# HicrestLaboratory/SPARTA

Hardware: AMD Instinct MI355X
Metric: Block-sparse SpMM GFLOP/s (higher is better)
Workload: dtype f32; 1 GPU; cant-like FEM 9x9x257 mesh x 3 dof (62451^2, 4325625 nnz; a synthetic STAND-IN for SuiteSparse cant, which cannot be fetched here), B = 128 cols, fp32; col_block_size=32, n_cols=128, block_rows=1952, nonzero_blocks=21910, vbs_area=22435840, parallelism=single GPU, launch=eager, preroll_steps=6457, kernel_rev=r5i

## Files before the change

### include/sparta_amd.h

```cpp
#ifndef SPARTA_AMD_H
#define SPARTA_AMD_H

#include <stdint.h>

#ifdef __cplusplus
extern "C" {
#endif

#define SPARTA_OK               0
#define SPARTA_ERR_INVALID     -1
#define SPARTA_ERR_ALLOC       -2
#define SPARTA_ERR_HIP         -3
#define SPARTA_ERR_UNSUPPORTED -4
#define SPARTA_ERR_IO          -5
#define SPARTA_ERR_NO_DEVICE   -6

#define SPARTA_F32  0
#define SPARTA_F16  1
#define SPARTA_BF16 2

#define SPARTA_COL_MAJOR 0
#define SPARTA_ROW_MAJOR 1

#define SPARTA_PTR_HOST   0
// ... 124 lines not shown

int sparta_vbs_save(const char* path, const sparta_vbs_host* v);
int sparta_vbs_load(const char* path, sparta_vbs_host* out);

int sparta_vbs_to_blocked_ell(const sparta_vbs_host* v, int64_t* ell_cols_out, int64_t* ell_col_ind, float* ell_values);

int sparta_blocking_info(int64_t rows, int64_t cols, const int64_t* rowptr, const int32_t* colidx,
                         const int64_t* grouping, int64_t col_block_size, int64_t* info_out, float* avg_height_out);

typedef struct sparta_vbs sparta_vbs_t;

int sparta_vbs_create(sparta_vbs_t** out, int64_t rows, int64_t cols, int64_t block_rows, int64_t block_col_size,
                      const int64_t* row_part, const int64_t* nzcount, const int64_t* jab, const float* mab,
                      int32_t dtype, int32_t device);

int sparta_vbs_create_range(sparta_vbs_t** out, int64_t rows, int64_t cols, int64_t block_rows, int64_t block_col_size,
                            const int64_t* row_part, const int64_t* nzcount, const int64_t* jab, const float* mab,
                            int64_t block_row_begin, int64_t block_row_end, int32_t dtype, int32_t device);

#define SPARTA_CREATE_UPDATABLE 1
#define SPARTA_CREATE_TRANSPOSE 2
int sparta_vbs_create_range_ex(sparta_vbs_t** out, int64_t rows, int64_t cols, int64_t block_rows, int64_t block_col_size,
                               const int64_t* row_part, const int64_t* nzcount, const int64_t* jab, const float* mab,
                               int64_t block_row_begin, int64_t block_row_end, int32_t dtype, int32_t device, int32_t flags);
int sparta_vbs_flags(const sparta_vbs_t* A, int32_t* flags_out);

int sparta_vbs_create_from_csr(sparta_vbs_t** out, int64_t rows, int64_t cols, const int64_t* rowptr, const int32_t* colidx, const float* vals,
                               const int64_t* grouping, int64_t col_block_size, int64_t row_block_size, int32_t force_fixed_size,
                               int32_t dtype, int32_t device);

int sparta_vbs_plan_stats(int64_t rows, int64_t cols, const int64_t* rowptr, const int32_t* colidx, const float* vals, const int64_t* grouping,
                          int64_t col_block_size, int64_t row_block_size, int32_t force_fixed_size, int32_t dtype, int64_t* stats);

int sparta_vbs_spmm(sparta_vbs_t* A, const void* B, int64_t ldb, int32_t b_layout, int32_t n_cols,
                    void* C, int64_t ldc, int32_t c_layout, int32_t accumulate,
                    int32_t ptr_space, void* stream, int32_t algo, float* dt_ms);

int sparta_vbs_spmm_gathered(sparta_vbs_t* A, const void* B_gathered, int64_t shard_rows, int64_t shard_stride, int32_t n_cols,
                             void* C, int64_t ldc, int32_t c_layout, int32_t accumulate, void* stream, int32_t algo, float* dt_ms);
int sparta_vbs_spmm_gathered_ld(sparta_vbs_t* A, const void* B_gathered, int64_t shard_rows, int64_t shard_ld, int64_t shard_stride, int32_t n_cols,
                                void* C, int64_t ldc, int32_t c_layout, int32_t accumulate, void* stream, int32_t algo, float* dt_ms);

int sparta_pack_blocks(const void* src, int64_t block_bytes, const int32_t* ids_dev, int64_t n_blocks, void* dst, void* stream);

int sparta_vbs_create_transposed(sparta_vbs_t** out, int64_t rows, int64_t cols, int64_t block_rows, int64_t block_col_size,
                                 const int64_t* row_part, const int64_t* nzcount, const int64_t* jab, const float* mab,
                                 int32_t dtype, int32_t device);
int sparta_vbs_spmm_ba(sparta_vbs_t* At, const void* B, int64_t ldb, int32_t M, void* C, int64_t ldc, int32_t accumulate,
                       int32_t ptr_space, void* stream, float* dt_ms);

int sparta_vbs_sddmm(sparta_vbs_t* A, const void* X, int64_t ldx, const void* Y, int64_t ldy, int32_t k, float* G, int32_t accumulate,
                     int32_t ptr_space, void* stream, float* dt_ms);

int sparta_vbs_set_values(sparta_vbs_t* A, const float* mab, int32_t ptr_space, void* stream, float* dt_ms);

typedef struct sparta_sgd_cfg { float lr, momentum, weight_decay, grad_scale; } sparta_sgd_cfg;
int sparta_vbs_sgd_step(sparta_vbs_t* A, float* W, const float* G, float* M, const sparta_sgd_cfg* cfg, void* stream, float* dt_ms);

typedef struct sparta_adam_cfg { float lr, beta1, beta2, eps, weight_decay, grad_scale; int32_t decoupled; int32_t reserved; } sparta_adam_cfg;
int sparta_vbs_adam_step(sparta_vbs_t* A, float* W, const float* G, float* M, float* V, void* S,
                         const sparta_adam_cfg* cfg, void* stream, float* dt_ms);
int sparta_vbs_step_info(const sparta_vbs_t* A, int64_t* info_out);

#define SPARTA_GRAD_CTL_BYTES 16448
#define SPARTA_GRAD_STATS_CHUNK 4096
#define SPARTA_GRAD_STATS_MAX_GRID 1024
typedef struct sparta_grad_ctl_cfg {
    float max_norm, growth_factor, backoff_factor;
    int32_t growth_interval;
    int32_t reserved[4];
} sparta_grad_ctl_cfg;
int sparta_grad_stats(const float* G, int64_t n, void* R, int32_t accumulate, void* stream, float* dt_ms);
int sparta_grad_ctl_finish(void* R, const sparta_grad_ctl_cfg* cfg, void* stream);
int sparta_vbs_sgd_step_ctl(sparta_vbs_t* A, float* W, const float* G, float* M, const sparta_sgd_cfg* cfg, const void* R, void* stream, float* dt_ms);
int sparta_vbs_adam_step_ctl(sparta_vbs_t* A, float* W, const float* G, float* M, float* V, void* S,
                             const sparta_adam_cfg* cfg, const void* R, void* stream, float* dt_ms);

int sparta_vbs_spmm_t(sparta_vbs_t* A, const void* X, int64_t ldx, int32_t n_cols, float* Ct, int64_t ldo, int32_t accumulate,
                      int32_t ptr_space, void* stream, float* dt_ms);
int sparta_spmm_t_host_check(int64_t rows, int64_t cols, int64_t block_rows, int64_t block_col_size, const int64_t* row_part,
                             const int64_t* nzcount, const int64_t* jab, const float* mab, int64_t block_row_begin, int64_t block_row_end,
                             const float* x, double* y, int64_t* info_out);
int sparta_frag_positions(const uint8_t* nonempty, uint8_t* pos, int32_t* pairs);

typedef struct sparta_b sparta_b_t;
int sparta_vbs_prepare_b(sparta_vbs_t* A, const void* B, int64_t ldb, int64_t shard_rows, int64_t shard_stride, int32_t n_cols, void* stream,
                         sparta_b_t** out);
int sparta_vbs_spmm_prepared(sparta_vbs_t* A, const sparta_b_t* Bp, void* C, int64_t ldc, int32_t c_layout, int32_t accumulate, void* stream,
                             float* dt_ms);
int sparta_b_destroy(sparta_b_t* Bp);

int sparta_vbs_set_class_timing(sparta_vbs_t* A, int32_t enable);
int sparta_vbs_class_times(sparta_vbs_t* A, float* ms_out);

int sparta_vbs_clock_mhz(sparta_vbs_t* A, double* mhz_out);

int sparta_vbs_destroy(sparta_vbs_t* A);

int sparta_vbs_info(const sparta_vbs_t* A, int64_t* info_out);

int sparta_vbs_sparse_info(const sparta_vbs_t* A, int64_t* info_out);

int sparta_vbs_colres_info(const sparta_vbs_t* A, int64_t* info_out);
int sparta_colres_host_check(int64_t rows, int64_t cols, const int64_t* rowptr, const int32_t* colidx, const float* vals, const int64_t* crow, const float* x,
                             float* y, int64_t* info_out);

int sparta_vbs_union_info(const sparta_vbs_t* A, int64_t* info_out);
int sparta_union_host_check(int64_t rows, int64_t cols, const int64_t* rowptr, const int32_t* colidx, const float* vals, const int64_t* grouping, int64_t col_block_size,
                            int64_t row_block_size, int32_t force_fixed_size, int32_t max_workers, const float* x, double* y, int64_t* info_out);

int sparta_vbs_hub_info(const sparta_vbs_t* A, int64_t* info_out);

int sparta_device_count(void);

const char* sparta_last_error(void);
const char* sparta_version(void);

#ifdef __cplusplus
}
#endif
#endif
```

### sparta_amd/__init__.py

```python
from ._lib import (SpartaError, LIB_PATH, F32, F16, BF16, COL_MAJOR, ROW_MAJOR, SPMM_MFMA, SPMM_EXACT,
                   FMT_EL, FMT_MTX, IO_COMPAT, IO_STRICT)
from .host import (CSR, BlockingEngine, VBR, get_permutation, get_partition, get_fixed_size_grouping,
                   row_distance, merge_rows, BLOCKING_ALGOS, save_grouping, read_grouping_file, blocking_csv_row,
                   save_blocking_data, CSV_COLUMNS)
from .device import DeviceVBS, vbs_multiply, device_count
from . import gen, dist, autograd, optim, gradctl
from .optim import VbsSGD, VbsAdamW
from .gradctl import GradCtl

KERNEL_REV = "r5i"

cublas_fixed_blocks_multiply = vbs_multiply
cublas_blockmat_batched = vbs_multiply
cutlas_fixed_blocks_multiply = vbs_multiply
cutlas_blockmat_batched = vbs_multiply
```

### sparta_amd/_lib.py

```python
import ctypes as C
import os

try:
    import torch
except ImportError:
    torch = None

_HERE = os.path.dirname(os.path.abspath(__file__))
LIB_PATH = os.environ.get("SPARTA_AMD_LIB") or os.path.join(_HERE, "libsparta_amd.so")

OK, ERR_INVALID, ERR_ALLOC, ERR_HIP, ERR_UNSUPPORTED, ERR_IO, ERR_NO_DEVICE = 0, -1, -2, -3, -4, -5, -6
F32, F16, BF16 = 0, 1, 2
COL_MAJOR, ROW_MAJOR = 0, 1
PTR_HOST, PTR_DEVICE = 0, 1
SPMM_MFMA, SPMM_EXACT = 0, 1
CREATE_UPDATABLE = 1
CREATE_TRANSPOSE = 2
GRAD_CTL_BYTES, GRAD_STATS_CHUNK, GRAD_STATS_MAX_GRID = 16448, 4096, 1024
FMT_EL, FMT_MTX = 0, 1
IO_COMPAT, IO_STRICT = 0, 1

SYMBOLS = [
    "sparta_reorder_cfg_default", "sparta_reorder", "sparta_get_permutation", "sparta_get_partition",
    "sparta_get_fixed_size_grouping", "sparta_row_distance", "sparta_merge_rows", "sparta_vbs_build",
    "sparta_vbs_host_free", "sparta_blocking_info", "sparta_vbs_create", "sparta_vbs_create_range", "sparta_vbs_create_from_csr",
    "sparta_vbs_spmm", "sparta_vbs_spmm_gathered", "sparta_vbs_spmm_gathered_ld", "sparta_pack_blocks", "sparta_vbs_create_transposed", "sparta_vbs_spmm_ba", "sparta_vbs_set_class_timing",
    "sparta_vbs_class_times", "sparta_vbs_clock_mhz", "sparta_vbs_destroy", "sparta_vbs_info", "sparta_vbs_sparse_info", "sparta_vbs_colres_info", "sparta_colres_host_check", "sparta_vbs_union_info", "sparta_union_host_check", "sparta_vbs_hub_info", "sparta_device_count", "sparta_last_error",
    "sparta_version",
    "sparta_csr_read", "sparta_csr_read_buffer", "sparta_csr_host_free", "sparta_csr_write_edgelist", "sparta_grouping_write", "sparta_grouping_read",
    "sparta_blocking_csv_row", "sparta_degree_permutation", "sparta_vbs_save", "sparta_vbs_load", "sparta_vbs_to_blocked_ell",
    "sparta_vbs_build_partition", "sparta_vbs_partition_check", "sparta_vbs_plan_stats",
    "sparta_vbs_prepare_b", "sparta_vbs_spmm_prepared", "sparta_b_destroy",
    "sparta_vbs_sddmm",
    "sparta_vbs_create_range_ex", "sparta_vbs_set_values", "sparta_vbs_flags", "sparta_frag_positions",
    "sparta_vbs_spmm_t", "sparta_spmm_t_host_check",
    "sparta_vbs_sgd_step", "sparta_vbs_step_info", "sparta_vbs_adam_step",
    "sparta_grad_stats", "sparta_grad_ctl_finish", "sparta_vbs_sgd_step_ctl", "sparta_vbs_adam_step_ctl",
]


class CsrHost(C.Structure):
    _fields_ = [("rows", C.c_int64), ("cols", C.c_int64), ("nnz", C.c_int64), ("pattern_only", C.c_int32),
                ("rowptr", C.POINTER(C.c_int64)), ("colidx", C.POINTER(C.c_int32)), ("vals", C.POINTER(C.c_float))]


class CsvFields(C.Structure):
    _fields_ = [("matrix", C.c_char_p), ("rows", C.c_int64), ("cols", C.c_int64), ("nonzeros", C.c_int64),
                ("symmetrize", C.c_int32), ("blocking_algo", C.c_int32), ("tau", C.c_float),
                ("row_block_size", C.c_int32), ("col_block_size", C.c_int32), ("use_pattern", C.c_int32),
                ("sim_use_groups", C.c_int32), ("sim_measure", C.c_int32), ("reorder", C.c_int32),
                ("exp_name", C.c_char_p), ("b_cols", C.c_int32), ("warmup", C.c_int32), ("exp_repetitions", C.c_int32),
                ("multiplication_algo", C.c_int32), ("n_streams", C.c_int32),
                ("time_to_block", C.c_float), ("time_to_merge", C.c_float), ("time_to_compare", C.c_float),
                ("vbr_nzcount", C.c_int64), ("vbr_nzblocks_count", C.c_int64), ("vbr_average_height", C.c_float),
                ("vbr_longest_row", C.c_int64), ("merge_counter", C.c_int64), ("comparison_counter", C.c_int64),
                ("average_merge_tau", C.c_float), ("average_row_distance", C.c_float),
                ("avg_time_multiply", C.c_float), ("std_time_multiply", C.c_float)]


class ReorderCfg(C.Structure):
    _fields_ = [("blocking_algo", C.c_int32), ("sim_measure", C.c_int32), ("tau", C.c_float), ("use_groups", C.c_int32),
                ("col_block_size", C.c_int64), ("row_block_size", C.c_int64), ("use_pattern", C.c_int32),
                ("force_fixed_size", C.c_int32), ("structured_m", C.c_int32), ("structured_n", C.c_int32),
                ("minhash_bands", C.c_int32), ("minhash_rows", C.c_int32), ("minhash_max_eval", C.c_int32), ("minhash_max_rows", C.c_int32)]


class ReorderStats(C.Structure):
    _fields_ = [("comparison_counter", C.c_int64), ("merge_counter", C.c_int64), ("average_row_distance", C.c_float),
                ("average_merge_tau", C.c_float), ("timer_total", C.c_float), ("timer_comparisons", C.c_float),
                ("timer_merges", C.c_float), ("reserved", C.c_int32)]


class VbsHost(C.Structure):
    _fields_ = [("rows", C.c_int64), ("cols", C.c_int64), ("block_rows", C.c_int64), ("block_cols", C.c_int64),
                ("block_col_size", C.c_int64), ("nztot", C.c_int64), ("nblocks", C.c_int64),
                ("row_part", C.POINTER(C.c_int64)), ("nzcount", C.POINTER(C.c_int64)), ("jab", C.POINTER(C.c_int64)),
                ("mab", C.POINTER(C.c_float))]


class SgdCfg(C.Structure):
    _fields_ = [("lr", C.c_float), ("momentum", C.c_float), ("weight_decay", C.c_float), ("grad_scale", C.c_float)]


class AdamCfg(C.Structure):
    _fields_ = [("lr", C.c_float), ("beta1", C.c_float), ("beta2", C.c_float), ("eps", C.c_float), ("weight_decay", C.c_float),
                ("grad_scale", C.c_float), ("decoupled", C.c_int32), ("reserved", C.c_int32)]


class GradCtlCfg(C.Structure):
    _fields_ = [("max_norm", C.c_float), ("growth_factor", C.c_float), ("backoff_factor", C.c_float), ("growth_interval", C.c_int32),
                ("reserved", C.c_int32 * 4)]


class SpartaError(RuntimeError):
    def __init__(self, code, msg):
        super().__init__("sparta_amd error %d: %s" % (code, msg))
        self.code = code


def _load():
    if not os.path.exists(LIB_PATH):
        raise ImportError("sparta_amd: %s is missing -- build it with `make -C sparta_amd/csrc` "
                          "(python -c 'import __graft_entry__ as g; g.build()'). There is no CPU fallback." % LIB_PATH)
    L = C.CDLL(LIB_PATH)
    i64p, i32p, f32p, vp = C.POINTER(C.c_int64), C.POINTER(C.c_int32), C.POINTER(C.c_float), C.c_void_p
    L.sparta_reorder_cfg_default.argtypes = [C.POINTER(ReorderCfg)]
    L.sparta_reorder_cfg_default.restype = None
    L.sparta_reorder.argtypes = [C.c_int64, C.c_int64, i64p, i32p, C.POINTER(ReorderCfg), i64p, C.POINTER(ReorderStats)]
    L.sparta_get_permutation.argtypes = [i64p, C.c_int64, i64p]
    L.sparta_get_partition.argtypes = [i64p, C.c_int64, i64p, i64p]
    L.sparta_get_fixed_size_grouping.argtypes = [i64p, C.c_int64, C.c_int64, i64p]
    L.sparta_row_distance.argtypes = [C.c_int32, i64p, C.c_int64, C.c_int64, i64p, C.c_int64, C.c_int64, C.c_int64, f32p]
    L.sparta_merge_rows.argtypes = [i64p, C.c_int64, i64p, C.c_int64, i64p, i64p]
    L.sparta_vbs_build.argtypes = [C.c_int64, C.c_int64, i64p, i32p, f32p, i64p, C.c_int64, C.c_int64, C.c_int32,
                                   C.POINTER(VbsHost)]
    L.sparta_vbs_host_free.argtypes = [C.POINTER(VbsHost)]
    L.sparta_vbs_build_partition.argtypes = [C.c_int64, C.c_int64, i64p, i32p, f32p, i64p, C.c_int64, C.c_int64, C.POINTER(VbsHost)]
    L.sparta_vbs_partition_check.argtypes = [i64p, C.c_int64, C.c_int64]
    L.sparta_vbs_save.argtypes = [C.c_char_p, C.POINTER(VbsHost)]
    L.sparta_vbs_load.argtypes = [C.c_char_p, C.POINTER(VbsHost)]
    L.sparta_vbs_to_blocked_ell.argtypes = [C.POINTER(VbsHost), i64p, i64p, f32p]
    L.sparta_vbs_host_free.restype = None
    L.sparta_blocking_info.argtypes = [C.c_int64, C.c_int64, i64p, i32p, i64p, C.c_int64, i64p, f32p]
    L.sparta_vbs_create.argtypes = [C.POINTER(vp), C.c_int64, C.c_int64, C.c_int64, C.c_int64, i64p, i64p, i64p, f32p,
                                    C.c_int32, C.c_int32]
    L.sparta_vbs_create_range.argtypes = [C.POINTER(vp), C.c_int64, C.c_int64, C.c_int64, C.c_int64, i64p, i64p, i64p, f32p,
                                          C.c_int64, C.c_int64, C.c_int32, C.c_int32]
    L.sparta_vbs_create_range_ex.argtypes = [C.POINTER(vp), C.c_int64, C.c_int64, C.c_int64, C.c_int64, i64p, i64p, i64p, f32p,
                                             C.c_int64, C.c_int64, C.c_int32, C.c_int32, C.c_int32]
    L.sparta_vbs_set_values.argtypes = [vp, f32p, C.c_int32, vp, f32p]
    L.sparta_vbs_sgd_step.argtypes = [vp, f32p, f32p, f32p, C.POINTER(SgdCfg), vp, f32p]
    L.sparta_vbs_adam_step.argtypes = [vp, f32p, f32p, f32p, f32p, vp, C.POINTER(AdamCfg), vp, f32p]
    L.sparta_vbs_step_info.argtypes = [vp, i64p]
    L.sparta_grad_stats.argtypes = [f32p, C.c_int64, vp, C.c_int32, vp, f32p]
    L.sparta_grad_ctl_finish.argtypes = [vp, C.POINTER(GradCtlCfg), vp]
    L.sparta_vbs_sgd_step_ctl.argtypes = [vp, f32p, f32p, f32p, C.POINTER(SgdCfg), vp, vp, f32p]
    L.sparta_vbs_adam_step_ctl.argtypes = [vp, f32p, f32p, f32p, f32p, vp, C.POINTER(AdamCfg), vp, vp, f32p]
    L.sparta_vbs_flags.argtypes = [vp, i32p]
    L.sparta_vbs_spmm_t.argtypes = [vp, vp, C.c_int64, C.c_int32, f32p, C.c_int64, C.c_int32, C.c_int32, vp, f32p]
    L.sparta_spmm_t_host_check.argtypes = [C.c_int64, C.c_int64, C.c_int64, C.c_int64, i64p, i64p, i64p, f32p, C.c_int64, C.c_int64, f32p, C.POINTER(C.c_double), i64p]
    L.sparta_frag_positions.argtypes = [C.POINTER(C.c_uint8), C.POINTER(C.c_uint8), i32p]
    L.sparta_vbs_create_from_csr.argtypes = [C.POINTER(vp), C.c_int64, C.c_int64, i64p, i32p, f32p, i64p, C.c_int64, C.c_int64, C.c_int32, C.c_int32, C.c_int32]
    L.sparta_vbs_plan_stats.argtypes = [C.c_int64, C.c_int64, i64p, i32p, f32p, i64p, C.c_int64, C.c_int64, C.c_int32, C.c_int32, i64p]
    L.sparta_vbs_prepare_b.argtypes = [vp, vp, C.c_int64, C.c_int64, C.c_int64, C.c_int32, vp, C.POINTER(vp)]
    L.sparta_vbs_spmm_prepared.argtypes = [vp, vp, vp, C.c_int64, C.c_int32, C.c_int32, vp, f32p]
    L.sparta_b_destroy.argtypes = [vp]
    L.sparta_vbs_create_transposed.argtypes = [C.POINTER(vp), C.c_int64, C.c_int64, C.c_int64, C.c_int64, i64p, i64p, i64p, f32p, C.c_int32, C.c_int32]
    L.sparta_vbs_spmm_ba.argtypes = [vp, vp, C.c_int64, C.c_int32, vp, C.c_int64, C.c_int32, C.c_int32, vp, f32p]
    L.sparta_vbs_spmm.argtypes = [vp, vp, C.c_int64, C.c_int32, C.c_int32, vp, C.c_int64, C.c_int32, C.c_int32, C.c_int32, vp,
                                  C.c_int32, f32p]
    L.sparta_vbs_sddmm.argtypes = [vp, vp, C.c_int64, vp, C.c_int64, C.c_int32, f32p, C.c_int32, C.c_int32, vp, f32p]
    L.sparta_vbs_spmm_gathered.argtypes = [vp, vp, C.c_int64, C.c_int64, C.c_int32, vp, C.c_int64, C.c_int32, C.c_int32, vp, C.c_int32, f32p]
    L.sparta_vbs_spmm_gathered_ld.argtypes = [vp, vp, C.c_int64, C.c_int64, C.c_int64, C.c_int32, vp, C.c_int64, C.c_int32, C.c_int32, vp, C.c_int32, f32p]
    L.sparta_pack_blocks.argtypes = [vp, C.c_int64, vp, C.c_int64, vp, vp]
    L.sparta_vbs_set_class_timing.argtypes = [vp, C.c_int32]
    L.sparta_vbs_class_times.argtypes = [vp, f32p]
    L.sparta_vbs_clock_mhz.argtypes = [vp, C.POINTER(C.c_double)]
    L.sparta_vbs_destroy.argtypes = [vp]
    L.sparta_csr_read.argtypes = [C.c_char_p, C.c_char_p, C.c_int32, C.c_int32, C.c_int32, C.c_int32, C.POINTER(CsrHost)]
    L.sparta_csr_read_buffer.argtypes = [C.c_char_p, C.c_int64, C.c_char_p, C.c_int32, C.c_int32, C.c_int32, C.c_int32, C.POINTER(CsrHost)]
    L.sparta_csr_host_free.argtypes = [C.POINTER(CsrHost)]
    L.sparta_csr_host_free.restype = None
    L.sparta_csr_write_edgelist.argtypes = [C.c_char_p, C.c_int64, i64p, i32p, C.c_char_p, C.c_int32]
    L.sparta_grouping_write.argtypes = [C.c_char_p, i64p, C.c_int64]
    L.sparta_grouping_read.argtypes = [C.c_char_p, C.c_int64, i64p, C.c_int64, C.POINTER(C.c_int64)]
    L.sparta_blocking_csv_row.argtypes = [C.POINTER(CsvFields), C.c_char_p, C.c_int64, C.c_char_p, C.c_int64]
    L.sparta_degree_permutation.argtypes = [C.c_int64, i64p, C.c_int32, i64p]
    L.sparta_vbs_info.argtypes = [vp, i64p]
    L.sparta_vbs_sparse_info.argtypes = [vp, i64p]
    L.sparta_vbs_hub_info.argtypes = [vp, i64p]
    L.sparta_vbs_colres_info.argtypes = [vp, i64p]
    L.sparta_colres_host_check.argtypes = [C.c_int64, C.c_int64, i64p, i32p, f32p, i64p, f32p, f32p, i64p]
    L.sparta_vbs_union_info.argtypes = [vp, i64p]
    L.sparta_union_host_check.argtypes = [C.c_int64, C.c_int64, i64p, i32p, f32p, i64p, C.c_int64, C.c_int64, C.c_int32, C.c_int32, f32p, C.POINTER(C.c_double), i64p]
    L.sparta_device_count.argtypes = []
    L.sparta_last_error.restype = C.c_char_p
    L.sparta_version.restype = C.c_char_p
    return L


lib = _load()


def check(rc):
    if rc != OK:
        raise SpartaError(rc, lib.sparta_last_error().decode(errors="replace"))
```

### sparta_amd/csrc/vbs_capi.cpp

```cpp
#include <memory>

#include <cmath>
#include "vbs_kernel_common.hpp"

using namespace sparta_dev;

#define SPARTA_GUARD_BEGIN try {
#define SPARTA_GUARD_END(name_)                                                                                       \
    }                                                                                                                  \
    catch (const std::bad_alloc&) { return sparta::fail(SPARTA_ERR_ALLOC, std::string(name_) + ": out of host memory"); } \
    catch (const std::exception& e) { return sparta::fail(SPARTA_ERR_INVALID, std::string(name_) + ": " + e.what()); }  \
    catch (...) { return sparta::fail(SPARTA_ERR_INVALID, std::string(name_) + ": unknown C++ exception"); }

namespace {

bool force_generic() { const char* e = std::getenv("SPARTA_FORCE_GENERIC"); return e && e[0] == '1'; }

thread_local bool g_capturing = false;
struct CaptureScope {
    explicit CaptureScope(hipStream_t st, bool device_ptrs) {
        hipStreamCaptureStatus cs = hipStreamCaptureStatusNone;
        g_capturing = device_ptrs && hipStreamIsCapturing(st, &cs) == hipSuccess && cs != hipStreamCaptureStatusNone;
    }
    ~CaptureScope() { g_capturing = false; }
};
int capture_refusal(const char* what, const char* entry = "sparta_vbs_spmm") {
    return sparta::fail(SPARTA_ERR_UNSUPPORTED, std::string(entry) + ": the stream is being captured and this call still has to " + what +
                                                 " -- run it once outside the capture first");
}

int ensure_scratch(void** ptr, size_t* have, size_t need) {
    if (*have >= need) return SPARTA_OK;
    if (g_capturing) return capture_refusal("allocate scratch memory");
    if (*ptr) { (void)hipFree(*ptr); *ptr = nullptr; *have = 0; }
    HIP_TRY(hipMalloc(ptr, need));
    *have = need;
    return SPARTA_OK;
}

void destroy_impl(sparta_vbs* v) {
    if (!v) return;
    DeviceGuard g(v->device);
    if (v->d_A) (void)hipFree(v->d_A);
    if (v->d_jab) (void)hipFree(v->d_jab);
    for (int c = 0; c < 4; c++)
        if (v->d_tiles[c]) (void)hipFree(v->d_tiles[c]);
    if (v->d_brows) (void)hipFree(v->d_brows);
    for (int ty = 0; ty < 2; ty++) {
        if (v->d_steps[ty]) (void)hipFree(v->d_steps[ty]);
        if (v->d_steps_g[ty]) (void)hipFree(v->d_steps_g[ty]);
        if (v->d_wrange[ty]) (void)hipFree(v->d_wrange[ty]);
    }
    if (v->d_a_frag) (void)hipFree(v->d_a_frag);
    if (v->d_hub_steps) (void)hipFree(v->d_hub_steps);
    if (v->d_hub_steps_g) (void)hipFree(v->d_hub_steps_g);
    if (v->d_hub_tiles) (void)hipFree(v->d_hub_tiles);
    if (v->d_hub_wrange) (void)hipFree(v->d_hub_wrange);
    if (v->d_hub_A) (void)hipFree(v->d_hub_A);
    if (v->d_fix) (void)hipFree(v->d_fix);
    if (v->d_fix_slots) (void)hipFree(v->d_fix_slots);
    if (v->d_big_fix) (void)hipFree(v->d_big_fix);
    if (v->d_ws) (void)hipFree(v->d_ws);
    if (v->d_btail) (void)hipFree(v->d_btail);
    if (v->d_tune) (void)hipFree(v->d_tune);
    if (v->d_B16) (void)hipFree(v->d_B16);
    if (v->d_Bt) (void)hipFree(v->d_Bt);
    if (v->d_Ct) (void)hipFree(v->d_Ct);
    if (v->d_clk) (void)hipFree(v->d_clk);
    if (v->tev0) (void)hipEventDestroy(v->tev0);
    if (v->tev1) (void)hipEventDestroy(v->tev1);
    if (v->d_sp_rowptr) (void)hipFree(v->d_sp_rowptr);
    if (v->d_sp_col) (void)hipFree(v->d_sp_col);
    if (v->d_sp_val) (void)hipFree(v->d_sp_val);
    if (v->d_sp_crow) (void)hipFree(v->d_sp_crow);
    if (v->d_sp_list) (void)hipFree(v->d_sp_list);
    if (v->d_sp_segs) (void)hipFree(v->d_sp_segs);
    if (v->d_sp_stream_begin) (void)hipFree(v->d_sp_stream_begin);
    if (v->d_sp_long) (void)hipFree(v->d_sp_long);
    if (v->d_sp_part) (void)hipFree(v->d_sp_part);
    if (v->d_cr_col) (void)hipFree(v->d_cr_col);
    if (v->d_cr_val) (void)hipFree(v->d_cr_val);
    if (v->d_cr_meta) (void)hipFree(v->d_cr_meta);
    if (v->d_cr_parts) (void)hipFree(v->d_cr_parts);
    if (v->d_cr_mode) (void)hipFree(v->d_cr_mode);
    if (v->cr_small.col) (void)hipFree(v->cr_small.col);
    if (v->cr_small.val) (void)hipFree(v->cr_small.val);
    if (v->cr_small.meta) (void)hipFree(v->cr_small.meta);
    if (v->cr_small.dest) (void)hipFree(v->cr_small.dest);
    if (v->cr_small.longs) (void)hipFree(v->cr_small.longs);
    if (v->cr_small.parts) (void)hipFree(v->cr_small.parts);
    if (v->d_cr_dest) (void)hipFree(v->d_cr_dest);
    if (v->d_cr_longs) (void)hipFree(v->d_cr_longs);
    for (int ty = 0; ty < kUnionTypes; ty++) {
        if (v->d_u_rec[ty]) (void)hipFree(v->d_u_rec[ty]);
        if (v->d_u_ids[ty]) (void)hipFree(v->d_u_ids[ty]);
        if (v->d_u_a[ty]) (void)hipFree(v->d_u_a[ty]);
        if (v->d_u_wrange[ty]) (void)hipFree(v->d_u_wrange[ty]);
        if (v->d_u_tail[ty]) (void)hipFree(v->d_u_tail[ty]);
    }
    if (v->d_Brm) (void)hipFree(v->d_Brm);
    if (v->d_B) (void)hipFree(v->d_B);
    if (v->d_C) (void)hipFree(v->d_C);
    if (v->d_sd_items) (void)hipFree(v->d_sd_items);
    if (v->d_sd_ws) (void)hipFree(v->d_sd_ws);
    if (v->d_sd_h16) (void)hipFree(v->d_sd_h16);
    for (int ty = 0; ty < 2; ty++)
        if (v->d_upd_map[ty]) (void)hipFree(v->d_upd_map[ty]);
    if (v->d_upd_hub) (void)hipFree(v->d_upd_hub);
    if (v->d_upd_ws) (void)hipFree(v->d_upd_ws);
    if (v->d_t_items) (void)hipFree(v->d_t_items);
    if (v->d_t_blocks) (void)hipFree(v->d_t_blocks);
    if (v->d_t_A) (void)hipFree(v->d_t_A);
    if (v->d_t_src) (void)hipFree(v->d_t_src);
    if (v->d_t_ws) (void)hipFree(v->d_t_ws);
    if (v->d_t_h16) (void)hipFree(v->d_t_h16);
    if (v->ev0) (void)hipEventDestroy(v->ev0);
    if (v->ev1) (void)hipEventDestroy(v->ev1);
    for (int c = 0; c < 4; c++)
        for (int e = 0; e < 2; e++)
            if (v->cev[c][e]) (void)hipEventDestroy(v->cev[c][e]);
    delete v;
}




constexpr int64_t kColresCells = 160 * 1024 / 4;
struct ColresHost {
    std::vector<uint16_t> col;
    std::vector<float> val;
    std::vector<ColresPartDev> parts;
    std::vector<int32_t> meta, dest;
    std::vector<uint8_t> mode;
    std::vector<ColresLong> longs;
    std::vector<int32_t> krange;
    int32_t max_slices = 0, max_cells = 0, lmax = 0;
// ... 426 lines not shown
                    if (stream_of[(size_t)k] == x) streamed.insert(streamed.end(), sp_segs.begin() + w_begin[(size_t)k], sp_segs.begin() + w_begin[(size_t)k + 1]);
            }
            sp_stream_begin[8] = (int32_t)streamed.size();
            sp_segs.swap(streamed);
        }
    }
    n_sp_short = (int64_t)sp_list.size(); n_sp_long = (int64_t)sp_long.size();
    trace.lap("sparse rows (device form)");
    const uint8_t* skip = sparse_flag.empty() ? nullptr : sparse_flag.data();

    std::vector<TileDesc> tiles[4];
    std::vector<BlockRowDesc> brows;
    std::vector<int32_t> jab32((size_t)std::max<int64_t>(nblocks, 1));
    for (int64_t q = 0; q < nblocks; q++) {
        const int64_t jb = jab[jab_lo + q];
        if (jb < 0 || jb >= block_cols) return fail(SPARTA_ERR_INVALID, "sparta_vbs_create: jab entry out of range");
        jab32[(size_t)q] = (int32_t)jb;
    }
    int64_t exec_area = 0;
    {
        int64_t jo2 = 0, mo2 = 0;
        const int64_t row0 = row_part[br0];
        for (int64_t ib = br0; ib < br1; ib++) {
            const int64_t h = row_part[ib + 1] - row_part[ib];
            const int64_t nb = nzcount[ib];
            if (h > 0) {
                BlockRowDesc br{mo2, jo2, (int32_t)nb, (int32_t)h, (int32_t)(row_part[ib] - row0), 0};
                brows.push_back(br);
                int64_t r0 = skip && skip[ib - br0] ? h : 0;
                while (r0 < h) {
                    const int64_t rem = h - r0;
                    int cls;
                    int64_t mt;
                    if (rem > 32) { cls = 2; mt = std::min<int64_t>(rem, 64); }
                    else if (rem > 16) { cls = 1; mt = rem; }
                    else { cls = 0; mt = rem; }
                    const bool tail = (cols % w != 0) && nb > 0 && jab[jab_lo + jo2 + nb - 1] == block_cols - 1;
                    TileDesc t{mo2 + r0, jo2, (int32_t)nb, (int32_t)h, (int32_t)(row_part[ib] - row0 + r0),
                               (int32_t)mt | (tail ? TILE_TAIL : 0)};
                    tiles[cls].push_back(t);
                    const int64_t padded = cls == 0 ? 16 : ((mt + 31) / 32) * 32;
                    exec_area += padded * w * nb;
                    r0 += mt;
                }
            }
            jo2 += nb;
            mo2 += nb * h * w;
        }
    }

    int64_t n_real[4];
    for (int c = 0; c < 4; c++) n_real[c] = (int64_t)tiles[c].size();
    {
        const char* ord = std::getenv("SPARTA_TILE_ORDER");
        const bool natural = ord && std::strcmp(ord, "natural") == 0;
        for (int c = 0; c < 4; c++) {
            std::vector<TileDesc>& L = tiles[c];
            if (L.empty()) continue;
            const int64_t rows_pad = c == 0 ? 16 : (c == 1 ? 32 : 64);
            auto cost = [&](const TileDesc& t) { return (int64_t)t.nb * rows_pad + rows_pad / 4; };
            int64_t total = 0;
            for (const TileDesc& t : L) total += cost(t);
            std::vector<std::vector<TileDesc>> chunk(8);
            int64_t acc_cost = 0;
            for (const TileDesc& t : L) {
                int x = (int)std::min<int64_t>(7, (acc_cost * 8) / std::max<int64_t>(total, 1));
                chunk[(size_t)x].push_back(t);
                acc_cost += cost(t);
            }
            size_t maxlen = 0;
            for (auto& ch : chunk) {
                if (!natural) std::stable_sort(ch.begin(), ch.end(), [&](const TileDesc& a, const TileDesc& b) { return cost(a) > cost(b); });
                maxlen = std::max(maxlen, ch.size());
            }
            std::vector<TileDesc> arranged(maxlen * 8, TileDesc{0, 0, 0, 1, 0, 0});
            for (size_t x = 0; x < 8; x++)
                for (size_t j = 0; j < chunk[x].size(); j++) arranged[j * 8 + x] = chunk[x][j];
            L.swap(arranged);
        }
    }

    StreamPlanHost plan;
    {
        StreamPlanIn pin{cols, w, br0, br1, jab_lo, mab_lo, row_part, nzcount, jab, mab, dtype, device, skip, updatable && h16};
        trace.lap("tile lists");
        if (int rc = build_stream_plans(pin, plan)) return rc;
        trace.lap("stream plans");
    }
    UnionDevPlan uplan;
    if (ext && !ext->uni.empty()) {
        int n_cus = 256;
        if (!plan_debug) { hipDeviceProp_t pr; if (hipGetDeviceProperties(&pr, device) == hipSuccess && pr.multiProcessorCount > 0) n_cus = pr.multiProcessorCount; }
        const int wpc = [] { const char* e = std::getenv("SPARTA_UNION_WPC"); return e ? std::max(1, atoi(e)) : 3; }();
        if (int rc = build_union_plan(ext->uni, wpc * n_cus, uplan, dtype, n_cus)) return rc;
        trace.lap("column-compacted tiles (plan)");
    }
    std::vector<StepRec>(&steps)[2] = plan.steps;
    std::vector<int32_t>(&wrange)[2] = plan.wrange;
    std::vector<FixRec>& fix = plan.fix;
    std::vector<int32_t>& fix_slots = plan.fix_slots;
    const int n_workers = plan.n_workers, n_split = plan.n_split;
    const int64_t kp = plan.kp;

    struct VbsDeleter { void operator()(sparta_vbs* q) const { destroy_impl(q); } };
    std::unique_ptr<sparta_vbs, VbsDeleter> hold(new (std::nothrow) sparta_vbs);
    if (plan_debug) return fail(SPARTA_ERR_NO_DEVICE, "sparta_vbs_create: no HIP device visible (this path has no CPU fallback)");
    sparta_vbs* v = hold.get();
    if (!v) return fail(SPARTA_ERR_ALLOC, "sparta_vbs_create: out of host memory");
    v->device = device; v->dtype = dtype; v->create_flags = flags;
    v->zero_ranges = plan.zero_ranges;
    v->rows = row_part[br1] - row_part[br0]; v->cols = cols; v->block_rows = br1 - br0; v->w = w;
    v->nblocks = nblocks; v->nztot = nztot; v->exec_area = exec_area;

    DeviceGuard guard(device);
    if (!guard.ok) return fail(SPARTA_ERR_HIP, "sparta_vbs_create: hipSetDevice failed");
#define CREATE_TRY(expr)                                                                                     \
    do {                                                                                                     \
        hipError_t e_ = (expr);                                                                              \
        if (e_ != hipSuccess) {                                                                              \
            std::string m_ = std::string(#expr) + ": " + hipGetErrorString(e_);                              \
            return fail(e_ == hipErrorOutOfMemory ? SPARTA_ERR_ALLOC : SPARTA_ERR_HIP, m_);                  \
        }                                                                                                    \
    } while (0)
    if (!h16) {
        v->a_bytes = (nztot + 128) * (int64_t)sizeof(float);
        CREATE_TRY(hipMalloc((void**)&v->d_A, (size_t)v->a_bytes));
        CREATE_TRY(hipMemset(v->d_A, 0, (size_t)v->a_bytes));
        if (nztot > 0) CREATE_TRY(hipMemcpy(v->d_A, mab + mab_lo, (size_t)nztot * sizeof(float), hipMemcpyHostToDevice));
    } else {
        const std::vector<uint16_t>& a0 = plan.a16_steps[0];
        const std::vector<uint16_t>& a1 = plan.a16_steps[1];
        v->a_bytes = ((int64_t)a0.size() + (int64_t)a1.size() + 8 * 64 * 64) * (int64_t)sizeof(uint16_t);
        CREATE_TRY(hipMalloc((void**)&v->d_A, (size_t)v->a_bytes));
        CREATE_TRY(hipMemset(v->d_A, 0, (size_t)v->a_bytes));
        if (!a0.empty()) CREATE_TRY(hipMemcpy(v->d_A, a0.data(), a0.size() * sizeof(uint16_t), hipMemcpyHostToDevice));
        if (!a1.empty()) CREATE_TRY(hipMemcpy((uint16_t*)v->d_A + a0.size(), a1.data(), a1.size() * sizeof(uint16_t), hipMemcpyHostToDevice));
        v->kp16 = (int)kp;
        v->upd_base[1] = (int64_t)a0.size();
        for (int ty = 0; ty < 2 && updatable; ty++) {
            if (plan.upd_map[ty].empty()) continue;
            for (const UpdSlice& u : plan.upd_map[ty]) v->upd_cover[ty] += (int64_t)(u.rows_lo + u.rows_hi) * kp;
            CREATE_TRY(hipMalloc((void**)&v->d_upd_map[ty], plan.upd_map[ty].size() * sizeof(UpdSlice)));
            CREATE_TRY(hipMemcpy(v->d_upd_map[ty], plan.upd_map[ty].data(), plan.upd_map[ty].size() * sizeof(UpdSlice), hipMemcpyHostToDevice));
        }
        if (updatable && !plan.upd_hub.empty()) {
            v->n_upd_hub = (int64_t)plan.upd_hub.size();
            CREATE_TRY(hipMalloc((void**)&v->d_upd_hub, plan.upd_hub.size() * sizeof(UpdSlice)));
            CREATE_TRY(hipMemcpy(v->d_upd_hub, plan.upd_hub.data(), plan.upd_hub.size() * sizeof(UpdSlice), hipMemcpyHostToDevice));
        }
    }
    CREATE_TRY(hipMalloc((void**)&v->d_jab, jab32.size() * sizeof(int32_t)));
    CREATE_TRY(hipMemcpy(v->d_jab, jab32.data(), jab32.size() * sizeof(int32_t), hipMemcpyHostToDevice));
    for (int c = 0; c < 4; c++) {
        v->n_tiles[c] = (int64_t)tiles[c].size();
        v->n_real_tiles[c] = n_real[c];
        if (tiles[c].empty()) continue;
        CREATE_TRY(hipMalloc((void**)&v->d_tiles[c], tiles[c].size() * sizeof(TileDesc)));
        CREATE_TRY(hipMemcpy(v->d_tiles[c], tiles[c].data(), tiles[c].size() * sizeof(TileDesc), hipMemcpyHostToDevice));
    }
    v->n_brows = (int64_t)brows.size();
    if (!brows.empty()) {
        CREATE_TRY(hipMalloc((void**)&v->d_brows, brows.size() * sizeof(BlockRowDesc)));
        CREATE_TRY(hipMemcpy(v->d_brows, brows.data(), brows.size() * sizeof(BlockRowDesc), hipMemcpyHostToDevice));
    }
    if (!steps[0].empty() || !steps[1].empty() || !fix.empty() || !plan.zero_ranges.empty() || plan.n_hub_steps > 0) {
        v->has_tail = (cols % w) != 0;
        v->n_workers = n_workers; v->n_fix = (int32_t)fix.size(); v->n_split = n_split; v->n_slots = (int32_t)fix_slots.size();
        std::vector<int32_t> big_fix;
        for (size_t q = 0; q < fix.size(); q++) {
            v->max_tile_slots = std::max(v->max_tile_slots, fix[q].n_slots);
            if (fix[q].n_slots > 2 * kFixGroup) big_fix.push_back((int32_t)q);
        }
        v->n_big_fix = (int32_t)big_fix.size();
        if (!big_fix.empty()) {
            CREATE_TRY(hipMalloc((void**)&v->d_big_fix, big_fix.size() * sizeof(int32_t)));
            CREATE_TRY(hipMemcpy(v->d_big_fix, big_fix.data(), big_fix.size() * sizeof(int32_t), hipMemcpyHostToDevice));
        }
        for (int ty = 0; ty < 2; ty++) {
            std::vector<StepRec>& st = steps[ty];
            v->n_steps[ty] = (int64_t)st.size();
            if (st.empty()) continue;
            if (updatable && !h16) for (const StepRec& r : st) v->upd_cover[ty] += (int64_t)(r.mt_flags & 0xffff) * SK_KP;
            for (int k = 0; k < 32; k++) { StepRec d = st[(size_t)v->n_steps[ty] - 1]; d.mt_flags = (d.mt_flags & ~(STEP_LAST | STEP_SPLIT)) | STEP_FIRST; st.push_back(d); }
            CREATE_TRY(hipMalloc((void**)&v->d_steps[ty], st.size() * sizeof(StepRec)));
            CREATE_TRY(hipMemcpy(v->d_steps[ty], st.data(), st.size() * sizeof(StepRec), hipMemcpyHostToDevice));
            v->h_steps[ty] = st;
            v->n_plan_tiles[ty] = plan.n_plan_tiles[ty];
            v->tiles_row_aligned[ty] = plan.tiles_row_aligned[ty];
            if (ty == 0) v->wide16 = plan.wide16;
            CREATE_TRY(hipMalloc((void**)&v->d_wrange[ty], wrange[ty].size() * sizeof(int32_t)));
            CREATE_TRY(hipMemcpy(v->d_wrange[ty], wrange[ty].data(), wrange[ty].size() * sizeof(int32_t), hipMemcpyHostToDevice));
        }
        if (!plan.a_frag.empty()) {
            if (hipMalloc((void**)&v->d_a_frag, plan.a_frag.size() * sizeof(float)) == hipSuccess) {
                CREATE_TRY(hipMemcpy(v->d_a_frag, plan.a_frag.data(), plan.a_frag.size() * sizeof(float), hipMemcpyHostToDevice));
                v->a_bytes += (int64_t)(plan.a_frag.size() * sizeof(float));
            } else {
                (void)hipGetLastError();
                v->d_a_frag = nullptr;
            }
        }
        if (plan.n_hub_steps > 0) {
            v->hub_g = plan.hub_g; v->hub_workers = plan.hub_workers; v->n_hub_steps = plan.n_hub_steps; v->hub_area = plan.hub_area;
            v->hub_union_area = plan.hub_union_area; v->n_hub_tiles = plan.n_hub_tiles; v->n_hub_groups = plan.n_hub_groups;
            v->hub_chunks = plan.hub_chunks; v->hub_segments = plan.hub_segments;
            CREATE_TRY(hipMalloc((void**)&v->d_hub_steps, plan.hub_steps.size() * sizeof(HubStep)));
            CREATE_TRY(hipMemcpy(v->d_hub_steps, plan.hub_steps.data(), plan.hub_steps.size() * sizeof(HubStep), hipMemcpyHostToDevice));
            CREATE_TRY(hipMalloc((void**)&v->d_hub_tiles, plan.hub_tiles.size() * sizeof(HubTile)));
            CREATE_TRY(hipMemcpy(v->d_hub_tiles, plan.hub_tiles.data(), plan.hub_tiles.size() * sizeof(HubTile), hipMemcpyHostToDevice));
            CREATE_TRY(hipMalloc((void**)&v->d_hub_wrange, plan.hub_wrange.size() * sizeof(int32_t)));
            CREATE_TRY(hipMemcpy(v->d_hub_wrange, plan.hub_wrange.data(), plan.hub_wrange.size() * sizeof(int32_t), hipMemcpyHostToDevice));
            const size_t a_elems = plan.hub_a16_elems;
            CREATE_TRY(hipMalloc((void**)&v->d_hub_A, (a_elems + 64) * sizeof(uint16_t)));
            if (a_elems > 0) CREATE_TRY(hipMemcpy(v->d_hub_A, plan.hub_a16.get(), a_elems * sizeof(uint16_t), hipMemcpyHostToDevice));
            v->a_bytes += (int64_t)(a_elems * sizeof(uint16_t));
            v->exec_area += plan.hub_union_area;
            v->h_hub_steps.swap(plan.hub_steps);
        }
        if (!fix.empty()) {
            CREATE_TRY(hipMalloc((void**)&v->d_fix, fix.size() * sizeof(FixRec)));
            CREATE_TRY(hipMemcpy(v->d_fix, fix.data(), fix.size() * sizeof(FixRec), hipMemcpyHostToDevice));
        }
        CREATE_TRY(hipMalloc((void**)&v->d_fix_slots, std::max<size_t>(fix_slots.size(), 1) * sizeof(int32_t)));
        if (!fix_slots.empty()) CREATE_TRY(hipMemcpy(v->d_fix_slots, fix_slots.data(), fix_slots.size() * sizeof(int32_t), hipMemcpyHostToDevice));
    }
    for (int ty = 0; ty < kUnionTypes; ty++) {
        if (uplan.n_steps[ty] == 0) continue;
        v->u_workers[ty] = uplan.n_workers[ty]; v->u_steps[ty] = uplan.n_steps[ty]; v->u_tiles[ty] = uplan.n_tiles[ty]; v->u_steps_total += uplan.n_steps[ty];
        CREATE_TRY(hipMalloc((void**)&v->d_u_rec[ty], uplan.rec[ty].size() * sizeof(UnionRec)));
        CREATE_TRY(hipMemcpy(v->d_u_rec[ty], uplan.rec[ty].data(), uplan.rec[ty].size() * sizeof(UnionRec), hipMemcpyHostToDevice));
        CREATE_TRY(hipMalloc((void**)&v->d_u_ids[ty], uplan.ids[ty].size() * sizeof(int32_t)));
        CREATE_TRY(hipMemcpy(v->d_u_ids[ty], uplan.ids[ty].data(), uplan.ids[ty].size() * sizeof(int32_t), hipMemcpyHostToDevice));
        const size_t a_bytes_ty = h16 ? uplan.a16[ty].size() * sizeof(uint16_t) : uplan.a[ty].size() * sizeof(float);
        CREATE_TRY(hipMalloc((void**)&v->d_u_a[ty], a_bytes_ty));
        CREATE_TRY(hipMemcpy(v->d_u_a[ty], h16 ? (const void*)uplan.a16[ty].data() : (const void*)uplan.a[ty].data(), a_bytes_ty, hipMemcpyHostToDevice));
        CREATE_TRY(hipMalloc((void**)&v->d_u_wrange[ty], uplan.wrange[ty].size() * sizeof(int32_t)));
        CREATE_TRY(hipMemcpy(v->d_u_wrange[ty], uplan.wrange[ty].data(), uplan.wrange[ty].size() * sizeof(int32_t), hipMemcpyHostToDevice));
        CREATE_TRY(hipMalloc(&v->d_u_tail[ty], uplan.tail[ty].size() * sizeof(uint32_t)));
        CREATE_TRY(hipMemcpy(v->d_u_tail[ty], uplan.tail[ty].data(), uplan.tail[ty].size() * sizeof(uint32_t), hipMemcpyHostToDevice));
        v->a_bytes += (int64_t)(a_bytes_ty + uplan.ids[ty].size() * sizeof(int32_t) + uplan.tail[ty].size() * sizeof(uint32_t));
        v->exec_area += uplan.n_steps[ty] * 32 * uplan.type_rows[ty];
        v->u_exec_area += uplan.n_steps[ty] * 32 * uplan.type_rows[ty];
    }
    if (ext) {
        v->u_area = uplan.area; v->u_cols = uplan.cols; v->u_nnz = ext->uni.nnz; v->u_tail_nnz = ext->uni.tail_nnz; v->u_rows = uplan.rows;
        for (int hh = 0; hh < 2; hh++) { v->u_tiles_h[hh] = uplan.tiles_by_height[hh]; v->u_steps_h[hh] = uplan.steps_by_height[hh]; }
    }
    if (!sp_crow.empty()) {
        v->n_sp_rows = (int64_t)sp_crow.size(); v->n_sp_short = n_sp_short; v->n_sp_long = n_sp_long; v->sp_nnz = sp_rowptr.back();
        CREATE_TRY(hipMalloc((void**)&v->d_sp_rowptr, sp_rowptr.size() * sizeof(int64_t)));
        CREATE_TRY(hipMemcpy(v->d_sp_rowptr, sp_rowptr.data(), sp_rowptr.size() * sizeof(int64_t), hipMemcpyHostToDevice));
        CREATE_TRY(hipMalloc((void**)&v->d_sp_col, (sp_col.size() + 64) * sizeof(int32_t)));
        CREATE_TRY(hipMemset(v->d_sp_col, 0, (sp_col.size() + 64) * sizeof(int32_t)));
        CREATE_TRY(hipMalloc((void**)&v->d_sp_val, (sp_val.size() + 64) * sizeof(float)));
        CREATE_TRY(hipMemset(v->d_sp_val, 0, (sp_val.size() + 64) * sizeof(float)));
        if (!sp_col.empty()) {
            CREATE_TRY(hipMemcpy(v->d_sp_col, sp_col.data(), sp_col.size() * sizeof(int32_t), hipMemcpyHostToDevice));
            CREATE_TRY(hipMemcpy(v->d_sp_val, sp_val.data(), sp_val.size() * sizeof(float), hipMemcpyHostToDevice));
        }
        CREATE_TRY(hipMalloc((void**)&v->d_sp_crow, sp_crow.size() * sizeof(int32_t)));
        CREATE_TRY(hipMemcpy(v->d_sp_crow, sp_crow.data(), sp_crow.size() * sizeof(int32_t), hipMemcpyHostToDevice));
        if (!sp_list.empty()) {
            CREATE_TRY(hipMalloc((void**)&v->d_sp_list, sp_list.size() * sizeof(int32_t)));
            CREATE_TRY(hipMemcpy(v->d_sp_list, sp_list.data(), sp_list.size() * sizeof(int32_t), hipMemcpyHostToDevice));
        }
        if (!sp_long.empty()) {
            v->n_sp_segs = (int64_t)sp_segs.size();
            CREATE_TRY(hipMalloc(&v->d_sp_segs, sp_segs.size() * sizeof(SpSegRec)));
            CREATE_TRY(hipMemcpy(v->d_sp_segs, sp_segs.data(), sp_segs.size() * sizeof(SpSegRec), hipMemcpyHostToDevice));
            if (!sp_stream_begin.empty()) {
                CREATE_TRY(hipMalloc((void**)&v->d_sp_stream_begin, 9 * sizeof(int32_t)));
                CREATE_TRY(hipMemcpy(v->d_sp_stream_begin, sp_stream_begin.data(), 9 * sizeof(int32_t), hipMemcpyHostToDevice));
                for (int x = 0; x < 8; x++) v->sp_max_stream = std::max<int64_t>(v->sp_max_stream, sp_stream_begin[(size_t)x + 1] - sp_stream_begin[(size_t)x]);
            }
            CREATE_TRY(hipMalloc(&v->d_sp_long, sp_long.size() * sizeof(SpLongRec)));
            CREATE_TRY(hipMemcpy(v->d_sp_long, sp_long.data(), sp_long.size() * sizeof(SpLongRec), hipMemcpyHostToDevice));
        }
    }
    if (!h16 && !sp_crow.empty()) {
        ColresHost H;
        if (build_colres(v->rows, cols, sp_rowptr, sp_col, sp_val, sp_crow, H)) {
            CREATE_TRY(hipMalloc(&v->d_cr_col, H.col.size() * sizeof(uint16_t)));
            CREATE_TRY(hipMemcpy(v->d_cr_col, H.col.data(), H.col.size() * sizeof(uint16_t), hipMemcpyHostToDevice));
            if (!H.val.empty()) {
// ... 157 lines not shown
}

int sparta_vbs_create_from_csr(sparta_vbs_t** out, int64_t rows, int64_t cols, const int64_t* rowptr, const int32_t* colidx, const float* vals,
                               const int64_t* grouping, int64_t col_block_size, int64_t row_block_size, int32_t force_fixed_size,
                               int32_t dtype, int32_t device) {
    return create_from_csr_impl(out, rows, cols, rowptr, colidx, vals, grouping, col_block_size, row_block_size, force_fixed_size, dtype, device, false);
}

int sparta_vbs_create_transposed(sparta_vbs_t** out, int64_t rows, int64_t cols, int64_t block_rows, int64_t w, const int64_t* row_part,
                                 const int64_t* nzcount, const int64_t* jab, const float* mab, int32_t dtype, int32_t device) {
    using sparta::fail;
    if (!out) return fail(SPARTA_ERR_INVALID, "sparta_vbs_create_transposed: out is NULL");
    *out = nullptr;
    if (rows <= 0 || cols <= 0 || block_rows <= 0 || w <= 0 || !row_part || !nzcount)
        return fail(SPARTA_ERR_INVALID, "sparta_vbs_create_transposed: bad dimensions or NULL index array");
    if (rows > INT32_MAX || cols > INT32_MAX) return fail(SPARTA_ERR_UNSUPPORTED, "sparta_vbs_create_transposed: more than 2^31 - 1 rows or columns");
    try {
        std::vector<int64_t> rp((size_t)cols + 1, 0);
        int64_t jo = 0, mo = 0;
        for (int64_t ib = 0; ib < block_rows; ib++) {
            const int64_t h = row_part[ib + 1] - row_part[ib], nb = nzcount[ib];
            if (h < 0 || nb < 0) return fail(SPARTA_ERR_INVALID, "sparta_vbs_create_transposed: invalid row_part / nzcount");
            for (int64_t b = 0; b < nb; b++) {
                const int64_t c0 = jab[jo + b] * w;
                if (c0 < 0 || c0 >= cols) return fail(SPARTA_ERR_INVALID, "sparta_vbs_create_transposed: jab entry out of range");
                for (int64_t k = 0; k < w && c0 + k < cols; k++)
                    for (int64_t i = 0; i < h; i++) rp[(size_t)(c0 + k) + 1] += mab[mo + (b * w + k) * h + i] != 0.0f;
            }
            jo += nb; mo += nb * h * w;
        }
        for (int64_t j = 0; j < cols; j++) rp[(size_t)j + 1] += rp[(size_t)j];
        std::vector<int32_t> ci((size_t)rp[(size_t)cols]);
        std::vector<float> va((size_t)rp[(size_t)cols]);
        std::vector<int64_t> fill(rp.begin(), rp.end() - 1);
        jo = 0; mo = 0;
        for (int64_t ib = 0; ib < block_rows; ib++) {
            const int64_t h = row_part[ib + 1] - row_part[ib], nb = nzcount[ib];
            for (int64_t b = 0; b < nb; b++) {
                const int64_t c0 = jab[jo + b] * w;
                for (int64_t k = 0; k < w && c0 + k < cols; k++)
                    for (int64_t i = 0; i < h; i++) {
                        const float a = mab[mo + (b * w + k) * h + i];
                        if (a != 0.0f) { const int64_t q = fill[(size_t)(c0 + k)]++; ci[(size_t)q] = (int32_t)(row_part[ib] + i); va[(size_t)q] = a; }
                    }
            }
            jo += nb; mo += nb * h * w;
        }
        std::vector<int64_t> grouping((size_t)cols);
        for (int64_t j = 0; j < cols; j++) grouping[(size_t)j] = j / w;
        return create_from_csr_impl(out, cols, rows, rp.data(), ci.data(), va.data(), grouping.data(), 32, 0, 0, dtype, device, true);
    } catch (const std::bad_alloc&) {
        return fail(SPARTA_ERR_ALLOC, "sparta_vbs_create_transposed: out of host memory");
    } catch (const std::exception& e) {
        return fail(SPARTA_ERR_INVALID, std::string("sparta_vbs_create_transposed: ") + e.what());
    }
}

int sparta_vbs_spmm_ba(sparta_vbs_t* At, const void* B, int64_t ldb, int32_t M, void* C, int64_t ldc, int32_t accumulate, int32_t ptr_space,
                       void* stream, float* dt_ms) {
    using sparta::fail;
    if (!At) return fail(SPARTA_ERR_INVALID, "sparta_vbs_spmm_ba: NULL handle");
    if (M <= 0 || ldb < M || ldc < M) return fail(SPARTA_ERR_INVALID, "sparta_vbs_spmm_ba: need M > 0, ldb >= M, ldc >= M");
    return sparta_vbs_spmm(At, B, ldb, SPARTA_ROW_MAJOR, M, C, ldc, SPARTA_ROW_MAJOR, accumulate, ptr_space, stream, SPARTA_SPMM_MFMA, dt_ms);
}

int sparta_vbs_create(sparta_vbs_t** out, int64_t rows, int64_t cols, int64_t block_rows, int64_t w, const int64_t* row_part,
                      const int64_t* nzcount, const int64_t* jab, const float* mab, int32_t dtype, int32_t device) {
    return sparta_vbs_create_range(out, rows, cols, block_rows, w, row_part, nzcount, jab, mab, 0, block_rows, dtype, device);
}

int sparta_vbs_destroy(sparta_vbs_t* A) {
    destroy_impl(A);
    return SPARTA_OK;
}

int sparta_vbs_info(const sparta_vbs_t* A, int64_t* info) {
    if (!A || !info) return sparta::fail(SPARTA_ERR_INVALID, "sparta_vbs_info: NULL argument");
    std::memset(info, 0, 16 * sizeof(int64_t));
    info[0] = A->rows; info[1] = A->cols; info[2] = A->block_rows; info[3] = A->w; info[4] = A->nblocks; info[5] = A->nztot;
    for (int c = 0; c < 3; c++) info[6 + c] = A->n_real_tiles[c];
    info[9] = A->n_sp_rows;
    info[10] = A->a_bytes; info[11] = A->exec_area;
    info[12] = A->n_steps[0] + A->n_steps[1]; info[13] = A->n_workers; info[14] = A->n_split; info[15] = A->last_path;
    return SPARTA_OK;
}

int sparta_vbs_flags(const sparta_vbs_t* A, int32_t* flags_out) {
    if (!A || !flags_out) return sparta::fail(SPARTA_ERR_INVALID, "sparta_vbs_flags: NULL argument");
    *flags_out = A->create_flags;
    return SPARTA_OK;
}

int sparta_frag_positions(const uint8_t* nonempty, uint8_t* pos, int32_t* pairs) {
    if (!nonempty || !pos || !pairs) return sparta::fail(SPARTA_ERR_INVALID, "sparta_frag_positions: NULL argument");
    uint32_t mask = 0;
    for (int k = 0; k < 32; k++) mask |= (uint32_t)(nonempty[k] != 0) << k;
    for (int k = 0; k < 32; k++) pos[k] = (uint8_t)frag_position(mask, k);
    *pairs = frag_pairs(mask);
    return SPARTA_OK;
}

int sparta_vbs_hub_info(const sparta_vbs_t* A, int64_t* info) {
    if (!A || !info) return sparta::fail(SPARTA_ERR_INVALID, "sparta_vbs_hub_info: NULL argument");
    info[0] = A->n_hub_steps; info[1] = A->n_hub_tiles; info[2] = A->n_hub_groups; info[3] = A->n_hub_steps > 0 ? A->hub_g : 0;
    info[4] = A->hub_area; info[5] = A->hub_union_area; info[6] = A->n_hub_steps > 0 ? A->hub_workers : 0; info[7] = A->hub_chunks; info[8] = A->hub_segments; info[9] = 0;
    return SPARTA_OK;
}

int sparta_vbs_union_info(const sparta_vbs_t* A, int64_t* info) {
    if (!A || !info) return sparta::fail(SPARTA_ERR_INVALID, "sparta_vbs_union_info: NULL argument");
    info[0] = A->u_tiles_h[0]; info[1] = A->u_tiles_h[1]; info[2] = A->u_steps_h[0]; info[3] = A->u_steps_h[1];
    info[4] = A->u_area; info[5] = A->u_cols; info[6] = A->u_nnz; info[7] = 0;
    for (int ty = 0; ty < kUnionTypes; ty++) info[7] = std::max<int64_t>(info[7], A->u_workers[ty]);
    info[8] = A->u_rows; info[9] = A->u_tail_nnz;
    info[10] = A->u_exec_area; info[11] = A->u_steps_total > 0 ? (A->dtype == SPARTA_F32 ? 16 : 32) : 0;
    return SPARTA_OK;
}

int sparta_vbs_sparse_info(const sparta_vbs_t* A, int64_t* info) {
    if (!A || !info) return sparta::fail(SPARTA_ERR_INVALID, "sparta_vbs_sparse_info: NULL argument");
    info[0] = A->n_sp_rows; info[1] = A->sp_nnz; info[2] = A->n_sp_short; info[3] = A->n_sp_long;
    return SPARTA_OK;
}

int sparta_colres_host_check(int64_t rows, int64_t cols, const int64_t* rowptr, const int32_t* colidx, const float* vals, const int64_t* crow, const float* x, float* y,
                             int64_t* info) {
    using sparta::fail;
    SPARTA_GUARD_BEGIN
    if (rows <= 0 || cols <= 0 || !rowptr || !colidx || !vals || !x || !y || !info) return fail(SPARTA_ERR_INVALID, "sparta_colres_host_check: bad argument");
    std::vector<int64_t> rp{0};
    std::vector<int32_t> ci, cr;
    std::vector<float> va;
    for (int64_t i = 0; i < rows; i++) {
        if (crow && crow[i] == -1) continue;
        ci.insert(ci.end(), colidx + rowptr[i], colidx + rowptr[i + 1]);
        va.insert(va.end(), vals + rowptr[i], vals + rowptr[i + 1]);
        rp.push_back((int64_t)ci.size());
        cr.push_back(crow ? (int32_t)(uint32_t)(crow[i] & 0xffffffffll) : (int32_t)i);
    }
    ColresHost H;
    for (int k = 0; k < 12; k++) info[k] = 0;
    const int force_parts = [] { const char* e = std::getenv("SPARTA_COLRES_FORCE_PARTS"); return e ? atoi(e) : 0; }();
    if (!build_colres(rows, cols, rp, ci, va, cr, H, force_parts)) return SPARTA_OK;
    const int n_ranges = (int)H.krange.size() - 1;
    for (const ColresPartDev& pd : H.parts) {
        const int32_t* wslice = H.meta.data() + pd.meta;
        const int32_t* woff = wslice + 17;
        const int32_t* bnd = woff + (size_t)n_ranges * 17;
        std::vector<float> acc((size_t)pd.n_slices * 64, 0.0f), cell((size_t)pd.plane, 0.0f);
        for (int r = 0; r < n_ranges; r++) {
            const int64_t k0 = H.krange[(size_t)r], klen = H.krange[(size_t)r + 1] - k0;
            for (int w = 0; w < kColresWaves; w++) {
                for (int32_t i = wslice[w]; i < wslice[w + 1]; i++) {
                    const int32_t t0 = i == wslice[w] ? 0 : bnd[(size_t)r * pd.n_slices + i - 1], t1 = bnd[(size_t)r * pd.n_slices + i];
                    if (t1 <= t0) return fail(SPARTA_ERR_INVALID, "sparta_colres_host_check: an empty slice in the image");
                    for (int l = 0; l < 64; l++) {
                        float a = acc[(size_t)i * 64 + (size_t)l];
                        for (int32_t t = t0; t < t1; t++) {
                            for (int u = 0; u < 4; u++) {
                                const size_t at = ((size_t)(woff[(size_t)r * 17 + w] + t) * 64 + (size_t)l) * 4 + (size_t)u;
                                const int64_t c = H.col[at];
                                if (c > klen) return fail(SPARTA_ERR_INVALID, "sparta_colres_host_check: column out of range in the image");
                                const float b = c == klen ? 0.0f : x[k0 + c];
                                a = H.val.empty() ? a + b : std::fma(H.val[at], b, a);
                            }
                        }
// ... 68 lines not shown
    if (!A || !info) return sparta::fail(SPARTA_ERR_INVALID, "sparta_vbs_colres_info: NULL argument");
    info[0] = A->cr_slices; info[1] = A->cr_entries; info[2] = A->cr_long; info[3] = A->cr_plane; info[4] = A->cr_lmax; info[5] = A->last_colres_nc;
    info[6] = A->cr_slices > 0 ? A->sp_nnz : 0; info[7] = A->cr_slices > 0 && A->cr_unit ? 1 : 0; info[8] = A->cr_parts; info[9] = A->cr_ranges; info[10] = A->cr_small.n_parts; info[11] = A->last_colres_small ? 1 : 0;
    return SPARTA_OK;
}

#ifdef SPARTA_TIMELINE
int sparta_debug_timeline(sparta_vbs_t* A, long long* out) {
    if (!A || !out || !A->d_clk) return -1;
    DeviceGuard guard(A->device);
    if (hipDeviceSynchronize() != hipSuccess) return -1;
    return hipMemcpy(out, A->d_clk + 16, (4 * 64 * 8 + 2048) * sizeof(long long), hipMemcpyDeviceToHost) == hipSuccess ? 0 : -1;
}
#endif

int sparta_vbs_clock_mhz(sparta_vbs_t* A, double* mhz_out) {
    using sparta::fail;
    if (!A || !mhz_out) return fail(SPARTA_ERR_INVALID, "sparta_vbs_clock_mhz: NULL argument");
    DeviceGuard guard(A->device);
    for (int c = 0; c < 4; c++) mhz_out[c] = 0.0;
    if (!A->class_timing || !A->d_clk) return SPARTA_OK;
    long long h[16];
    HIP_TRY(hipDeviceSynchronize());
    HIP_TRY(hipMemcpy(h, A->d_clk, sizeof(h), hipMemcpyDeviceToHost));
    for (int c = 0; c < 4; c++) {
        if (!A->class_ran[c]) continue;
        const long long dc = h[4 * c + 2] - h[4 * c], dr = h[4 * c + 3] - h[4 * c + 1];
        if (dr > 0 && dc > 0) mhz_out[c] = (double)dc / (double)dr * 100.0;
    }
    return SPARTA_OK;
}

}

namespace {

bool ring_tiles(const sparta_vbs_t* A) { return !A->tiles_row_aligned[0] && A->n_steps[0] < 6 * A->n_plan_tiles[0]; }

int32_t c_store_nt(const sparta_vbs_t* A, int ty, const float* C, int64_t ldc, bool c_row_major, bool ring = false) {
    if (const char* e = std::getenv("SPARTA_C_NT")) return atoi(e) != 0;
    if (A->n_plan_tiles[ty] <= 0) return 0;
    if (A->n_steps[ty] >= 6 * A->n_plan_tiles[ty]) return 1;
    return !c_row_major && (A->tiles_row_aligned[ty] || ring) && ldc % 32 == 0 && ((uintptr_t)C % 128) == 0;
}

void launch_zero_ranges(sparta_vbs_t* A, float* C, int64_t ldc, bool c_row_major, int n_cols, hipStream_t st) {
    for (const auto& zr : A->zero_ranges) {
        const int64_t n_lines = c_row_major ? zr.second : (int64_t)n_cols, line_len = c_row_major ? (int64_t)n_cols : zr.second;
        const unsigned gx = (unsigned)std::max<int64_t>(1, std::min<int64_t>(64, (line_len / 4 + kThreads - 1) / kThreads));
        const unsigned gy = (unsigned)std::max<int64_t>(1, std::min<int64_t>(n_lines, 16384));
        launch_zero_rows(dim3(gx, gy), st, C, ldc, (int)c_row_major, zr.first, zr.second, n_cols);
    }
}

int ensure_gathered_steps(sparta_vbs_t* A, int64_t shard_rows, hipStream_t st) {
    if (A->g_shard_rows == shard_rows) return SPARTA_OK;
    if (g_capturing) return capture_refusal("build the step lists of this slab height");
    for (int ty = 0; ty < 2; ty++) {
        if (A->h_steps[ty].empty()) continue;
        std::vector<StepRec> g = A->h_steps[ty];
        for (StepRec& r : g) { r.pad = (int32_t)(r.b_row / shard_rows); r.b_row = (int32_t)(r.b_row % shard_rows); }
        if (!A->d_steps_g[ty]) HIP_TRY(hipMalloc((void**)&A->d_steps_g[ty], g.size() * sizeof(StepRec)));
        HIP_TRY(hipMemcpyAsync(A->d_steps_g[ty], g.data(), g.size() * sizeof(StepRec), hipMemcpyHostToDevice, st));
        HIP_TRY(hipStreamSynchronize(st));
    }
    if (!A->h_hub_steps.empty()) {
        std::vector<HubStep> g = A->h_hub_steps;
        for (HubStep& r : g) if (!(r.flags & STEP_TAIL)) { r.shard = (int32_t)(r.b_row / shard_rows); r.b_row = (int32_t)(r.b_row % shard_rows); }
        if (!A->d_hub_steps_g) HIP_TRY(hipMalloc((void**)&A->d_hub_steps_g, g.size() * sizeof(HubStep)));
        HIP_TRY(hipMemcpyAsync(A->d_hub_steps_g, g.data(), g.size() * sizeof(HubStep), hipMemcpyHostToDevice, st));
        HIP_TRY(hipStreamSynchronize(st));
    }
    A->g_shard_rows = shard_rows;
    return SPARTA_OK;
}


int ensure_legacy_image(sparta_vbs_t* A, hipStream_t st) {
    if (A->d_A || A->dtype != SPARTA_F32) return SPARTA_OK;
    if (g_capturing) return capture_refusal("rebuild the reference-layout image of A");
    const size_t bytes = (size_t)(A->nztot + 128) * sizeof(float);
    HIP_TRY(hipMalloc((void**)&A->d_A, bytes));
    HIP_TRY(hipMemsetAsync(A->d_A, 0, bytes, st));
    if (A->n_steps[0] > 0) launch_f32_legacy_from_frag(st, A->d_steps[0], A->n_steps[0], A->d_a_frag, A->d_A);
    HIP_TRY(hipGetLastError());
    A->a_bytes += (int64_t)bytes;
    return SPARTA_OK;
}
void drop_legacy_image(sparta_vbs_t* A) {
    static const bool keep = [] { const char* e = std::getenv("SPARTA_F32_KEEP_LEGACY"); return e && atoi(e) != 0; }();
    if (A->create_flags & SPARTA_CREATE_TRANSPOSE) return;
    if (keep || g_capturing || A->legacy_dropped || !A->d_A || !A->d_a_frag || A->dtype != SPARTA_F32 || A->n_steps[1] != 0 || A->n_sp_rows != 0 || A->class_timing) return;
    (void)hipFree(A->d_A);
    A->d_A = nullptr;
    A->a_bytes -= (int64_t)((A->nztot + 128) * sizeof(float));
    A->legacy_dropped = true;
}

int ensure_brm(sparta_vbs_t* A, const void* dB, int64_t ldb, bool b_row_major, int64_t shard_rows, int64_t shard_stride, int bk, int32_t n_cols, hipStream_t st,
               bool aligned16) {
    if (A->brm_ready) return SPARTA_OK;
    const size_t esz = bk == 0 ? 4 : 2;
    const int64_t per16 = 16 / (int64_t)esz;
    if (b_row_major && shard_rows == 0 && (!aligned16 || (ldb % per16 == 0 && ((uintptr_t)dB % 16) == 0))) { A->brm_ready = dB; A->brm_ld = ldb; return SPARTA_OK; }
    if (A->prepared_brm && !b_row_major) { A->brm_ready = A->prepared_brm; A->brm_ld = A->prepared_ld; return SPARTA_OK; }
    if (g_capturing && A->d_Brm_bytes < (size_t)A->cols * (size_t)((n_cols + per16 - 1) / per16 * per16) * esz) return capture_refusal("allocate the row-major copy of B");
    const int64_t ld = (n_cols + per16 - 1) / per16 * per16;
    if (int rc = ensure_scratch(&A->d_Brm, &A->d_Brm_bytes, (size_t)A->cols * (size_t)ld * esz)) return rc;
    if (b_row_major) {
        HIP_TRY(hipMemcpy2DAsync(A->d_Brm, (size_t)ld * esz, dB, (size_t)ldb * esz, (size_t)n_cols * esz, (size_t)A->cols, hipMemcpyDeviceToDevice, st));
    } else {
        const int64_t n_wg = ((A->cols + 63) / 64) * (int64_t)((n_cols + 63) / 64);
        if (n_wg > INT32_MAX) return sparta::fail(SPARTA_ERR_UNSUPPORTED, "sparta_vbs_spmm: B too large for the transpose grid");
        launch_b_to_row_major(bk != 0, (unsigned)n_wg, st, dB, ldb, shard_rows, shard_stride, A->cols, (int)n_cols, A->d_Brm, ld);
    }
    A->brm_ready = A->d_Brm; A->brm_ld = ld;
    return SPARTA_OK;
}

int launch_union_tiles(sparta_vbs_t* A, const void* dB, int64_t ldb, bool b_row_major, int64_t shard_rows, int64_t shard_stride, int32_t n_cols, float* dC,
                       int64_t ldc, bool c_row_major, bool accumulate, hipStream_t st) {
    if (A->u_steps_total == 0) return SPARTA_OK;
    if ((c_row_major ? 64 * ldc + 128 : 32 * ldc + 128) * 4 >= ((int64_t)1 << 31) - 65536)
        return sparta::fail(SPARTA_ERR_UNSUPPORTED, "sparta_vbs_spmm: leading dimension of C too large for the column-compacted tile kernel (32-bit offsets inside a tile)");
    const int bk = A->dtype == SPARTA_F32 ? 0 : (A->dtype == SPARTA_BF16 ? 2 : 1);
    if (int rc = ensure_brm(A, dB, ldb, b_row_major, shard_rows, shard_stride, bk, n_cols, st, true)) return rc;
    UnionParams up;
    up.B = (const float*)A->brm_ready; up.ldb = A->brm_ld; up.C = dC; up.ldc = ldc;
    up.n_cols = n_cols; up.accumulate = accumulate ? 1 : 0; up.c_row_major = c_row_major ? 1 : 0;
    up.pad = [] { const char* e = std::getenv("SPARTA_UNION_PROBE"); return e ? atoi(e) : 0; }();
    for (int ty = 0; ty < kUnionTypes; ty++) {
        UnionSide& sd = up.side[ty];
        sd.rec = A->d_u_rec[ty]; sd.ids = A->d_u_ids[ty]; sd.A = A->d_u_a[ty]; sd.worker_range = A->d_u_wrange[ty]; sd.tail = (const uint2*)A->d_u_tail[ty];
        sd.n_workers = A->u_steps[ty] > 0 ? A->u_workers[ty] : 0;
        const char* e = std::getenv("SPARTA_C_NT");
        sd.c_nt = e ? (atoi(e) != 0) : (A->u_steps[ty] >= 6 * A->u_tiles[ty] ? 1 : 0);
    }
    if (bk == 0) launch_union_f32((unsigned)((n_cols + kTN - 1) / kTN), st, up);
    else launch_union_h16(bk == 2, (unsigned)((n_cols + kTN - 1) / kTN), st, up);
    HIP_TRY(hipGetLastError());
    return SPARTA_OK;
}

int launch_sparse_rows(sparta_vbs_t* A, const void* dB, int64_t ldb, bool b_row_major, int64_t shard_rows, int64_t shard_stride, int bk,
                       int32_t n_cols, float* dC, int64_t ldc, bool c_row_major, bool accumulate, hipStream_t st) {
    const size_t esz = bk == 0 ? 4 : 2;
    A->last_colres_nc = 0;
    if (bk == 0 && A->cr_slices > 0 && !b_row_major && !c_row_major && shard_rows == 0) {
        const int nc = colres_columns(A, n_cols);
        if (nc > 0) {
            int nc_used = nc;
            bool used_small = false;
            ColresParams cp;
            cp.col4 = (const uint2*)A->d_cr_col; cp.val4 = (const float4*)A->d_cr_val; cp.parts = (const ColresPartDev*)A->d_cr_parts; cp.meta = A->d_cr_meta;
            cp.dest = A->d_cr_dest; cp.longs = (const ColresLong*)A->d_cr_longs; cp.mode = (const uint8_t*)A->d_cr_mode;
            cp.B = (const float*)dB; cp.ldb = ldb; cp.C = dC; cp.ldc = ldc;
            for (int r = 0; r <= kColresMaxRanges; r++) cp.krange[r] = A->cr_krange[r];
            cp.n_parts = A->cr_parts; cp.n_ranges = A->cr_ranges; cp.N = n_cols; cp.accumulate = accumulate ? 1 : 0;
            cp.vec_out = ldc % 4 == 0 && ((uintptr_t)dC % 16) == 0 ? 1 : 0;
            cp.vec_in = ldb % 4 == 0 && ((uintptr_t)dB % 16) == 0 ? 1 : 0;
            cp.probe = [] { const char* e = std::getenv("SPARTA_COLRES_PROBE"); return e ? atoi(e) : 0; }();
            size_t lds_bytes = (size_t)A->cr_plane * (size_t)nc * sizeof(float);
            if (A->cr_small.slices > 0) {
                const char* es = std::getenv("SPARTA_COLRES_SMALL");
                const char* en = std::getenv("SPARTA_COLRES_NC");
                const int fit = (int)std::min<int64_t>(std::min<int64_t>(4, kColresCells / A->cr_plane), n_cols);
                int ncs = 0;
                for (int c = 1; c <= fit && ncs == 0; c++) if ((int64_t)((n_cols + c - 1) / c) * A->cr_small.n_parts <= 256 && A->cr_small.slices <= colres_max_slices(c)) ncs = c;
                if (ncs > 0 && !en && !(es && atoi(es) == 0)) {
                    nc_used = ncs; used_small = true;
                    cp.col4 = (const uint2*)A->cr_small.col; cp.val4 = (const float4*)A->cr_small.val; cp.parts = (const ColresPartDev*)A->cr_small.parts; cp.meta = A->cr_small.meta;
                    cp.dest = A->cr_small.dest; cp.longs = (const ColresLong*)A->cr_small.longs;
                    cp.n_parts = A->cr_small.n_parts;
                    lds_bytes = (size_t)A->cr_plane * (size_t)ncs * sizeof(float);
                }
// ... 240 lines not shown
        A->prepared_brm = nullptr;
        if (int rc = spmm16_core(A, A->d_Bt, ld_t, b_layout, shard_rows, shard_rows > 0 ? shard_rows * kTN : 0, kTN, A->d_Ct, A->rows, SPARTA_COL_MAJOR, 0,
                                 SPARTA_PTR_DEVICE, st, algo, nullptr)) return rc;
    }
    launch_col_tail_merge(st, (const float*)A->d_Ct, A->rows, dC, ldc, (int)(c_layout == SPARTA_ROW_MAJOR), n_main, n_t, (int)(accumulate != 0));
    HIP_TRY(hipGetLastError());
    if (dt_ms) {
        HIP_TRY(hipEventRecord(A->tev1, st));
        HIP_TRY(hipEventSynchronize(A->tev1));
        HIP_TRY(hipEventElapsedTime(dt_ms, A->tev0, A->tev1));
    }
    if (ptr_space == SPARTA_PTR_HOST) {
        HIP_TRY(hipMemcpyAsync(C, A->d_C, c_elems * sizeof(float), hipMemcpyDeviceToHost, st));
        HIP_TRY(hipStreamSynchronize(st));
    }
    return SPARTA_OK;
}

int spmm_impl(sparta_vbs_t* A, const void* B, int64_t ldb, int32_t b_layout, int64_t shard_rows, int64_t shard_stride, int32_t n_cols,
              void* C, int64_t ldc, int32_t c_layout, int32_t accumulate, int32_t ptr_space, void* stream, int32_t algo,
              float* dt_ms) {
    using sparta::fail;
    if (!A || !B || !C) return fail(SPARTA_ERR_INVALID, "sparta_vbs_spmm: NULL argument");
    if (n_cols <= 0) return fail(SPARTA_ERR_INVALID, "sparta_vbs_spmm: n_cols must be > 0");
    if (b_layout != SPARTA_COL_MAJOR && b_layout != SPARTA_ROW_MAJOR) return fail(SPARTA_ERR_INVALID, "sparta_vbs_spmm: bad b_layout");
    if (c_layout != SPARTA_COL_MAJOR && c_layout != SPARTA_ROW_MAJOR) return fail(SPARTA_ERR_INVALID, "sparta_vbs_spmm: bad c_layout");
    if (shard_rows == 0 && ldb < (b_layout == SPARTA_COL_MAJOR ? A->cols : (int64_t)n_cols))
        return fail(SPARTA_ERR_INVALID, "sparta_vbs_spmm: ldb too small");
    if (ldc < (c_layout == SPARTA_COL_MAJOR ? A->rows : (int64_t)n_cols)) return fail(SPARTA_ERR_INVALID, "sparta_vbs_spmm: ldc too small");
    if (algo != SPARTA_SPMM_MFMA && algo != SPARTA_SPMM_EXACT) return fail(SPARTA_ERR_INVALID, "sparta_vbs_spmm: bad algo");
    if (ptr_space != SPARTA_PTR_HOST && ptr_space != SPARTA_PTR_DEVICE) return fail(SPARTA_ERR_INVALID, "sparta_vbs_spmm: bad ptr_space");

    DeviceGuard guard(A->device);
    if (!guard.ok) return fail(SPARTA_ERR_HIP, "sparta_vbs_spmm: hipSetDevice failed");
    hipStream_t st = (hipStream_t)stream;
    const CaptureScope capture(st, ptr_space == SPARTA_PTR_DEVICE);
    if (g_capturing && dt_ms) return capture_refusal("time the product (dt_ms != NULL synchronises)");
    if (A->dtype != SPARTA_F32)
        return spmm16_impl(A, B, ldb, b_layout, shard_rows, shard_stride, n_cols, C, ldc, c_layout, accumulate, ptr_space, st, algo, dt_ms);

    const float* dB = (const float*)B;
    float* dC = (float*)C;
    const size_t b_elems = (size_t)ldb * (size_t)(b_layout == SPARTA_COL_MAJOR ? n_cols : A->cols);
    const size_t c_elems = (size_t)ldc * (size_t)(c_layout == SPARTA_COL_MAJOR ? n_cols : A->rows);
    if (ptr_space == SPARTA_PTR_HOST) {
        if (int rc = ensure_scratch(&A->d_B, &A->d_B_bytes, b_elems * sizeof(float))) return rc;
        if (int rc = ensure_scratch(&A->d_C, &A->d_C_bytes, c_elems * sizeof(float))) return rc;
        HIP_TRY(hipMemcpyAsync(A->d_B, B, b_elems * sizeof(float), hipMemcpyHostToDevice, st));
        if (accumulate) HIP_TRY(hipMemcpyAsync(A->d_C, C, c_elems * sizeof(float), hipMemcpyHostToDevice, st));
        else if (c_elems > 0) HIP_TRY(hipMemsetAsync(A->d_C, 0, c_elems * sizeof(float), st));
        dB = (const float*)A->d_B;
        dC = (float*)A->d_C;
    }

    struct BrmScope { sparta_vbs_t* a; ~BrmScope() { a->brm_ready = nullptr; a->brm_ld = 0; } } brm_scope{A};
    A->brm_ready = nullptr; A->brm_ld = 0;
    if (algo == SPARTA_SPMM_EXACT && A->ext_sparse && (A->n_sp_rows > 0 || A->u_steps_total > 0))
        return fail(SPARTA_ERR_UNSUPPORTED, "sparta_vbs_spmm: SPARTA_SPMM_EXACT needs the dense image of every block-row (handle made by sparta_vbs_create_from_csr)");
    if (dt_ms) HIP_TRY(hipEventRecord(A->ev0, st));
    if (algo == SPARTA_SPMM_EXACT) {
        if (int rc = ensure_legacy_image(A, st)) return rc;
        if (A->n_brows > 0) {
            launch_f32_exact((unsigned)A->n_brows, st, A->d_brows, A->d_jab, A->d_A, dB, dC, ldb, ldc, A->cols, (int)n_cols, (int)A->w,
                             (int)(b_layout == SPARTA_ROW_MAJOR), (int)(c_layout == SPARTA_ROW_MAJOR), (int)accumulate, shard_rows, shard_stride);
        }
    } else {
        const char* nv = std::getenv("SPARTA_NO_VEC");
        const bool novec = nv && nv[0] == '1';
        const int n_nt = (n_cols + kTN - 1) / kTN;
        const bool full_slabs = (n_cols % kTN) == 0;
        const int64_t ld_lim = ((int64_t)1 << 31) / (128 * 4) - 64;
        const bool ld_ok = (b_layout == SPARTA_ROW_MAJOR ? ldb * 32 : ldb * 128) < ((int64_t)1 << 29) - 4096 &&
                           (c_layout == SPARTA_ROW_MAJOR ? ldc * 64 : ldc * 128) < ((int64_t)1 << 29) - 4096;
        (void)ld_lim;
        const bool can_stream = A->n_workers > 0 && full_slabs && !novec && !force_generic() && ld_ok;
        const bool can_class = (A->w % kKP) == 0 && full_slabs && !novec && !force_generic();

        auto run_stream = [&](float* Cout, bool prof) -> int {
            const size_t slab = (size_t)A->n_slots * SK_SLOT_FLOATS;
            if (A->n_split > 0)
                if (int rc = ensure_scratch(&A->d_ws, &A->d_ws_bytes, slab * n_nt * sizeof(float))) return rc;
            if (shard_rows > 0)
                if (int rc = ensure_gathered_steps(A, shard_rows, st)) return rc;
            if (A->n_steps[1] > 0 || !(A->d_a_frag && b_layout == SPARTA_COL_MAJOR && shard_rows == 0))
                if (int rc = ensure_legacy_image(A, st)) return rc;
            StreamParams sp;
            sp.A = A->d_A; sp.B = dB; sp.C = Cout; sp.ws = (float*)A->d_ws;
            sp.ldb = ldb; sp.ldc = ldc; sp.cols = A->cols; sp.shard_rows = shard_rows; sp.shard_stride = shard_stride;
            sp.ws_slab_stride = (int64_t)slab; sp.accumulate = accumulate != 0; sp.c_row_major = c_layout == SPARTA_ROW_MAJOR;
            sp.N = n_cols; sp.w = (int32_t)A->w; sp.B_tail = nullptr;
            sp.clk = nullptr;
            sp.stagger = [] { const char* e = std::getenv("SPARTA_STAGGER"); return e ? atoi(e) : 0; }();
            if (A->n_steps[0] + A->n_steps[1] > 0) {
                if (prof) HIP_TRY(hipEventRecord(A->cev[0][0], st));
                if (A->has_tail && shard_rows == 0) {
                    if (int rc = ensure_scratch(&A->d_btail, &A->d_btail_bytes, (size_t)A->w * n_cols * sizeof(float))) return rc;
                    const int64_t row0 = ((A->cols - 1) / A->w) * A->w;
                    launch_tail_copy(st, dB, ldb, (int)(b_layout == SPARTA_ROW_MAJOR), row0, A->cols, (int)A->w, (int)n_cols, (float*)A->d_btail);
                    sp.B_tail = (const float*)A->d_btail;
                }
                const dim3 grid((unsigned)A->n_workers, (unsigned)n_nt);
                const int probe_ty = A->n_steps[1] >= A->n_steps[0] ? 1 : 0;
                for (int ty = 1; ty >= 0; ty--) {
                    if (A->n_steps[ty] == 0) continue;
                    sp.steps = shard_rows > 0 ? A->d_steps_g[ty] : A->d_steps[ty]; sp.worker_range = A->d_wrange[ty]; sp.c_nt = c_store_nt(A, ty, sp.C, sp.ldc, sp.c_row_major != 0);
                    sp.clk = (prof && ty == probe_ty) ? A->d_clk : nullptr;
                    if (ty == 0 && A->d_a_frag && b_layout == SPARTA_COL_MAJOR && shard_rows == 0) {
                        StreamParams sd = sp;
                        sd.A = A->d_a_frag;
                        const int cst = [] { const char* e = std::getenv("SPARTA_CSTAGE"); return e ? atoi(e) : -1; }();
                        const bool c_stage = c_layout == SPARTA_COL_MAJOR && (cst >= 0 ? cst != 0 : ring_tiles(A));
                        sd.c_nt = c_store_nt(A, ty, sd.C, sd.ldc, sd.c_row_major != 0, c_stage);
                        launch_f32_direct(c_stage, grid, st, sd);
                    } else launch_f32_stream(ty != 0, b_layout == SPARTA_ROW_MAJOR, shard_rows > 0, grid, st, sp);
                }
                if (prof) { HIP_TRY(hipEventRecord(A->cev[0][1], st)); A->class_ran[0] = true; }
            }
            const bool fix_launch = A->n_fix > 0 && !(accumulate && A->n_split == 0);
            const bool zero_launch = !A->zero_ranges.empty() && !accumulate;
            if (fix_launch || zero_launch) {
                if (prof) HIP_TRY(hipEventRecord(A->cev[1][0], st));
                if (fix_launch && A->n_big_fix > 0)
                    launch_fixup_group(dim3((unsigned)A->n_big_fix, (unsigned)n_nt, (unsigned)((A->max_tile_slots + kFixGroup - 1) / kFixGroup)), st, A->d_fix,
                                       A->d_big_fix, A->d_fix_slots, (float*)A->d_ws, (int64_t)slab);
                if (fix_launch)
                    launch_fixup(dim3((unsigned)A->n_fix, (unsigned)n_nt), st, A->d_fix, A->d_fix_slots, (const float*)A->d_ws, (int64_t)slab, Cout, ldc,
                                 (int)(c_layout == SPARTA_ROW_MAJOR), (int)(accumulate != 0));
                if (zero_launch) launch_zero_ranges(A, Cout, ldc, c_layout == SPARTA_ROW_MAJOR, n_cols, st);
                if (prof) { HIP_TRY(hipEventRecord(A->cev[1][1], st)); A->class_ran[1] = true; }
            }
            return SPARTA_OK;
        };
        auto run_class = [&](float* Cout, bool generic, bool prof) -> int {
            if (int rc = ensure_legacy_image(A, st)) return rc;
            SpmmParams p;
            p.jab = A->d_jab; p.A = A->d_A; p.B = dB; p.C = Cout; p.ldb = ldb; p.ldc = ldc; p.cols = A->cols;
            p.n_ntiles = n_nt; p.N = n_cols; p.w = (int32_t)A->w;
            p.b_row_major = b_layout == SPARTA_ROW_MAJOR; p.c_row_major = c_layout == SPARTA_ROW_MAJOR;
            p.accumulate = accumulate != 0;
            p.shard_rows = shard_rows; p.shard_stride = shard_stride;
            p.vec_ok = novec ? 0 : 1;
            for (int c = 3; c >= 0; c--) {
                if (A->n_tiles[c] == 0) continue;
                if (A->n_tiles[c] * (int64_t)p.n_ntiles > INT32_MAX) return fail(SPARTA_ERR_UNSUPPORTED, "sparta_vbs_spmm: grid too large");
                p.tiles = A->d_tiles[c]; p.n_tiles = (int32_t)A->n_tiles[c];
                p.clk = prof ? A->d_clk + 4 * c : nullptr;
                if (prof) HIP_TRY(hipEventRecord(A->cev[c][0], st));
                launch_f32_class(c, p.b_row_major != 0, generic, p, st);
                if (prof) { HIP_TRY(hipEventRecord(A->cev[c][1], st)); A->class_ran[c] = true; }
            }
            return SPARTA_OK;
        };

        int path = 3;
        const char* pe = std::getenv("SPARTA_PATH");
        const std::string forced = pe ? pe : "auto";
        if (forced == "stream") path = can_stream ? 1 : 3;
        else if (forced == "class") path = can_class ? 2 : 3;
        else if (forced == "generic") path = 3;
        else if (can_stream && can_class) {
            const int64_t key = ((int64_t)n_cols << 8) | (b_layout << 2) | (c_layout << 1) | (shard_rows > 0 ? 1 : 0);
            path = 0;
            for (const auto& kv : A->tuned) if (kv.first == key) path = kv.second;
            if (path == 0 && g_capturing) return capture_refusal("time its two product paths");
            if (path == 0) {
                if (int rc = ensure_scratch(&A->d_tune, &A->d_tune_bytes, c_elems * sizeof(float))) return rc;
                float best[3] = {0.0f, 1e30f, 1e30f};
                for (int cand = 1; cand <= 2; cand++) {
                    for (int rep = 0; rep < 4; rep++) {
                        HIP_TRY(hipEventRecord(A->tev0, st));
                        if (int rc = cand == 1 ? run_stream((float*)A->d_tune, false) : run_class((float*)A->d_tune, false, false)) return rc;
                        HIP_TRY(hipEventRecord(A->tev1, st));
                        HIP_TRY(hipEventSynchronize(A->tev1));
                        float ms = 0.0f;
                        HIP_TRY(hipEventElapsedTime(&ms, A->tev0, A->tev1));
                        if (rep > 0) best[cand] = std::min(best[cand], ms);
                    }
                }
                path = best[1] <= best[2] ? 1 : 2;
                A->tuned.emplace_back(key, path);
                A->tune_ms[0] = best[1]; A->tune_ms[1] = best[2];
            }
        } else if (can_stream) path = 1;
        else if (can_class) path = 2;

        const bool prof = A->class_timing;
        for (int c = 0; c < 4; c++) A->class_ran[c] = false;
        if (path == 1) { if (int rc = run_stream(dC, prof)) return rc; }
        else if (int rc = run_class(dC, path == 3, prof)) return rc;
        A->last_path = path;
        if (path == 1 && b_layout == SPARTA_COL_MAJOR && shard_rows == 0) drop_legacy_image(A);

        if (A->u_steps_total > 0) {
            const bool rec = prof && !A->class_ran[2];
            if (rec) HIP_TRY(hipEventRecord(A->cev[2][0], st));
            if (int rc = launch_union_tiles(A, dB, ldb, b_layout == SPARTA_ROW_MAJOR, shard_rows, shard_stride, n_cols, dC, ldc, c_layout == SPARTA_ROW_MAJOR,
// ... 644 lines not shown
```

### sparta_amd/csrc/vbs_device.hpp

```cpp
#pragma once
#include <hip/hip_runtime.h>

#include <algorithm>
#include <cstdint>
#include <cstdlib>
#include <cstring>
#include <new>
#include <string>
#include <type_traits>
#include <utility>
#include <memory>
#include <vector>

#include "host_core.hpp"

namespace sparta_dev {

typedef float f32x4 __attribute__((ext_vector_type(4)));
typedef float f32x4u __attribute__((ext_vector_type(4), aligned(4)));
typedef float f32x16 __attribute__((ext_vector_type(16)));
typedef unsigned int u32x4 __attribute__((ext_vector_type(4)));

constexpr int kThreads = 256;
constexpr int kTN = 128;
constexpr int kKP = 64;

struct TileDesc {
    int64_t a_off;
    int64_t jab_off;
    int32_t nb;
    int32_t h;
    int32_t c_row;
    int32_t mt_flags;
};
constexpr int32_t TILE_TAIL = 1 << 16;
static_assert(sizeof(TileDesc) == 32, "TileDesc must stay 32 bytes");

struct SpmmParams {
    const TileDesc* tiles;
    const int32_t* jab;
    const float* A;
    const float* B;
    float* C;
    int64_t ldb, ldc;
    int64_t cols;
    int32_t n_tiles, n_ntiles;
    int32_t N, w;
    int32_t b_row_major, c_row_major;
    int32_t accumulate, vec_ok;
    int64_t shard_stride;
    int64_t shard_rows;
    long long* clk;
};

constexpr int SK_KP = 32;
constexpr int SK_TM = 64;
constexpr int32_t STEP_FIRST = 1 << 16;
constexpr int32_t STEP_LAST = 1 << 17;
constexpr int32_t STEP_SPLIT = 1 << 18;
constexpr int32_t STEP_LO_ABSENT = 1 << 27;
constexpr int32_t STEP_HI_ABSENT = 1 << 28;
constexpr int32_t STEP_KPAIRS_SHIFT = 24;
constexpr int64_t kAFragSlice = 1040;
constexpr int32_t STEP_TAIL = 1 << 19;
constexpr int SK_SLOT_FLOATS = 32 * kThreads;

struct StepRec {
    int64_t a_off;
    int32_t b_row;
    int32_t h;
    int32_t c_row;
    int32_t mt_flags;
    int32_t slot;
    int32_t pad;
};
static_assert(sizeof(StepRec) == 32, "StepRec must stay 32 bytes");

struct FixRec {
    int32_t c_row, mt;
    int32_t slot_begin, n_slots;
};

struct StreamParams {
    const StepRec* steps;
    const int32_t* worker_range;
    const float* A;
    const float* B;
    const float* B_tail;
    float* C;
    float* ws;
    int64_t ldb, ldc, cols;
    int64_t shard_rows, shard_stride;
    int64_t ws_slab_stride;
    int32_t accumulate, c_row_major;
    int32_t N, w;
    long long* clk;
    int32_t c_nt;
    int32_t stagger;
    int32_t sub_ranges = 0;
};

constexpr int kHubGMax = 4;
struct HubStep {
    uint32_t a_lo, a_hi;
    int32_t b_row;
    int32_t shard;
    int32_t flags;
    int32_t slot;
    int32_t tile;
    int32_t pad;
};
static_assert(sizeof(HubStep) == 32, "HubStep must stay 32 bytes");
struct HubTile { int32_t c_row[4]; int32_t mt[4]; };
struct HubParams {
    const HubStep* steps;
    const int32_t* worker_range;
    const HubTile* tiles;
    const uint16_t* A;
    const uint16_t* B;
    const uint16_t* B_tail;
    float* C;
    float* ws;
    int64_t ldb, ldc;
    int64_t shard_stride;
    int64_t ws_slab_stride;
    int32_t accumulate, c_row_major, c_nt, w;
    int32_t n_slabs;
    int32_t n_workers;
    int32_t n_cols;
    int32_t pad0;
};

constexpr int kFixGroup = 16;

struct SparseParams {
    const int64_t* rowptr;
    const int32_t* col;
    const float* val;
    const int32_t* crow;
    const int32_t* list;
    int32_t n_list;
    const void* B;
    int64_t b_col_stride;
    int64_t shard_rows, shard_stride;
    int64_t ldb;
    float* out;
    int64_t ldo;
    int32_t out_is_c, accumulate, N;
    int32_t scalar_gather;
};

constexpr int kColresWaves = 16;
struct ColresLong { int32_t row, first, n, pad; };
constexpr int kColresMaxParts = 4, kColresMaxRanges = 4;
constexpr int kColresCellsPerPlane = 160 * 1024 / 4;
struct ColresPartDev {
    int32_t r0, rows;
    int32_t n_slices, n_long;
    int32_t plane;
    int32_t meta;
    int32_t dest;
    int32_t longs;
    int32_t all_store;
    int32_t pad;
// ... 70 lines not shown
struct SgdCfg { float lr, momentum, weight_decay, grad_scale; };
constexpr int kGradCtlUnroll = 4;
constexpr int64_t kGradCtlChunk = (int64_t)kThreads * 4 * kGradCtlUnroll;
constexpr int kGradCtlMaxGrid = 1024;
constexpr size_t kGradCtlBytes = 64 + 16 * (size_t)kGradCtlMaxGrid;
constexpr int kGradCtlCoef = 7, kGradCtlSkip = 8;
struct AdamCfg { float lr, beta1, beta2, eps, weight_decay, grad_scale, omb1, omb2, dk; int32_t decoupled; };
struct AdamArgs { float* W; const float* G; float* M; float* V; float* S; AdamCfg c; const uint32_t* R = nullptr; };

struct SpmmTBlock { int64_t off; int32_t h, r0; };
static_assert(sizeof(SpmmTBlock) == 16, "SpmmTBlock must stay 16 bytes");
struct SpmmTItem { int32_t jb, q0, l0, l1; };
struct SpmmTSrc { int64_t src, dst; int32_t h, pad0; int64_t pad1; };
static_assert(sizeof(SpmmTSrc) == 32, "SpmmTSrc must stay 32 bytes");
struct SpmmTParams {
    const SpmmTItem* items;
    const SpmmTBlock* blocks;
    const void* A;
    const void* X;
    float* Ct;
    int64_t ldx, ldo, cols;
    int32_t n_cols, w, accumulate, pad;
};
constexpr int kSpmmTSlab = 128;

#define HIP_TRY(expr)                                                                                   \
    do {                                                                                                \
        hipError_t e_ = (expr);                                                                         \
        if (e_ != hipSuccess)                                                                           \
            return sparta::fail(SPARTA_ERR_HIP, std::string(#expr) + ": " + hipGetErrorString(e_));     \
    } while (0)

struct DeviceGuard {
    int prev = -1;
    bool ok = true;
    explicit DeviceGuard(int dev) {
        if (hipGetDevice(&prev) != hipSuccess) { ok = false; return; }
        if (prev != dev && hipSetDevice(dev) != hipSuccess) ok = false;
    }
    ~DeviceGuard() {
        int cur = -1;
        if (prev >= 0 && hipGetDevice(&cur) == hipSuccess && cur != prev) (void)hipSetDevice(prev);
    }
};

}

struct sparta_vbs {
    int device = 0, dtype = SPARTA_F32;
    int64_t rows = 0, cols = 0, block_rows = 0, w = 0, nblocks = 0, nztot = 0;
    float* d_A = nullptr;
    int kp16 = 0;
    int32_t* d_jab = nullptr;
    sparta_dev::TileDesc* d_tiles[4] = {nullptr, nullptr, nullptr, nullptr};
    int64_t n_tiles[4] = {0, 0, 0, 0};
    int64_t n_real_tiles[4] = {0, 0, 0, 0};
    sparta_dev::BlockRowDesc* d_brows = nullptr;
    int64_t n_brows = 0;
    int64_t exec_area = 0;
    int64_t a_bytes = 0;
    hipEvent_t ev0 = nullptr, ev1 = nullptr;
    hipEvent_t cev[4][2] = {{nullptr, nullptr}, {nullptr, nullptr}, {nullptr, nullptr}, {nullptr, nullptr}};
    bool class_timing = false;
    bool class_ran[4] = {false, false, false, false};
    sparta_dev::StepRec* d_steps[2] = {nullptr, nullptr};
    std::vector<sparta_dev::StepRec> h_steps[2];
    sparta_dev::StepRec* d_steps_g[2] = {nullptr, nullptr};
    int64_t g_shard_rows = 0;
    int32_t* d_wrange[2] = {nullptr, nullptr};
    sparta_dev::FixRec* d_fix = nullptr;
    std::vector<std::pair<int64_t, int64_t>> zero_ranges;
    int32_t* d_fix_slots = nullptr;
    int64_t n_steps[2] = {0, 0};
    int32_t n_workers = 0, n_fix = 0, n_split = 0, n_slots = 0;
    int32_t max_tile_slots = 0;
    int32_t* d_big_fix = nullptr;
    int32_t n_big_fix = 0;
    void* d_ws = nullptr;
    size_t d_ws_bytes = 0;
    int64_t n_plan_tiles[2] = {0, 0};
    bool tiles_row_aligned[2] = {true, true};
    bool wide16 = false;
    float* d_a_frag = nullptr;
    bool legacy_dropped = false;
    sparta_dev::HubStep* d_hub_steps = nullptr;
    sparta_dev::HubStep* d_hub_steps_g = nullptr;
    std::vector<sparta_dev::HubStep> h_hub_steps;
    sparta_dev::HubTile* d_hub_tiles = nullptr;
    int32_t* d_hub_wrange = nullptr;
    uint16_t* d_hub_A = nullptr;
    int hub_g = 0, hub_workers = 0;
    int64_t n_hub_steps = 0, hub_area = 0, hub_union_area = 0, n_hub_tiles = 0, n_hub_groups = 0, hub_chunks = 0, hub_segments = 0;
    bool has_tail = false;
    void* d_btail = nullptr;
    size_t d_btail_bytes = 0;
    int last_path = 0;
    std::vector<std::pair<int64_t, int>> tuned;
    float tune_ms[2] = {0.0f, 0.0f};
    void* d_tune = nullptr;
    size_t d_tune_bytes = 0;
    void* d_B16 = nullptr;
    size_t d_B16_bytes = 0;
    void* d_Bt = nullptr;
    size_t d_Bt_bytes = 0;
    void* d_Ct = nullptr;
    size_t d_Ct_bytes = 0;
    long long* d_clk = nullptr;
    hipEvent_t tev0 = nullptr, tev1 = nullptr;
    int64_t n_sp_rows = 0, n_sp_short = 0, n_sp_long = 0, sp_nnz = 0;
    bool ext_sparse = false;
    int64_t* d_sp_rowptr = nullptr;
    int32_t* d_sp_col = nullptr;
    float* d_sp_val = nullptr;
    int32_t* d_sp_crow = nullptr;
    int32_t* d_sp_list = nullptr;
    void* d_sp_segs = nullptr;
    void* d_sp_long = nullptr;
    int64_t n_sp_segs = 0;
    int32_t* d_sp_stream_begin = nullptr;
    int64_t sp_max_stream = 0;
    void* d_sp_part = nullptr;
    size_t d_sp_part_bytes = 0;
    void* d_cr_col = nullptr;
    void* d_cr_val = nullptr;
    int32_t* d_cr_meta = nullptr;
    int32_t* d_cr_dest = nullptr;
    void* d_cr_longs = nullptr;
    int32_t cr_slices = 0, cr_long = 0, cr_plane = 0, cr_lmax = 0;
    int32_t cr_parts = 0, cr_ranges = 0, cr_span = 0;
    int32_t cr_krange[sparta_dev::kColresMaxRanges + 1] = {0, 0, 0, 0, 0};
    void* d_cr_parts = nullptr;
    void* d_cr_mode = nullptr;
    bool cr_unit = false;
    struct ColresSmall {
        void* col = nullptr; void* val = nullptr; int32_t* meta = nullptr; int32_t* dest = nullptr; void* longs = nullptr; void* parts = nullptr;
        int32_t slices = 0, plane = 0, n_parts = 0;
    } cr_small;
    bool last_colres_small = false;
    int64_t cr_entries = 0;
    int last_colres_nc = 0;
    sparta_dev::UnionRec* d_u_rec[sparta_dev::kUnionTypes] = {nullptr, nullptr, nullptr, nullptr};
    int32_t* d_u_ids[sparta_dev::kUnionTypes] = {nullptr, nullptr, nullptr, nullptr};
    void* d_u_a[sparta_dev::kUnionTypes] = {nullptr, nullptr, nullptr, nullptr};
    int32_t* d_u_wrange[sparta_dev::kUnionTypes] = {nullptr, nullptr, nullptr, nullptr};
    void* d_u_tail[sparta_dev::kUnionTypes] = {nullptr, nullptr, nullptr, nullptr};
    int32_t u_workers[sparta_dev::kUnionTypes] = {0, 0, 0, 0};
    int64_t u_steps[sparta_dev::kUnionTypes] = {0, 0, 0, 0}, u_tiles[sparta_dev::kUnionTypes] = {0, 0, 0, 0};
    int64_t u_tiles_h[2] = {0, 0}, u_steps_h[2] = {0, 0}, u_steps_total = 0;
    int64_t u_area = 0, u_cols = 0, u_nnz = 0;
    int64_t u_tail_nnz = 0, u_rows = 0;
    int64_t u_exec_area = 0;
    const void* brm_ready = nullptr;
    int64_t brm_ld = 0;
    void* d_Brm = nullptr;
    size_t d_Brm_bytes = 0;
    const void* prepared_brm = nullptr;
    int64_t prepared_ld = 0;
    void* d_B = nullptr;
    size_t d_B_bytes = 0;
    void* d_C = nullptr;
    size_t d_C_bytes = 0;
    sparta_dev::SddmmItem* d_sd_items = nullptr;
    int64_t n_sd_items = -1;
    void* d_sd_ws = nullptr;
    size_t d_sd_ws_bytes = 0;
    void* d_sd_h16 = nullptr;
    size_t d_sd_h16_bytes = 0;
    int32_t create_flags = 0;
    sparta_dev::UpdSlice* d_upd_map[2] = {nullptr, nullptr};
    int64_t upd_base[2] = {0, 0};
    sparta_dev::UpdSlice* d_upd_hub = nullptr;
    int64_t n_upd_hub = 0;
    void* d_upd_ws = nullptr;
    size_t d_upd_ws_bytes = 0;
    int64_t upd_cover[2] = {0, 0};
    int32_t step_last_fused = -1, step_last_launches = 0;
    sparta_dev::SpmmTItem* d_t_items = nullptr;
    sparta_dev::SpmmTBlock* d_t_blocks = nullptr;
    int64_t n_t_items = 0;
    uint16_t* d_t_A = nullptr;
    sparta_dev::SpmmTSrc* d_t_src = nullptr;
    int64_t n_t_src = 0;
    void* d_t_ws = nullptr;
    size_t d_t_ws_bytes = 0;
    void* d_t_h16 = nullptr;
    size_t d_t_h16_bytes = 0;
};

namespace sparta_dev {

void launch_f32_class(int cls, bool b_row_major, bool generic, const SpmmParams& p, hipStream_t st);
void launch_f32_exact(unsigned n_brows, hipStream_t st, const BlockRowDesc* rows, const int32_t* jab, const float* A, const float* B, float* C,
                      int64_t ldb, int64_t ldc, int64_t cols, int N, int w, int b_row_major, int c_row_major, int accumulate, int64_t shard_rows,
                      int64_t shard_stride);
void launch_f32_stream(bool mi2, bool b_row_major, bool gathered, dim3 grid, hipStream_t st, const StreamParams& sp);
void launch_f32_direct(bool c_stage, dim3 grid, hipStream_t st, const StreamParams& sp);
void launch_f32_legacy_from_frag(hipStream_t st, const StepRec* steps, int64_t n_steps, const float* a_frag, float* A);
void launch_fixup_group(dim3 grid, hipStream_t st, const FixRec* fix, const int32_t* big, const int32_t* fix_slots, float* ws_all, int64_t ws_slab_stride);
void launch_fixup(dim3 grid, hipStream_t st, const FixRec* fix, const int32_t* fix_slots, const float* ws_all, int64_t ws_slab_stride, float* C, int64_t ldc,
                  int c_row_major, int accumulate);
void launch_tail_copy(hipStream_t st, const float* B, int64_t ldb, int b_row_major, int64_t row0, int64_t cols, int w, int N, float* B_tail);
void launch_zero_rows(dim3 grid, hipStream_t st, float* C, int64_t ldc, int c_row_major, int64_t row0, int64_t nrows, int N);
void launch_h16_stream(int kp, bool mi2, bool bf16, bool gathered, bool c_stage, bool wide, dim3 grid, hipStream_t st, const StreamParams& sp);
void launch_h16_slab256(bool bf16, dim3 grid, hipStream_t st, const StreamParams& sp);
bool h16_uses_direct_kernel(int kp, bool mi2);
void launch_h16_quad(int kp, bool bf16, bool gathered, dim3 grid, hipStream_t st, const StreamParams& sp);
void launch_h16_hub(int variant, bool bf16, bool gathered, hipStream_t st, const HubParams& p);
int hub_variant_kp(int variant);
int hub_variant_g(int variant);
void launch_tail_copy_h16(hipStream_t st, const uint16_t* B, int64_t ldb, int64_t row0, int64_t cols, int w, int N, uint16_t* B_tail);
void launch_convert_h16(bool bf16, hipStream_t st, const float* src, int64_t ld_in, int64_t rows, int64_t n_cols, uint16_t* dst, int64_t ld_out);
void launch_col_tail_merge(hipStream_t st, const float* Ct, int64_t rows, float* C, int64_t ldc, int c_row_major, int col0, int n_t, int accumulate);
void launch_sparse_kernels(int vec, int bk, const SparseParams& q, unsigned gy, hipStream_t st, const int32_t* list, int64_t n_short, const SpSegRec* segs,
                           int64_t n_segs, const SpLongRec* longs, int64_t n_long, float* part, const int32_t* stream_begin = nullptr, int64_t max_stream = 0);
void launch_b_to_row_major(bool is16, unsigned grid, hipStream_t st, const void* B, int64_t ldb, int64_t shard_rows, int64_t shard_stride, int64_t rows, int N,
                           void* out, int64_t ld_out);
void launch_union_f32(unsigned n_slabs, hipStream_t st, const UnionParams& p);
void launch_union_h16(bool bf16, unsigned n_slabs, hipStream_t st, const UnionParams& p);
void launch_sddmm(int dtype, unsigned n_items, hipStream_t st, const SddmmParams& p);
void launch_update_copy(hipStream_t st, const float* mab, int64_t n, float* A);
void launch_update_f32_frag(hipStream_t st, StepRec* steps, int64_t n_steps, const float* mab, float* a_frag, float* A_out);
void launch_update_h16(bool bf16, bool hub, int tms, int kp, hipStream_t st, const UpdSlice* map, int64_t n_slices, const float* mab, uint16_t* dst);
void launch_update_h16_t(bool bf16, hipStream_t st, const SpmmTSrc* src, int64_t n_blocks, int w, const float* mab, uint16_t* dst);
void launch_sgd_step(hipStream_t st, int64_t n, float* W, const float* G, float* M, const SgdCfg& cfg, const uint32_t* R);
void launch_sgd_f32_frag(hipStream_t st, StepRec* steps, int64_t n_steps, float* W, const float* G, float* M, const SgdCfg& cfg, const uint32_t* R, float* a_frag, float* A_out);
void launch_sgd_h16(bool bf16, int tms, int kp, hipStream_t st, const UpdSlice* map, int64_t n_slices, float* W, const float* G, float* M, const SgdCfg& cfg, const uint32_t* R, uint16_t* dst);
void launch_adam_tick(hipStream_t st, const AdamArgs& a);
void launch_adam_step(hipStream_t st, int64_t n, const AdamArgs& a);
void launch_adam_f32_frag(hipStream_t st, StepRec* steps, int64_t n_steps, const AdamArgs& a, float* a_frag, float* A_out);
void launch_adam_h16(bool bf16, int tms, int kp, hipStream_t st, const UpdSlice* map, int64_t n_slices, const AdamArgs& a, uint16_t* dst);
void launch_spmm_t(int dtype, unsigned n_items, hipStream_t st, const SpmmTParams& p);
int launch_colres(int nc, const ColresParams& p, size_t lds_bytes, hipStream_t st);
int colres_max_slices(int nc);
void launch_pack_blocks(dim3 grid, hipStream_t st, const void* src, const int32_t* ids, void* dst, int64_t block_vec);
void launch_grad_stats(hipStream_t st, const float* G, int64_t n, void* R, bool accumulate);
void launch_grad_ctl_finish(hipStream_t st, void* R, float max_norm, float growth_factor, float backoff_factor, int32_t growth_interval);

struct StreamPlanIn {
    int64_t cols, w, br0, br1, jab_lo, mab_lo;
    const int64_t* row_part; const int64_t* nzcount; const int64_t* jab; const float* mab;
    int32_t dtype, device;
    const uint8_t* skip;
    bool updatable = false;
};
struct StreamPlanHost {
    std::vector<StepRec> steps[2];
    std::vector<int32_t> wrange[2];
    std::vector<FixRec> fix;
    std::vector<std::pair<int64_t, int64_t>> zero_ranges;
    std::vector<int32_t> fix_slots;
    std::vector<uint16_t> a16_steps[2];
    int n_workers = 0, n_split = 0;
    int plan_aligned[2] = {0, 0};
    bool wide16 = false;
    bool window_plan = false;
    int64_t kp = SK_KP;
    int64_t n_plan_tiles[2] = {0, 0};
    bool tiles_row_aligned[2] = {true, true};
    std::vector<float> a_frag;
    std::vector<HubStep> hub_steps;
    std::vector<HubTile> hub_tiles;
    std::vector<int32_t> hub_wrange;
    std::unique_ptr<uint16_t[]> hub_a16;
    size_t hub_a16_elems = 0;
    int hub_g = 0;
    int hub_workers = 0;
    int64_t n_hub_steps = 0, hub_area = 0, hub_union_area = 0;
    int64_t n_hub_tiles = 0, n_hub_groups = 0, hub_chunks = 0, hub_segments = 0;
    std::vector<UpdSlice> upd_map[2];
    std::vector<UpdSlice> upd_hub;
};
struct UnionDevPlan {
    std::vector<UnionRec> rec[kUnionTypes];
    std::vector<int32_t> ids[kUnionTypes];
    std::vector<float> a[kUnionTypes];
    std::vector<uint16_t> a16[kUnionTypes];
    std::vector<int32_t> wrange[kUnionTypes];
    std::vector<uint32_t> tail[kUnionTypes];
    int32_t n_workers[kUnionTypes] = {0, 0, 0, 0};
    int64_t n_steps[kUnionTypes] = {0, 0, 0, 0}, n_tiles[kUnionTypes] = {0, 0, 0, 0};
    int32_t type_rows[kUnionTypes] = {0, 0, 0, 0};
    int64_t tiles_by_height[2] = {0, 0}, steps_by_height[2] = {0, 0};
    int64_t area = 0, cols = 0, rows = 0;
};
int build_union_plan(const sparta::UnionPlanHost& U, int max_workers, UnionDevPlan& P, int dtype = SPARTA_F32, int n_cus = 0);
void union_plan_host_apply(const UnionDevPlan& P, const float* x, double* y);

constexpr int64_t kZeroRangeRows = 2048;
int build_stream_plans(const StreamPlanIn& in, StreamPlanHost& P);
struct SpmmTIndexHost {
    std::vector<SpmmTBlock> blocks;
    std::vector<SpmmTItem> items;
    std::vector<SpmmTSrc> src;
    int64_t image_elems = 0;
    int64_t cols_with_blocks = 0, max_list = 0;
};
int build_spmm_t_index(int64_t cols, int64_t w, int64_t br0, int64_t br1, const int64_t* row_part, const int64_t* nzcount, const int64_t* jab, int64_t jab_lo, bool h16,
                       SpmmTIndexHost& T);
void pack_spmm_t_block(const float* blk, int64_t h, int64_t w, bool bf16, uint16_t* dst);
uint16_t to_h16(float v, bool bf16);

}
```

### sparta_amd/csrc/vbs_kernel_common.hpp

```cpp
#pragma once
#include "vbs_device.hpp"

namespace sparta_dev {

__host__ __device__ inline uint32_t frag_seq_mask(uint32_t nonempty) {
    uint32_t seq = 0;
    for (int m = 0; m < 8; m++) {
        const uint32_t nib = (nonempty >> (4 * m)) & 15u, r = (uint32_t)(m & 3);
        seq |= (((nib >> r) | (nib << (4 - r))) & 15u) << (4 * m);
    }
    return seq;
}
__host__ __device__ inline int frag_position(uint32_t nonempty, int k) {
    const uint32_t seq = frag_seq_mask(nonempty);
    const int m = k >> 2, s = 4 * m + (((k & 3) - m) & 3);
    const uint32_t before = (1u << s) - 1u;
    const int c = ((nonempty >> k) & 1u) ? __builtin_popcount(seq & before) : __builtin_popcount(seq) + __builtin_popcount(~seq & before);
    return (c >> 1) + 16 * (c & 1);
}
__host__ __device__ inline int frag_pairs(uint32_t nonempty) {
    const int nk = __builtin_popcount(nonempty), n_mfma = nk + 1 >= 2 ? (nk + 1) / 2 : 1;
    return (n_mfma + 1) / 2;
}

}

#ifdef __HIP__
namespace sparta_dev {

#ifdef SPARTA_TIMELINE
#define TL_STEPS 64
#define TL_FIRST 16
#define TL_STAMP(k) do { if (tl_on) asm volatile("s_memtime %0" : "=s"(tl[k])); } while (0)
#else
#define TL_STAMP(k) do { } while (0)
#endif


template <int I, int N, class F>
__device__ __forceinline__ void static_for(F&& f) {
    if constexpr (I < N) { f(std::integral_constant<int, I>{}); static_for<I + 1, N>(f); }
}

__device__ __forceinline__ void clock_probe(long long* clk, int slot) {
    if (clk != nullptr && blockIdx.x == 0 && blockIdx.y == 0 && threadIdx.x == 0) {
        clk[slot] = (long long)__builtin_readcyclecounter();
        clk[slot + 1] = (long long)wall_clock64();
    }
}

template <int MF>
struct Acc;
template <>
struct Acc<32> { typedef f32x16 type; };
template <>
struct Acc<16> { typedef f32x4 type; };

__device__ __forceinline__ int32_t sk_field(int vrec0, int vrec1, int s, int f) {
    const int ln = ((s & 7) << 3) + f;
    const int32_t x0 = __builtin_amdgcn_readlane(vrec0, ln), x1 = __builtin_amdgcn_readlane(vrec1, ln);
    return ((s >> 3) & 1) ? x1 : x0;
}

__device__ __forceinline__ void sk_store_tile(const f32x16& acc0, const f32x16& acc1, int mt, int c_row, int col0, float* C,
                                              int64_t ldc, int c_row_major, int accumulate, int lm, int g) {
#pragma unroll
    for (int mi = 0; mi < 2; mi++) {
        const int row = mi * 32 + lm;
        if (row >= mt) continue;
#pragma unroll
        for (int r = 0; r < 16; r++) {
            const int col = col0 + (r & 3) + 8 * (r >> 2) + 4 * g;
            float* dst = c_row_major ? C + (int64_t)(c_row + row) * ldc + col : C + (int64_t)(c_row + row) + (int64_t)col * ldc;
            float v = mi == 0 ? acc0[r] : acc1[r];
            if (accumulate) v += *dst;
            *dst = v;
        }
    }
}

constexpr int kCRingStride = 65;
constexpr int kCRingFloats = 32 * kCRingStride;
struct CRing {
    float* ring;
    int32_t win_base = 0, pend_lo = 0, pend_hi = 0;

    __device__ __forceinline__ void flush_block(const StreamParams& p, int n0, int lm, int g, uint32_t voffC, int32_t b, int32_t lo, int32_t hi) {
        float* cbase = p.C + (int64_t)b + (int64_t)n0 * p.ldc;
        const __amdgpu_buffer_rsrc_t rC = __builtin_amdgcn_make_buffer_rsrc(cbase, 0, 0x7ffffff0, 0x00020000);
        const uint32_t jstep = (uint32_t)p.ldc * 4u;
        const int32_t row = b + lm;
        if (row >= lo && row < hi) {
            float v[16];
#pragma unroll
            for (int q = 0; q < 16; q++) v[q] = ring[((q & 3) + 8 * (q >> 2) + 4 * g) * kCRingStride + (row & 63)];
            if (p.accumulate) {
                uint32_t old[16];
#pragma unroll
                for (int q = 0; q < 16; q++) old[q] = __builtin_amdgcn_raw_buffer_load_b32(rC, voffC, (uint32_t)((q & 3) + 8 * (q >> 2)) * jstep, 0);
#pragma unroll
                for (int q = 0; q < 16; q++) v[q] += __uint_as_float(old[q]);
            }
            if (p.c_nt) {
#pragma unroll
                for (int q = 0; q < 16; q++) __builtin_amdgcn_raw_buffer_store_b32(__float_as_uint(v[q]), rC, voffC, (uint32_t)((q & 3) + 8 * (q >> 2)) * jstep, 2);
// ... 27 lines not shown
```

### sparta_amd/csrc/vbs_plan.cpp

```cpp
#include <cstdio>
#include <queue>

#include "vbs_kernel_common.hpp"

namespace sparta_dev {

uint16_t to_h16(float v, bool bf16) {
    if (bf16) {
        uint32_t u;
        std::memcpy(&u, &v, 4);
        if ((u & 0x7fffffffu) > 0x7f800000u) return (uint16_t)((u >> 16) | 0x40);
        return (uint16_t)((u + 0x7fffu + ((u >> 16) & 1u)) >> 16);
    }
    const _Float16 h = (_Float16)v;
    uint16_t o;
    std::memcpy(&o, &h, 2);
    return o;
}


int build_stream_plans(const StreamPlanIn& in, StreamPlanHost& P) {
    using sparta::fail;
    const int64_t cols = in.cols, w = in.w, br0 = in.br0, br1 = in.br1, jab_lo = in.jab_lo, mab_lo = in.mab_lo;
    const int64_t* row_part = in.row_part; const int64_t* nzcount = in.nzcount; const int64_t* jab = in.jab; const float* mab = in.mab;
// ... 25 lines not shown
        if (const char* e = std::getenv("SPARTA_STREAM_INTERLEAVE")) interleave_mode = atoi(e);
        interleave = interleave_mode != 0;
        double slot_bias = 0.0;
        if (const char* e = std::getenv("SPARTA_SLOT_BIAS")) slot_bias = std::max(-0.9, std::min(0.9, atof(e)));
        int align_mode = -1;
        if (const char* e = std::getenv("SPARTA_STREAM_ALIGN")) align_mode = atoi(e) ? 1 : 0;
        if ((int64_t)cols > INT32_MAX)
            return fail(SPARTA_ERR_UNSUPPORTED, "sparta_vbs_create: matrix too large for 32-bit step indexing");
        struct PairSrc { int64_t a_off_hi; int32_t h_hi, rows_hi, lo_present, hi_present; };
        std::vector<PairSrc> pair_tab(1);
        std::vector<uint8_t> pair_role((size_t)(br1 - br0), 0);
        std::vector<int64_t> jo_of((size_t)(br1 - br0) + 1, 0), mo_of((size_t)(br1 - br0) + 1, 0);
        for (int64_t ib = br0; ib < br1; ib++) {
            jo_of[(size_t)(ib - br0) + 1] = jo_of[(size_t)(ib - br0)] + nzcount[ib];
            mo_of[(size_t)(ib - br0) + 1] = mo_of[(size_t)(ib - br0)] + nzcount[ib] * (row_part[ib + 1] - row_part[ib]) * w;
        }
        const bool pair_on = h16 && [] { const char* e = std::getenv("SPARTA_H16_PAIR"); return !e || atoi(e) != 0; }();
        if (pair_on) {
            for (int64_t ib = br0; ib + 1 < br1; ib++) {
                const int64_t h1 = row_part[ib + 1] - row_part[ib], h2 = row_part[ib + 2] - row_part[ib + 1];
                const bool s1 = in.skip && in.skip[ib - br0], s2 = in.skip && in.skip[ib + 1 - br0];
                if (!s1 && !s2 && h1 == 32 && h2 >= 1 && h2 <= 32 && nzcount[ib] > 0 && nzcount[ib + 1] > 0) {
                    pair_role[(size_t)(ib - br0)] = 1; pair_role[(size_t)(ib + 1 - br0)] = 2;
                    ib++;
                }
            }
        }
        std::vector<uint8_t> hub_role((size_t)(br1 - br0), 0);
        struct HubGroup { int64_t ib[kHubGMax]; int n; };
        std::vector<HubGroup> hub_groups;
        int hub_G = 4;
        {
            const char* e0 = std::getenv("SPARTA_HUB");
            const bool hub_on = h16 && kp == 64 && !(e0 && atoi(e0) == 0) && [] { const char* e = std::getenv("SPARTA_H16_PATH"); return !(e && e[0] == 'l'); }();
            if (const char* e = std::getenv("SPARTA_HUB_G")) hub_G = atoi(e) == 2 ? 2 : 4;
            int64_t hub_min = 64;
            if (const char* e = std::getenv("SPARTA_HUB_MIN_STEPS")) hub_min = std::max<int64_t>(1, atoll(e));
            double tau = 0.5;
            if (const char* e = std::getenv("SPARTA_HUB_TAU")) tau = atof(e);
            const int window = 48;
            if (hub_on) {
                std::vector<int64_t> cand;
                for (int64_t ib = br0; ib < br1; ib++) {
                    const int64_t h = row_part[ib + 1] - row_part[ib], nb = nzcount[ib];
                    if ((in.skip && in.skip[ib - br0]) || pair_role[(size_t)(ib - br0)] != 0) continue;
                    if (h > 32 && h <= 64 && nb * (w / 64) >= hub_min) cand.push_back(ib);
                }
                std::stable_sort(cand.begin(), cand.end(), [&](int64_t a, int64_t b) { return nzcount[a] > nzcount[b]; });
                auto jaccard = [&](int64_t a, int64_t b) {
                    const int64_t* pa = jab + jab_lo + jo_of[(size_t)(a - br0)]; const int64_t na = nzcount[a];
                    const int64_t* pb = jab + jab_lo + jo_of[(size_t)(b - br0)]; const int64_t nb2 = nzcount[b];
                    int64_t i = 0, j = 0, both = 0;
                    while (i < na && j < nb2) { if (pa[i] == pb[j]) { both++; i++; j++; } else if (pa[i] < pb[j]) i++; else j++; }
                    return (double)both / (double)(na + nb2 - both);
                };
                std::vector<uint8_t> used(cand.size(), 0);
                int64_t hub_steps_total = 0;
                for (size_t q = 0; q < cand.size(); q++) {
                    if (used[q]) continue;
                    used[q] = 1;
                    HubGroup g{{cand[q], 0, 0, 0}, 1};
                    std::vector<std::pair<double, size_t>> sim;
                    int seen = 0;
                    for (size_t r = q + 1; r < cand.size() && seen < window; r++) {
                        if (used[r]) continue;
                        seen++;
                        if ((double)nzcount[cand[r]] < tau * (double)nzcount[cand[q]]) break;
                        const double js = jaccard(cand[q], cand[r]);
                        if (js >= tau) sim.emplace_back(-js, r);
                    }
                    std::sort(sim.begin(), sim.end());
                    for (size_t k = 0; k < sim.size() && g.n < hub_G; k++) { g.ib[g.n++] = cand[sim[k].second]; used[sim[k].second] = 1; }
                    if (g.n < 2) continue;
                    std::sort(g.ib, g.ib + g.n);
                    hub_groups.push_back(g);
                    hub_steps_total += nzcount[cand[q]] * (w / 64);
                }
                int64_t hub_min_total = 8 * (int64_t)n_workers;
                if (const char* e = std::getenv("SPARTA_HUB_MIN_TOTAL")) hub_min_total = atoll(e);
                if (hub_steps_total < hub_min_total) hub_groups.clear();
                for (const HubGroup& g : hub_groups) for (int u = 0; u < g.n; u++) hub_role[(size_t)(g.ib[u] - br0)] = 1;
            }
        }
        for (int ty = 0; ty < 2; ty++) {
            std::vector<StepRec>& st = steps[ty];
            struct TileSpan { int64_t first, last; int32_t c_row, mt; };
            std::vector<TileSpan> spans;
            std::vector<int64_t> cum;
            int64_t total_cost = 0;
            {
                int64_t jo2 = 0, mo2 = 0;
                const int64_t row0 = row_part[br0];
                for (int64_t ib = br0; ib < br1; ib++) {
                    const int64_t h = row_part[ib + 1] - row_part[ib];
                    const int64_t nb = nzcount[ib];
                    const bool skipped = in.skip && in.skip[ib - br0];
#ifdef SPARTA_TIMELINE
                    const int dbg_probe = [] { const char* e = std::getenv("SPARTA_DBG_PROBE"); return e ? atoi(e) : 0; }();
#else
                    constexpr int dbg_probe = 0;
#endif
                    const bool zero_range = nb == 0 && !skipped && h >= kZeroRangeRows;
                    if (zero_range && ty == 0) P.zero_ranges.emplace_back(row_part[ib] - row0, h);
                    const uint8_t role = pair_role[(size_t)(ib - br0)];
                    if (role == 1 && ty == 1) {
                        const int64_t h2 = row_part[ib + 2] - row_part[ib + 1], nb2 = nzcount[ib + 1];
                        const int64_t jo_b = jo_of[(size_t)(ib + 1 - br0)], mo_b = mo_of[(size_t)(ib + 1 - br0)];
                        const int32_t c_row = (int32_t)(row_part[ib] - row0), mt = (int32_t)(32 + h2);
                        TileSpan sp{(int64_t)st.size(), 0, c_row, mt};
                        int64_t a = 0, b2 = 0;
                        while (a < nb || b2 < nb2) {
                            const int64_t ja = a < nb ? jab[jab_lo + jo2 + a] : INT64_MAX, jb2 = b2 < nb2 ? jab[jab_lo + jo_b + b2] : INT64_MAX;
                            const int64_t jb = std::min(ja, jb2);
                            const bool lo = ja == jb, hi = jb2 == jb;
                            for (int64_t ks = 0; ks < w; ks += kp) {
                                StepRec r;
                                r.a_off = lo ? mo2 + (a * w + ks) * h : 0;
                                r.b_row = (int32_t)(jb * w + ks);
                                r.h = (int32_t)h;
                                r.c_row = c_row;
                                r.mt_flags = mt | (lo ? 0 : STEP_LO_ABSENT) | (hi ? 0 : STEP_HI_ABSENT);
                                if ((jb + 1) * w > cols) { r.mt_flags |= STEP_TAIL; r.b_row = (int32_t)ks; }
                                r.slot = -1;
                                r.pad = (int32_t)pair_tab.size();
                                pair_tab.push_back(PairSrc{hi ? mo_b + (b2 * w + ks) * h2 : 0, (int32_t)h2, (int32_t)h2, lo ? 1 : 0, hi ? 1 : 0});
                                cum.push_back(total_cost);
                                total_cost += c2;
                                st.push_back(r);
                            }
                            a += lo; b2 += hi;
                        }
                        total_cost += ct;
                        sp.last = (int64_t)st.size() - 1;
                        st[(size_t)sp.first].mt_flags |= STEP_FIRST;
                        st[(size_t)sp.last].mt_flags |= STEP_LAST;
                        spans.push_back(sp);
                    }
                    if (role != 0 || hub_role[(size_t)(ib - br0)]) { jo2 += nb; mo2 += nb * h * w; continue; }
                    for (int64_t r0 = 0; r0 < h && !skipped && !zero_range; r0 += SK_TM) {
                        const int32_t mt = (int32_t)std::min<int64_t>(SK_TM, h - r0);
                        if ((mt > 32 ? 1 : 0) != ty) continue;
                        const int32_t c_row = (int32_t)(row_part[ib] - row0 + r0);
                        if (nb == 0) {
                            fix.push_back(FixRec{c_row, mt, 0, 0});
                            continue;
                        }
                        TileSpan sp{(int64_t)st.size(), 0, c_row, mt};
                        for (int64_t b = 0; b < nb; b++) {
                            const int64_t jb = jab[jab_lo + jo2 + b];
                            for (int64_t ks = 0; ks < w; ks += kp) {
                                StepRec r;
                                r.a_off = mo2 + r0 + (b * w + ks) * h;
                                r.b_row = (int32_t)(jb * w + ks);
                                r.h = (int32_t)h;
                                r.c_row = c_row;
                                r.mt_flags = mt;
                                if ((jb + 1) * w > cols) { r.mt_flags |= STEP_TAIL; r.b_row = (int32_t)ks; }
                                r.slot = -1;
                                r.pad = 0;
                                if (dbg_probe) {
                                    if (dbg_probe & 1) r.b_row = (int32_t)ks;
                                    if ((dbg_probe & 2) && h16) r.a_off = (ks) * h;
                                    if ((dbg_probe & 2) && !h16) r.a_off = r0 + (b * w + ks) * h;
                                    if (dbg_probe & 4) r.c_row = 0;
                                }
                                cum.push_back(total_cost);
                                total_cost += ty ? c2 : c1;
                                st.push_back(r);
                            }
                        }
                        total_cost += ct;
                        sp.last = (int64_t)st.size() - 1;
                        st[(size_t)sp.first].mt_flags |= STEP_FIRST;
                        st[(size_t)sp.last].mt_flags |= STEP_LAST;
                        spans.push_back(sp);
                    }
                    jo2 += nb;
                    mo2 += nb * h * w;
                }
            }
            if ((int64_t)st.size() > INT32_MAX - 64)
                return fail(SPARTA_ERR_UNSUPPORTED, "sparta_vbs_create: matrix too large for 32-bit step indexing");
            const int64_t S = (int64_t)st.size();
            P.n_plan_tiles[ty] = (int64_t)spans.size();
            for (const TileSpan& sp : spans) if (sp.c_row % 32 != 0) P.tiles_row_aligned[ty] = false;
            if (S == 0) continue;
            const bool ring_like = ty == 0 && !P.tiles_row_aligned[ty] && S < 6 * (int64_t)spans.size() &&
                                   [] { const char* e = std::getenv("SPARTA_CSTAGE"); return !e || atoi(e) != 0; }();
            const bool wide = h16 && kp == 32 && ty == 0 && !ring_like && [] { const char* e = std::getenv("SPARTA_H16_WIDE"); return e && atoi(e) != 0; }() &&
                              [] { const char* e = std::getenv("SPARTA_H16_PATH"); return !(e && e[0] == 'l'); }();
            if (ty == 0) P.wide16 = wide;
            const int n_workers = wide ? 2 * P.n_workers : P.n_workers;
            cum.push_back(total_cost);
            const int per_x = n_workers / 8;
            std::vector<int64_t> bnd((size_t)n_workers + 1, S);
            bnd[0] = 0;
            int64_t win_cols = 0;
            if (const char* e = std::getenv("SPARTA_TILE_WINDOW_COLS")) win_cols = std::max(0, atoi(e));
            const bool win_plan = h16 && ty == 1 && !wide && win_cols >= w && S >= 4 * (int64_t)n_workers;
            std::vector<int32_t> sp_tile, sp_seq, tile_pieces;
            std::vector<TileSpan> tile_spans;
            if (win_plan) {
                int64_t min_steps = 64;
                if (const char* e = std::getenv("SPARTA_TILE_WINDOW_MIN")) min_steps = std::max(1, atoi(e));
                struct Piece { int64_t first, last, win; int32_t tile, seq; };
                std::vector<Piece> pieces;
                auto win_of = [&](int64_t q) { const StepRec& r = st[(size_t)q]; return ((r.mt_flags & STEP_TAIL) ? cols - 1 : (int64_t)r.b_row) / win_cols; };
                tile_spans = spans;
                tile_pieces.assign(spans.size(), 0);
                for (size_t t = 0; t < spans.size(); t++) {
                    int64_t a = spans[t].first;
                    int32_t seq = 0;
                    while (a <= spans[t].last) {
                        int64_t b = a, wcur = win_of(a);
                        while (b < spans[t].last) {
                            const int64_t wn = win_of(b + 1);
                            if (wn != wcur) { if (b - a + 1 >= min_steps) break; wcur = wn; }
                            b++;
                        }
                        if (spans[t].last - b < min_steps) b = spans[t].last;
                        pieces.push_back(Piece{a, b, win_of(a), (int32_t)t, seq++});
                        a = b + 1;
                    }
                    tile_pieces[t] = seq;
                }
                std::stable_sort(pieces.begin(), pieces.end(), [](const Piece& x, const Piece& y) { return x.win < y.win; });
                std::vector<std::vector<size_t>> mine((size_t)n_workers);
                {
                    typedef std::pair<int64_t, int> LW;
                    std::priority_queue<LW, std::vector<LW>, std::greater<LW>> heap;
                    for (int pos = 0; pos < n_workers; pos++) heap.push(LW(0, pos));
                    for (size_t i = 0; i < pieces.size(); i++) {
                        LW lw = heap.top();
                        heap.pop();
                        mine[(size_t)lw.second].push_back(i);
                        lw.first += (pieces[i].last - pieces[i].first + 1) * (int64_t)c2 + ct;
                        heap.push(lw);
                    }
                }
                std::vector<StepRec> ns;
                std::vector<TileSpan> nspans;
                ns.reserve(st.size());
                for (int pos = 0; pos < n_workers; pos++) {
                    bnd[(size_t)pos] = (int64_t)ns.size();
                    for (size_t i : mine[(size_t)pos]) {
                        const Piece& pc = pieces[i];
                        TileSpan sp = tile_spans[(size_t)pc.tile];
                        sp.first = (int64_t)ns.size();
                        ns.insert(ns.end(), st.begin() + pc.first, st.begin() + pc.last + 1);
                        sp.last = (int64_t)ns.size() - 1;
// ... 119 lines not shown
            for (int pos = 0; pos < n_workers; pos++) {
                const int64_t s0 = bnd[(size_t)pos], s1 = bnd[(size_t)pos + 1];
                if (s0 >= s1) continue;
                while (ti < spans.size() && spans[ti].last < s0) ti++;
                for (size_t t = ti; t < spans.size() && spans[t].first < s1; t++) {
                    const int64_t a = std::max(spans[t].first, s0), b = std::min(spans[t].last, s1 - 1);
                    const bool whole = a == spans[t].first && b == spans[t].last && (!win_plan || tile_pieces[(size_t)sp_tile[t]] == 1);
                    st[(size_t)a].mt_flags |= STEP_FIRST;
                    st[(size_t)b].mt_flags |= STEP_LAST;
                    if (!whole && win_plan) {
                        const int32_t slot = slot_base + n_win_slots++;
                        st[(size_t)b].mt_flags |= STEP_SPLIT;
                        st[(size_t)b].slot = slot;
                        tile_slots[(size_t)sp_tile[t]].push_back(std::make_pair(sp_seq[t], slot));
                    } else if (!whole) {
                        const int32_t slot = (int32_t)fix_slots.size();
                        st[(size_t)b].mt_flags |= STEP_SPLIT;
                        st[(size_t)b].slot = slot;
                        if (a == spans[t].first) {
                            fix.push_back(FixRec{spans[t].c_row, spans[t].mt, (int32_t)fix_slots.size(), 0});
                            n_split++;
                        }
                        fix_slots.push_back(slot);
                        fix.back().n_slots++;
                    }
                }
            }
            if (win_plan)
                for (size_t t = 0; t < tile_slots.size(); t++) {
                    if (tile_slots[t].empty()) continue;
                    std::sort(tile_slots[t].begin(), tile_slots[t].end());
                    fix.push_back(FixRec{tile_spans[t].c_row, tile_spans[t].mt, (int32_t)fix_slots.size(), (int32_t)tile_slots[t].size()});
                    for (const auto& ps : tile_slots[t]) fix_slots.push_back(ps.second);
                    n_split++;
                }
            if (h16) {
                const size_t slice = (size_t)(ty ? 64 : 32) * (size_t)kp;
                const int64_t tms = ty ? 64 : 32;
                const size_t base = ty ? a16_steps[0].size() : 0;
                a16_steps[ty].assign((size_t)S * slice, 0);
                const bool bf = dtype == SPARTA_BF16;
                uint16_t* all = a16_steps[ty].data();
                if (in.updatable) P.upd_map[ty].assign((size_t)S, UpdSlice{0, 0, 0, 0, 0, 0});
                sparta::parallel_for_dynamic(S, 256, [&](int64_t lo, int64_t hi, int) {
                    for (int64_t q = lo; q < hi; q++) {
                        StepRec& r = st[(size_t)q];
                        uint16_t* dst = all + (size_t)q * slice;
                        if (r.pad != 0) {
                            const PairSrc& ps = pair_tab[(size_t)r.pad];
                            for (int64_t kk = 0; kk < kp; kk++) {
                                uint16_t* d2 = dst + (kk >> 3) * tms * 8 + (kk & 7);
                                if (ps.lo_present) {
                                    const float* colp = mab + mab_lo + r.a_off + kk * (int64_t)r.h;
                                    for (int64_t rr = 0; rr < 32; rr++) d2[rr * 8] = to_h16(colp[rr], bf);
                                }
                                if (ps.hi_present) {
                                    const float* colp = mab + mab_lo + ps.a_off_hi + kk * (int64_t)ps.h_hi;
                                    for (int64_t rr = 0; rr < ps.rows_hi; rr++) d2[(32 + rr) * 8] = to_h16(colp[rr], bf);
                                }
                            }
                            if (in.updatable)
                                P.upd_map[ty][(size_t)q] = UpdSlice{ps.lo_present ? r.a_off : 0, ps.hi_present ? ps.a_off_hi : 0, r.h, ps.h_hi, ps.lo_present ? 32 : 0, ps.hi_present ? ps.rows_hi : 0};
                            r.pad = 0;
                            r.a_off = (int64_t)(base + (size_t)q * slice);
                            continue;
                        }
                        const float* blk = mab + mab_lo + r.a_off;
                        const int64_t hh = r.h, mt = r.mt_flags & 0xffff;
                        for (int64_t kk = 0; kk < kp; kk++) {
                            const float* colp = blk + kk * hh;
                            uint16_t* d2 = dst + (kk >> 3) * tms * 8 + (kk & 7);
                            for (int64_t rr = 0; rr < mt; rr++) d2[rr * 8] = to_h16(colp[rr], bf);
                        }
                        if (in.updatable) P.upd_map[ty][(size_t)q] = UpdSlice{r.a_off, 0, r.h, 0, (int32_t)mt, 0};
                        r.a_off = (int64_t)(base + (size_t)q * slice);
                    }
                });
            }
            {
                const char* de = std::getenv("SPARTA_F32_PLAN");
                const bool off = de && std::strcmp(de, "legacy") == 0;
                int64_t one_tile_area = 0;
                for (int64_t q = 0; q < S; q++) one_tile_area += (int64_t)(st[(size_t)q].mt_flags & 0xffff) * SK_KP;
                if (!off && ty == 0 && !h16 && S <= ((int64_t)2 << 20) && S * kAFragSlice <= 4 * std::max<int64_t>(one_tile_area, 1) + (1 << 20)) {
                    std::vector<float>& af = P.a_frag;
                    af.assign(((size_t)S + 4) * (size_t)kAFragSlice, 0.0f);
                    sparta::parallel_for_dynamic(S, 256, [&](int64_t lo, int64_t hi, int) {
                        for (int64_t q = lo; q < hi; q++) {
                            StepRec& r = st[(size_t)q];
                            const float* blk = mab + mab_lo + r.a_off;
                            const int64_t hh = r.h, mt = r.mt_flags & 0xffff;
                            uint32_t nonempty = 0;
                            for (int k = 0; k < 32; k++) {
                                bool any = false;
                                for (int64_t m = 0; m < mt && !any; m++) any = blk[(int64_t)k * hh + m] != 0.0f;
                                nonempty |= (uint32_t)any << k;
                            }
                            uint8_t pos[32];
                            for (int k = 0; k < 32; k++) pos[k] = (uint8_t)frag_position(nonempty, k);
                            float* dst = af.data() + (size_t)q * (size_t)kAFragSlice;
                            std::memcpy(dst, pos, 32);
                            float* frag = dst + 16;
                            for (int k = 0; k < 32; k++) {
                                if (!((nonempty >> k) & 1u)) continue;
                                const int kp = pos[k], g = kp >> 4, j = (kp & 15) >> 2, e = kp & 3;
                                for (int64_t m = 0; m < mt; m++) frag[((j * 2 + g) * 32 + m) * 4 + e] = blk[(int64_t)k * hh + m];
                            }
                            const int pairs = frag_pairs(nonempty);
                            r.mt_flags = (r.mt_flags & ~(7 << STEP_KPAIRS_SHIFT)) | ((pairs - 1) << STEP_KPAIRS_SHIFT);
                        }
                    });
                    for (size_t q = (size_t)S; q < (size_t)S + 4; q++) {
                        uint8_t pos[32];
                        for (int k = 0; k < 32; k++) pos[k] = (uint8_t)k;
                        std::memcpy(af.data() + q * (size_t)kAFragSlice, pos, 32);
                    }
                }
            }
        }
        if (!hub_groups.empty()) {
            const int G = hub_G;
            const int64_t block_cols = (cols - 1) / w + 1, spb = w / 64;
            const int hub_workers = P.n_workers;
            int64_t n_ranges = 16;
            struct UStep { int32_t jb; int8_t mask; int32_t bidx[kHubGMax]; };
            std::vector<std::vector<UStep>> un(hub_groups.size());
            sparta::parallel_for_dynamic((int64_t)hub_groups.size(), 1, [&](int64_t lo, int64_t hi, int) {
                for (int64_t gi = lo; gi < hi; gi++) {
                    const HubGroup& g = hub_groups[(size_t)gi];
                    int64_t pos[kHubGMax] = {0, 0, 0, 0};
                    std::vector<UStep>& u = un[(size_t)gi];
                    for (;;) {
                        int64_t jb = INT64_MAX;
                        for (int k = 0; k < g.n; k++) if (pos[k] < nzcount[g.ib[k]]) jb = std::min(jb, jab[jab_lo + jo_of[(size_t)(g.ib[k] - br0)] + pos[k]]);
                        if (jb == INT64_MAX) break;
                        UStep x{(int32_t)jb, 0, {-1, -1, -1, -1}};
                        for (int k = 0; k < g.n; k++)
                            if (pos[k] < nzcount[g.ib[k]] && jab[jab_lo + jo_of[(size_t)(g.ib[k] - br0)] + pos[k]] == jb) { x.mask |= (int8_t)(1 << k); x.bidx[k] = (int32_t)pos[k]; pos[k]++; }
                        u.push_back(x);
                    }
                }
            });
            int64_t total_union = 0;
            for (const auto& u : un) total_union += (int64_t)u.size();
            const int64_t S_all = total_union * spb;
            auto unit_sizes = [&](int64_t C, std::vector<int64_t>& cost) {
                cost.assign((size_t)(C * (int64_t)hub_groups.size()), 0);
                for (size_t gi = 0; gi < hub_groups.size(); gi++) {
                    size_t c0 = 0;
                    for (int64_t c = 0; c < C; c++) {
                        const int64_t jb_end = (c + 1) * block_cols / C;
                        size_t c1 = c0;
                        while (c1 < un[gi].size() && un[gi][c1].jb < jb_end) c1++;
                        cost[(size_t)(c * (int64_t)hub_groups.size()) + gi] = (int64_t)(c1 - c0) * spb;
                        c0 = c1;
                    }
                }
            };
            auto aligned_cut = [&](const std::vector<int64_t>& cost, std::vector<int64_t>* bnd_out) -> int64_t {
                const double T = (double)S_all / (double)hub_workers;
                int64_t worst = 0, load = 0, at = 0;
                int wk = 0;
                if (bnd_out) { bnd_out->assign((size_t)hub_workers + 1, S_all); (*bnd_out)[0] = 0; }
                for (size_t q = 0; q < cost.size(); q++) {
                    if (cost[q] == 0) continue;
                    if (load > 0 && (double)load + 0.5 * (double)cost[q] > T && wk + 1 < hub_workers) {
                        worst = std::max(worst, load); load = 0; wk++;
// ... 249 lines not shown
```

### sparta_amd/device.py

```python
import ctypes as C
import numpy as np

from . import _lib
from ._lib import lib, check

_i64p = C.POINTER(C.c_int64)
_f32p = C.POINTER(C.c_float)


def _ctl_ptr(ctl, device):
    if ctl is None:
        return None
    R = getattr(ctl, "R", ctl)
    if not (R.is_cuda and R.device.index == device and R.is_contiguous() and R.numel() * R.element_size() >= _lib.GRAD_CTL_BYTES):
        raise ValueError("ctl must be a GradCtl, or a contiguous tensor of GRAD_CTL_BYTES = %d bytes, on device %d" % (_lib.GRAD_CTL_BYTES, device))
    return C.c_void_p(R.data_ptr())


def device_count():
    return int(lib.sparta_device_count())


class ValuesRecord:
    _autograd_values = None
# ... 17 lines not shown
        mab = np.ascontiguousarray(vbmat.mab, np.float32)
        b0, b1 = (0, vbmat.block_rows) if block_row_range is None else block_row_range
        check(lib.sparta_vbs_create_range_ex(C.byref(self.h), vbmat.rows, vbmat.cols, vbmat.block_rows, vbmat.block_col_size,
                                             rp.ctypes.data_as(_i64p), nz.ctypes.data_as(_i64p), jab.ctypes.data_as(_i64p),
                                             mab.ctypes.data_as(_f32p), int(b0), int(b1), int(dtype), self.device,
                                             (_lib.CREATE_UPDATABLE if updatable else 0) | (_lib.CREATE_TRANSPOSE if transposable else 0)))
        info = self.info()
        self.rows, self.cols = info["rows"], info["cols"]

    @classmethod
    def from_csr(cls, cmat, grouping, col_block_size, row_block_size=0, force_fixed_size=False, device=0, dtype=_lib.F32):
        self = cls(None, device=device, dtype=dtype)
        g = np.ascontiguousarray(grouping, np.int64)
        if g.shape != (cmat.rows,):
            raise ValueError("grouping must have one entry per row")
        rp = np.ascontiguousarray(cmat.rowptr, np.int64)
        ci = np.ascontiguousarray(cmat.colidx, np.int32)
        vals = None if cmat.vals is None else np.ascontiguousarray(cmat.vals, np.float32)
        check(lib.sparta_vbs_create_from_csr(C.byref(self.h), cmat.rows, cmat.cols, rp.ctypes.data_as(_i64p), ci.ctypes.data_as(C.POINTER(C.c_int32)),
                                             None if vals is None else vals.ctypes.data_as(_f32p), g.ctypes.data_as(_i64p), int(col_block_size),
                                             int(row_block_size), int(bool(force_fixed_size)), int(dtype), self.device))
        info = self.info()
        self.rows, self.cols = info["rows"], info["cols"]
        return self

    @staticmethod
    def plan_stats(cmat, grouping, col_block_size, row_block_size=0, force_fixed_size=False, dtype=_lib.F32):
        g = np.ascontiguousarray(grouping, np.int64)
        if g.shape != (cmat.rows,):
            raise ValueError("grouping must have one entry per row")
        rp = np.ascontiguousarray(cmat.rowptr, np.int64)
        ci = np.ascontiguousarray(cmat.colidx, np.int32)
        vals = None if cmat.vals is None else np.ascontiguousarray(cmat.vals, np.float32)
        st = np.zeros(8, np.int64)
        check(lib.sparta_vbs_plan_stats(cmat.rows, cmat.cols, rp.ctypes.data_as(_i64p), ci.ctypes.data_as(C.POINTER(C.c_int32)),
                                        None if vals is None else vals.ctypes.data_as(_f32p), g.ctypes.data_as(_i64p), int(col_block_size),
                                        int(row_block_size), int(bool(force_fixed_size)), int(dtype), st.ctypes.data_as(_i64p)))
        keys = ["tile_blocks", "tile_area", "mfma_steps", "sparse_nnz", "sparse_rows", "block_rows", "rows", "union_steps"]
        return {k: int(st[i]) for i, k in enumerate(keys)}

    @staticmethod
    def predict_cost(cmat, grouping, col_block_size, row_block_size=0, force_fixed_size=False, dtype=_lib.F32, n_cols=128):
        st = DeviceVBS.plan_stats(cmat, grouping, col_block_size, row_block_size, force_fixed_size, dtype)
        esz = 4.0 if dtype == _lib.F32 else 2.0
        t_tiles = 2.0 * st["tile_area"] * n_cols / ((100e12 if dtype == _lib.F32 else 220e12))
        rate = 9.5e12 if (cmat.cols >= 4 * 65536 and st["sparse_nnz"] >= (4 << 20)) else 5.9e12
        t_sparse = st["sparse_nnz"] * (n_cols * esz + 8.0) / rate + st["sparse_rows"] * n_cols * 4.0 / 5.9e12
        st["ms_tiles"], st["ms_sparse"] = t_tiles * 1e3, t_sparse * 1e3
        st["ms"] = (t_tiles + t_sparse) * 1e3
        return st

    @classmethod
    def transposed_of(cls, vbmat, device=0, dtype=_lib.F32):
        self = cls(None, device=device, dtype=dtype)
        rp = np.ascontiguousarray(vbmat.row_part, np.int64)
        nz = np.ascontiguousarray(vbmat.nzcount, np.int64)
        jab = np.ascontiguousarray(vbmat.jab, np.int64)
        mab = np.ascontiguousarray(vbmat.mab, np.float32)
        check(lib.sparta_vbs_create_transposed(C.byref(self.h), vbmat.rows, vbmat.cols, vbmat.block_rows, vbmat.block_col_size,
                                               rp.ctypes.data_as(_i64p), nz.ctypes.data_as(_i64p), jab.ctypes.data_as(_i64p),
                                               mab.ctypes.data_as(_f32p), int(dtype), self.device))
        info = self.info()
        self.rows, self.cols = info["rows"], info["cols"]
        return self

    def spmm_BA_host(self, B, M, C_out, accumulate=True):
        B = np.ascontiguousarray(B, np.float32).reshape(-1)
        if not (isinstance(C_out, np.ndarray) and C_out.dtype == np.float32 and C_out.flags.c_contiguous):
            raise ValueError("C must be a contiguous float32 numpy array (it is written in place)")
        if B.size < M * self.cols or C_out.size < M * self.rows:
            raise ValueError("B or C too small")
        dt = C.c_float(0)
        check(lib.sparta_vbs_spmm_ba(self.h, B.ctypes.data_as(C.c_void_p), int(M), int(M), C_out.ctypes.data_as(C.c_void_p), int(M),
                                     int(bool(accumulate)), _lib.PTR_HOST, None, C.byref(dt)))
        return dt.value

    def info(self):
        a = np.zeros(16, np.int64)
        check(lib.sparta_vbs_info(self.h, a.ctypes.data_as(_i64p)))
        keys = ["rows", "cols", "block_rows", "block_col_size", "nblocks", "nztot", "tiles16", "tiles32", "tiles64",
                "sparse_rows", "a_bytes", "exec_area", "stream_steps", "stream_workers", "split_tiles", "last_path"]
        return {k: int(a[i]) for i, k in enumerate(keys)}

    def sparse_info(self):
        a = np.zeros(4, np.int64)
        check(lib.sparta_vbs_sparse_info(self.h, a.ctypes.data_as(_i64p)))
        return {"rows": int(a[0]), "nnz": int(a[1]), "short_rows": int(a[2]), "hub_rows": int(a[3])}

    def colres_info(self):
        a = np.zeros(12, np.int64)
        check(lib.sparta_vbs_colres_info(self.h, a.ctypes.data_as(_i64p)))
        return {"slices": int(a[0]), "entries": int(a[1]), "long_rows": int(a[2]), "plane": int(a[3]), "lmax": int(a[4]), "nc": int(a[5]), "nnz": int(a[6]), "unit": int(a[7]),
                "parts": int(a[8]), "ranges": int(a[9]), "small_parts": int(a[10]), "used_small": int(a[11])}

    def union_info(self):
        a = np.zeros(12, np.int64)
        check(lib.sparta_vbs_union_info(self.h, a.ctypes.data_as(_i64p)))
        keys = ["tiles32", "tiles64", "steps32", "steps64", "area", "list_entries", "nnz", "workers", "rows", "tail_nnz", "exec_area", "row_tile"]
        return {k: int(a[i]) for i, k in enumerate(keys)}

    def hub_info(self):
        a = np.zeros(10, np.int64)
        check(lib.sparta_vbs_hub_info(self.h, a.ctypes.data_as(_i64p)))
        keys = ["steps", "tiles", "groups", "tiles_per_group", "stored_area", "union_area", "workers", "chunks", "segments"]
        return {k: int(a[i]) for i, k in enumerate(keys)}

    def spmm_host(self, B, n_cols, C_out, accumulate=True, algo=_lib.SPMM_MFMA, b_layout=_lib.COL_MAJOR,
                  c_layout=_lib.COL_MAJOR):
        B = np.ascontiguousarray(B, np.float32).reshape(-1)
        if not (isinstance(C_out, np.ndarray) and C_out.dtype == np.float32 and C_out.flags.c_contiguous):
            raise ValueError("C must be a contiguous float32 numpy array (it is written in place)")
        ldb = self.cols if b_layout == _lib.COL_MAJOR else n_cols
        ldc = self.rows if c_layout == _lib.COL_MAJOR else n_cols
        if B.size < self.cols * n_cols or C_out.size < self.rows * n_cols:
            raise ValueError("B or C too small")
        dt = C.c_float(0)
        check(lib.sparta_vbs_spmm(self.h, B.ctypes.data_as(C.c_void_p), ldb, b_layout, int(n_cols),
                                  C_out.ctypes.data_as(C.c_void_p), ldc, c_layout, int(bool(accumulate)), _lib.PTR_HOST, None,
                                  int(algo), C.byref(dt)))
        return dt.value

    def spmm(self, B, C_out, n_cols, accumulate=False, algo=_lib.SPMM_MFMA, b_layout=_lib.COL_MAJOR, c_layout=_lib.COL_MAJOR,
             ldb=None, ldc=None, timed=False, stream=None):
        import torch
        want_b = {_lib.F32: torch.float32, _lib.F16: torch.float16, _lib.BF16: torch.bfloat16}[self.dtype]
        if not (B.is_cuda and C_out.is_cuda and B.dtype == want_b and C_out.dtype == torch.float32):
            raise ValueError("B must be a %s tensor and C a float32 tensor, both on the GPU" % want_b)
        if B.device.index != self.device or C_out.device.index != self.device:
            raise ValueError("B and C must live on device %d" % self.device)
        ldb = (self.cols if b_layout == _lib.COL_MAJOR else n_cols) if ldb is None else ldb
        ldc = (self.rows if c_layout == _lib.COL_MAJOR else n_cols) if ldc is None else ldc
        need_b = ldb * (n_cols if b_layout == _lib.COL_MAJOR else self.cols)
        need_c = ldc * (n_cols if c_layout == _lib.COL_MAJOR else self.rows)
        if B.numel() < need_b or C_out.numel() < need_c or not B.is_contiguous() or not C_out.is_contiguous():
            raise ValueError("B or C too small / not contiguous for the stated leading dimensions")
        st = torch.cuda.current_stream(self.device).cuda_stream if stream is None else stream
        dt = C.c_float(0)
        check(lib.sparta_vbs_spmm(self.h, C.c_void_p(B.data_ptr()), int(ldb), b_layout, int(n_cols), C.c_void_p(C_out.data_ptr()),
                                  int(ldc), c_layout, int(bool(accumulate)), _lib.PTR_DEVICE, C.c_void_p(st), int(algo),
                                  C.byref(dt) if timed else None))
        return dt.value if timed else None

    def _nztot(self):
        if getattr(self, "_nztot_cached", None) is None:
            self._nztot_cached = self.info()["nztot"]
        return self._nztot_cached

    def sddmm(self, X, Y, G_out, k, accumulate=False, ldx=None, ldy=None, timed=False, stream=None):
        import torch
        want = {_lib.F32: torch.float32, _lib.F16: torch.float16, _lib.BF16: torch.bfloat16}[self.dtype]
        if not (X.is_cuda and Y.is_cuda and G_out.is_cuda and X.dtype == want and Y.dtype == want and G_out.dtype == torch.float32):
            raise ValueError("X and Y must be %s tensors and G a float32 tensor, all on the GPU" % want)
        if X.device.index != self.device or Y.device.index != self.device or G_out.device.index != self.device:
            raise ValueError("X, Y and G must live on device %d" % self.device)
        k = int(k)
        if k <= 0:
            raise ValueError("k must be > 0")
        ldx = self.rows if ldx is None else int(ldx)
        ldy = self.cols if ldy is None else int(ldy)
        nztot = self._nztot()
        if (X.numel() < ldx * (k - 1) + self.rows or Y.numel() < ldy * (k - 1) + self.cols or G_out.numel() < nztot
                or not X.is_contiguous() or not Y.is_contiguous() or not G_out.is_contiguous()):
            raise ValueError("X, Y or G too small / not contiguous for the stated leading dimensions")
        st = torch.cuda.current_stream(self.device).cuda_stream if stream is None else stream
        dt = C.c_float(0)
        check(lib.sparta_vbs_sddmm(self.h, C.c_void_p(X.data_ptr()), ldx, C.c_void_p(Y.data_ptr()), ldy, k,
# ... 266 lines not shown
```

Before: 25050 GFLOP/s.

## Add packed f32 SpMM path that compacts nonempty k-groups into shared MFMA steps

Adds a packed fp32 stream plan in which the nonempty 4-column groups of several blocks in a tile are packed into shared 32-wide k slots. Each packed step carries a per-slot B-row table, so the kernel gathers the matching B rows and runs only the MFMA pairs that are occupied. A new kernel consumes this layout, and the planner's cost weights are adjusted to reflect packed tile costs. The aim is to skip MFMA work and A/B traffic on all-zero column groups. The cost is an extra indirection per slot, uncoalesced B gathers, and considerably more plan-building complexity.

Measured after the change: 27190 GFLOP/s, median of 6. +8.5%, better.

```diff
diff --git a/include/sparta_amd.h b/include/sparta_amd.h
--- a/include/sparta_amd.h
+++ b/include/sparta_amd.h
@@ -230,6 +230,8 @@
                              const int64_t* nzcount, const int64_t* jab, const float* mab, int64_t block_row_begin, int64_t block_row_end,
                              const float* x, double* y, int64_t* info_out);
 int sparta_frag_positions(const uint8_t* nonempty, uint8_t* pos, int32_t* pairs);
+int sparta_f32_pack_blocks(int32_t n_blocks, const uint8_t* group_masks, int32_t* step_of_block, int32_t* slot0_of_block, int32_t* n_steps);
+int sparta_vbs_packed_info(const sparta_vbs_t* A, int64_t* info_out);
 
 typedef struct sparta_b sparta_b_t;
 int sparta_vbs_prepare_b(sparta_vbs_t* A, const void* B, int64_t ldb, int64_t shard_rows, int64_t shard_stride, int32_t n_cols, void* stream,
diff --git a/sparta_amd/__init__.py b/sparta_amd/__init__.py
--- a/sparta_amd/__init__.py
+++ b/sparta_amd/__init__.py
@@ -8,7 +8,7 @@
 from .optim import VbsSGD, VbsAdamW
 from .gradctl import GradCtl
 
-KERNEL_REV = "r5i"
+KERNEL_REV = "r5j"
 
 cublas_fixed_blocks_multiply = vbs_multiply
 cublas_blockmat_batched = vbs_multiply
diff --git a/sparta_amd/_lib.py b/sparta_amd/_lib.py
--- a/sparta_amd/_lib.py
+++ b/sparta_amd/_lib.py
@@ -36,6 +36,7 @@
     "sparta_vbs_spmm_t", "sparta_spmm_t_host_check",
     "sparta_vbs_sgd_step", "sparta_vbs_step_info", "sparta_vbs_adam_step",
     "sparta_grad_stats", "sparta_grad_ctl_finish", "sparta_vbs_sgd_step_ctl", "sparta_vbs_adam_step_ctl",
+    "sparta_f32_pack_blocks", "sparta_vbs_packed_info",
 ]
 
 
@@ -140,6 +141,8 @@
     L.sparta_vbs_spmm_t.argtypes = [vp, vp, C.c_int64, C.c_int32, f32p, C.c_int64, C.c_int32, C.c_int32, vp, f32p]
     L.sparta_spmm_t_host_check.argtypes = [C.c_int64, C.c_int64, C.c_int64, C.c_int64, i64p, i64p, i64p, f32p, C.c_int64, C.c_int64, f32p, C.POINTER(C.c_double), i64p]
     L.sparta_frag_positions.argtypes = [C.POINTER(C.c_uint8), C.POINTER(C.c_uint8), i32p]
+    L.sparta_f32_pack_blocks.argtypes = [C.c_int32, C.POINTER(C.c_uint8), i32p, i32p, i32p]
+    L.sparta_vbs_packed_info.argtypes = [vp, i64p]
     L.sparta_vbs_create_from_csr.argtypes = [C.POINTER(vp), C.c_int64, C.c_int64, i64p, i32p, f32p, i64p, C.c_int64, C.c_int64, C.c_int32, C.c_int32, C.c_int32]
     L.sparta_vbs_plan_stats.argtypes = [C.c_int64, C.c_int64, i64p, i32p, f32p, i64p, C.c_int64, C.c_int64, C.c_int32, C.c_int32, i64p]
     L.sparta_vbs_prepare_b.argtypes = [vp, vp, C.c_int64, C.c_int64, C.c_int64, C.c_int32, vp, C.POINTER(vp)]
diff --git a/sparta_amd/csrc/k_f32_packed.hip b/sparta_amd/csrc/k_f32_packed.hip
--- /dev/null
+++ b/sparta_amd/csrc/k_f32_packed.hip
@@ -0,0 +1,260 @@
+#include "vbs_kernel_common.hpp"
+
+using namespace sparta_dev;
+
+namespace {
+
+template <bool CSTAGE, bool TAIL = true>
+__global__ __launch_bounds__(kThreads, 2) void vbs_spmm_f32_packed_kernel(const StreamParams p) {
+    constexpr int TN = kTN, LDBW = 36;
+    constexpr int WSTAGE = 32 * LDBW;
+    __shared__ __attribute__((aligned(16))) float lds[4 * 2 * WSTAGE + (CSTAGE ? 4 * kCRingFloats : 0)];
+    const int tid = threadIdx.x;
+    const int lane = tid & 63, wave = tid >> 6;
+    const int lm = lane & 31, g = lane >> 5;
+    const int n0 = blockIdx.y * TN;
+    const int s_begin = p.worker_range[2 * blockIdx.x];
+    const int n = p.worker_range[2 * blockIdx.x + 1] - s_begin;
+    if (n <= 0) return;
+    clock_probe(p.clk, 0);
+    float* ws = p.ws + (int64_t)blockIdx.y * p.ws_slab_stride;
+
+    const int32_t* srec = reinterpret_cast<const int32_t*>(p.steps + s_begin);
+    int vwin = srec[lane];
+    int vnext = 0;
+#define field(pos, f) __builtin_amdgcn_readlane(vwin, 8 * (pos) + (f))
+    enum { F_AOFF_LO = 0, F_AOFF_HI = 1, F_BROW = 2, F_H = 3, F_CROW = 4, F_FLAGS = 5, F_SLOT = 6, F_SHARD = 7 };
+
+    const int bc = lane >> 3, bs = lane & 7;
+    const int64_t ld_t = (int64_t)p.w;
+    const uint32_t voffB = (uint32_t)(((32 * wave + bc) * p.ldb) * 4);
+    const uint32_t voffBt = (uint32_t)(((n0 + 32 * wave + bc) * ld_t) * 4);
+    const uint32_t qstepB = (uint32_t)(8 * p.ldb * 4), qstepBt = (uint32_t)(8 * ld_t * 4);
+    const uint32_t voffA = (uint32_t)((g * 32 + lm) * 16);
+    const uint32_t voffT = (uint32_t)(bs * 4);
+    const uint32_t voffC = p.c_row_major ? (uint32_t)((lm * p.ldc + 32 * wave + 4 * g) * 4) : (uint32_t)((lm + (32 * wave + 4 * g) * p.ldc) * 4);
+    char* const ldsw = reinterpret_cast<char*>(lds) + wave * (2 * WSTAGE * 4);
+    const uint32_t lwB = (uint32_t)((bc * LDBW + 2 * bs) * 4);
+    const uint32_t lrB = (uint32_t)((lm * LDBW + 16 * g) * 4);
+    const __amdgpu_buffer_rsrc_t rBslab = __builtin_amdgcn_make_buffer_rsrc(const_cast<float*>(p.B + (int64_t)n0 * p.ldb), 0, 0x7ffffff0, 0x00020000);
+
+    u32x4 bs0[4], bs1[4];
+    u32x4 as0[4], as1[4], as2[4], as3[4];
+    uint32_t tb0 = 0, tb1 = 0, tb2 = 0, tb3 = 0;
+
+    const float* a_cur = p.A + (int64_t)s_begin * kAFragSlice;
+    uint32_t vo_cur = voffB;
+    int32_t tail_prev = 0;
+    auto load_table = [&](const float* slice, uint32_t& tb) __attribute__((always_inline)) {
+        const __amdgpu_buffer_rsrc_t rT = __builtin_amdgcn_make_buffer_rsrc(const_cast<float*>(slice), 0, 32, 0x00020000);
+        tb = __builtin_amdgcn_raw_buffer_load_b32(rT, voffT, 0, 0);
+    };
+    auto issue_loads_b = [&](auto pos_tag, u32x4 (&rb)[4], uint32_t tb) __attribute__((always_inline)) -> int32_t {
+        constexpr int s = decltype(pos_tag)::value;
+        const int32_t flags = field(s, F_FLAGS);
+        if constexpr (TAIL) {
+            const int32_t tail = (flags & STEP_TAIL) != 0;
+            if (tail != tail_prev) {
+                vo_cur = tail ? voffBt : voffB;
+                asm volatile("" : "+v"(vo_cur));
+                tail_prev = tail;
+            }
+            const float* bptr = tail ? p.B_tail : p.B + (int64_t)n0 * p.ldb;
+            const __amdgpu_buffer_rsrc_t rB = __builtin_amdgcn_make_buffer_rsrc(const_cast<float*>(bptr), 0, 0x7ffffff0, 0x00020000);
+            const uint32_t qs = tail ? qstepBt : qstepB;
+            const uint32_t vo = vo_cur + (tb << 2);
+#pragma unroll
+            for (int q = 0; q < 4; q++) rb[q] = __builtin_amdgcn_raw_buffer_load_b128(rB, vo, qs * q, 0);
+        } else {
+            const uint32_t vo = voffB + (tb << 2);
+#pragma unroll
+            for (int q = 0; q < 4; q++) rb[q] = __builtin_amdgcn_raw_buffer_load_b128(rBslab, vo, qstepB * q, 0);
+        }
+        return flags;
+    };
+    auto issue_loads_a = [&](int32_t flags, u32x4 (&ra)[4], uint32_t& tb_new) __attribute__((always_inline)) {
+        const int32_t n_quads = (((flags >> STEP_KPAIRS_SHIFT) & 7) >> 1) + 1;
+        const __amdgpu_buffer_rsrc_t rA = __builtin_amdgcn_make_buffer_rsrc(const_cast<float*>(a_cur + 16), 0, n_quads * 1024, 0x00020000);
+#pragma unroll
+        for (int j = 0; j < 4; j++) ra[j] = __builtin_amdgcn_raw_buffer_load_b128(rA, voffA, 1024 * j, 0);
+        load_table(a_cur + 2 * kAFragSlice, tb_new);
+        a_cur += kAFragSlice;
+    };
+    int32_t fq0 = 0, fq1 = 0, fq2 = 0, fq_new = 0;
+
+    auto write_b_q = [&](auto stage_tag, auto q_tag, const u32x4 (&rb)[4]) __attribute__((always_inline)) {
+        constexpr int ST = decltype(stage_tag)::value, q = decltype(q_tag)::value;
+        char* wp = ldsw + lwB + (ST * WSTAGE + 8 * q * LDBW) * 4;
+        uint2 lo, hi;
+        lo.x = rb[q][0]; lo.y = rb[q][1]; hi.x = rb[q][2]; hi.y = rb[q][3];
+        *reinterpret_cast<uint2*>(wp) = lo;
+        *reinterpret_cast<uint2*>(wp + 64) = hi;
+    };
+
+    f32x16 acc;
+#pragma unroll
+    for (int r = 0; r < 16; r++) acc[r] = 0.0f;
+
+    CRing cr;
+    cr.ring = lds + 4 * 2 * WSTAGE + wave * kCRingFloats;
+
+    auto step = [&](auto u_tag, int32_t flags, u32x4 (&wa)[4], u32x4 (&nb)[4], u32x4 (&na)[4], uint32_t tb_use, uint32_t& tb_new) __attribute__((always_inline)) {
+        constexpr int i = decltype(u_tag)::value;
+        constexpr int PAR = i & 1;
+        f32x4 fb[4];
+#pragma unroll
+        for (int j = 0; j < 4; j++) fb[j] = *reinterpret_cast<const f32x4*>(ldsw + lrB + (PAR * WSTAGE + 4 * j) * 4);
+        const int32_t n_pairs = ((flags >> STEP_KPAIRS_SHIFT) & 7) + 1;
+        int32_t flags_new = 0;
+        static_for<0, 8>([&](auto t2_tag) __attribute__((always_inline)) {
+            constexpr int t2 = decltype(t2_tag)::value;
+            if (t2 < n_pairs) {
+                acc = __builtin_amdgcn_mfma_f32_32x32x2f32(fb[t2 >> 1][2 * (t2 & 1)], __uint_as_float(wa[t2 >> 1][2 * (t2 & 1)]), acc, 0, 0, 0);
+                acc = __builtin_amdgcn_mfma_f32_32x32x2f32(fb[t2 >> 1][2 * (t2 & 1) + 1], __uint_as_float(wa[t2 >> 1][2 * (t2 & 1) + 1]), acc, 0, 0, 0);
+            }
+            if constexpr (t2 < 4) {
+                write_b_q(std::integral_constant<int, 1 - PAR>{}, t2_tag, nb);
+            } else if constexpr (t2 == 4) {
+                flags_new = issue_loads_b(std::integral_constant<int, i + 3>{}, nb, tb_use);
+            } else if constexpr (t2 == 5) {
+                issue_loads_a(flags_new, na, tb_new);
+            }
+        });
+        fq_new = flags_new;
+        if (flags & STEP_LAST) {
+            if (flags & STEP_SPLIT) {
+                const __amdgpu_buffer_rsrc_t rW = __builtin_amdgcn_make_buffer_rsrc(ws + (int64_t)field(i, F_SLOT) * SK_SLOT_FLOATS, 0, SK_SLOT_FLOATS * 4, 0x00020000);
+#pragma unroll
+                for (int q = 0; q < 16; q++) {
+                    __builtin_amdgcn_raw_buffer_store_b32(__float_as_uint(acc[q]), rW, (uint32_t)tid * 4u, (uint32_t)(q * kThreads * 4), 0);
+                    __builtin_amdgcn_raw_buffer_store_b32(0u, rW, (uint32_t)tid * 4u, (uint32_t)((16 + q) * kThreads * 4), 0);
+                }
+            } else if (CSTAGE) {
+                cr.park(p, n0, lm, g, voffC, acc, field(i, F_CROW), flags & 0xffff);
+            } else {
+                const int mt = flags & 0xffff;
+                const int64_t c_row = field(i, F_CROW);
+                float* cbase = p.c_row_major ? p.C + c_row * p.ldc + n0 : p.C + c_row + (int64_t)n0 * p.ldc;
+                const __amdgpu_buffer_rsrc_t rC = __builtin_amdgcn_make_buffer_rsrc(cbase, 0, 0x7ffffff0, 0x00020000);
+                const uint32_t jstep = p.c_row_major ? 4u : (uint32_t)p.ldc * 4u;
+                if (lm < mt) {
+                    float v[16];
+#pragma unroll
+                    for (int q = 0; q < 16; q++) v[q] = acc[q];
+                    if (p.accumulate) {
+                        uint32_t old[16];
+#pragma unroll
+                        for (int q = 0; q < 16; q++) old[q] = __builtin_amdgcn_raw_buffer_load_b32(rC, voffC, (uint32_t)((q & 3) + 8 * (q >> 2)) * jstep, 0);
+#pragma unroll
+                        for (int q = 0; q < 16; q++) v[q] += __uint_as_float(old[q]);
+                    }
+                    if (p.c_nt) {
+#pragma unroll
+                        for (int q = 0; q < 16; q++) __builtin_amdgcn_raw_buffer_store_b32(__float_as_uint(v[q]), rC, voffC, (uint32_t)((q & 3) + 8 * (q >> 2)) * jstep, 2);
+                    } else {
+#pragma unroll
+                        for (int q = 0; q < 16; q++) __builtin_amdgcn_raw_buffer_store_b32(__float_as_uint(v[q]), rC, voffC, (uint32_t)((q & 3) + 8 * (q >> 2)) * jstep, 0);
+                    }
+                }
+            }
+#pragma unroll
+            for (int q = 0; q < 16; q++) acc[q] = 0.0f;
+        }
+    };
+
+    using c0 = std::integral_constant<int, 0>;
+    using c1 = std::integral_constant<int, 1>;
+    using c2 = std::integral_constant<int, 2>;
+    using c3 = std::integral_constant<int, 3>;
+    auto window_swap = [&]() __attribute__((always_inline)) {
+        asm volatile("s_waitcnt vmcnt(16)" : "+v"(vnext) : : "memory");
+        vwin = vnext;
+    };
+    auto window_request = [&](int i) __attribute__((always_inline)) {
+        const int32_t* nb = srec + (int64_t)(i + 4) * 8 + lane;
+        asm volatile("global_load_dword %0, %1, off" : "=&v"(vnext) : "v"(nb) : "memory");
+    };
+    load_table(a_cur, tb0);
+    load_table(a_cur + kAFragSlice, tb1);
+    fq0 = issue_loads_b(c0{}, bs0, tb0);
+    issue_loads_a(fq0, as0, tb2);
+    fq1 = issue_loads_b(c1{}, bs1, tb1);
+    issue_loads_a(fq1, as1, tb3);
+#pragma unroll
+    for (int q = 0; q < 4; q++) {
+        char* wp = ldsw + lwB + (8 * q * LDBW) * 4;
+        uint2 lo, hi;
+        lo.x = bs0[q][0]; lo.y = bs0[q][1]; hi.x = bs0[q][2]; hi.y = bs0[q][3];
+        *reinterpret_cast<uint2*>(wp) = lo;
+        *reinterpret_cast<uint2*>(wp + 64) = hi;
+    }
+    fq2 = issue_loads_b(c2{}, bs0, tb2);
+    issue_loads_a(fq2, as2, tb0);
+    const int n4 = n & ~3;
+    for (int i = 0; i < n4; i += 4) {
+        if (i > 0) window_swap();
+        window_request(i);
+        step(c0{}, fq0, as0, bs1, as3, tb3, tb1);
+        fq0 = fq1; fq1 = fq2; fq2 = fq_new;
+        step(c1{}, fq0, as1, bs0, as0, tb0, tb2);
+        fq0 = fq1; fq1 = fq2; fq2 = fq_new;
+        step(c2{}, fq0, as2, bs1, as1, tb1, tb3);
+        fq0 = fq1; fq1 = fq2; fq2 = fq_new;
+        step(c3{}, fq0, as3, bs0, as2, tb2, tb0);
+        fq0 = fq1; fq1 = fq2; fq2 = fq_new;
+    }
+    if (n > n4) {
+        if (n4 > 0) window_swap();
+        step(c0{}, fq0, as0, bs1, as3, tb3, tb1);
+        fq0 = fq1; fq1 = fq2; fq2 = fq_new;
+        if (n - n4 >= 2) {
+            step(c1{}, fq0, as1, bs0, as0, tb0, tb2);
+            fq0 = fq1; fq1 = fq2; fq2 = fq_new;
+        }
+        if (n - n4 == 3) step(c2{}, fq0, as2, bs1, as1, tb1, tb3);
+    }
+    if (CSTAGE) cr.flush(p, n0, lm, g, voffC, true);
+    clock_probe(p.clk, 2);
+#undef field
+}
+
+__global__ __launch_bounds__(kThreads) void vbs_f32_legacy_from_pack_kernel(const StepRec* steps, const PackLoc* loc, int64_t n_steps, const float* a_pack, float* A) {
+    for (int64_t q = blockIdx.x; q < n_steps; q += gridDim.x) {
+        const int64_t a_off = steps[q].a_off, h = steps[q].h;
+        const int mt = steps[q].mt_flags & 0xffff;
+        const float* frag = a_pack + (int64_t)loc[q].step * kAFragSlice + 16;
+        const uint32_t mask = ((uint32_t)loc[q].slot0_mask >> 8) & 0xffu, slot0 = (uint32_t)loc[q].slot0_mask & 0xffu;
+        for (int x = threadIdx.x; x < 32 * 32; x += kThreads) {
+            const int k = x >> 5, m = x & 31;
+            if (m >= mt) continue;
+            const int gm = k >> 2, e = k & 3;
+            float v = 0.0f;
+            if ((mask >> gm) & 1u) {
+                const int s = (int)slot0 + __builtin_popcount(mask & ((1u << gm) - 1u));
+                v = frag[(((s >> 1) * 2 + (e >> 1)) * 32 + m) * 4 + 2 * (s & 1) + (e & 1)];
+            }
+            A[a_off + (int64_t)k * h + m] = v;
+        }
+    }
+}
+
+}
+
+namespace sparta_dev {
+
+void launch_f32_legacy_from_pack(hipStream_t st, const StepRec* steps, const PackLoc* loc, int64_t n_steps, const float* a_pack, float* A) {
+    const unsigned grid = (unsigned)std::max<int64_t>(1, std::min<int64_t>(n_steps, 65536));
+    hipLaunchKernelGGL(vbs_f32_legacy_from_pack_kernel, dim3(grid), dim3(kThreads), 0, st, steps, loc, n_steps, a_pack, A);
+}
+
+void launch_f32_packed(bool c_stage, dim3 grid, hipStream_t st, const StreamParams& sp) {
+    if (sp.B_tail != nullptr) {
+        if (c_stage) hipLaunchKernelGGL((vbs_spmm_f32_packed_kernel<true, true>), grid, dim3(kThreads), 0, st, sp);
+        else hipLaunchKernelGGL((vbs_spmm_f32_packed_kernel<false, true>), grid, dim3(kThreads), 0, st, sp);
+    } else {
+        if (c_stage) hipLaunchKernelGGL((vbs_spmm_f32_packed_kernel<true, false>), grid, dim3(kThreads), 0, st, sp);
+        else hipLaunchKernelGGL((vbs_spmm_f32_packed_kernel<false, false>), grid, dim3(kThreads), 0, st, sp);
+    }
+}
+
+}
diff --git a/sparta_amd/csrc/vbs_capi.cpp b/sparta_amd/csrc/vbs_capi.cpp
--- a/sparta_amd/csrc/vbs_capi.cpp
+++ b/sparta_amd/csrc/vbs_capi.cpp
@@ -52,6 +52,10 @@
         if (v->d_wrange[ty]) (void)hipFree(v->d_wrange[ty]);
     }
     if (v->d_a_frag) (void)hipFree(v->d_a_frag);
+    if (v->d_a_pack) (void)hipFree(v->d_a_pack);
+    if (v->d_psteps) (void)hipFree(v->d_psteps);
+    if (v->d_pwrange) (void)hipFree(v->d_pwrange);
+    if (v->d_pack_loc) (void)hipFree(v->d_pack_loc);
     if (v->d_hub_steps) (void)hipFree(v->d_hub_steps);
     if (v->d_hub_steps_g) (void)hipFree(v->d_hub_steps_g);
     if (v->d_hub_tiles) (void)hipFree(v->d_hub_tiles);
@@ -644,7 +648,7 @@
 
     StreamPlanHost plan;
     {
-        StreamPlanIn pin{cols, w, br0, br1, jab_lo, mab_lo, row_part, nzcount, jab, mab, dtype, device, skip, updatable && h16};
+        StreamPlanIn pin{cols, w, br0, br1, jab_lo, mab_lo, row_part, nzcount, jab, mab, dtype, device, skip, updatable && h16, !h16 && flags == 0};
         trace.lap("tile lists");
         if (int rc = build_stream_plans(pin, plan)) return rc;
         trace.lap("stream plans");
@@ -762,6 +766,24 @@
                 v->d_a_frag = nullptr;
             }
         }
+        if (!plan.a_pack.empty()) {
+            std::vector<StepRec>& ps = plan.psteps;
+            v->n_psteps = (int64_t)ps.size(); v->pack_slots = plan.pack_slots;
+            for (int k = 0; k < 32; k++) { StepRec d = ps[(size_t)v->n_psteps - 1]; d.mt_flags = (d.mt_flags & ~(STEP_LAST | STEP_SPLIT)) | STEP_FIRST; ps.push_back(d); }
+            if (hipMalloc((void**)&v->d_a_pack, plan.a_pack.size() * sizeof(float)) == hipSuccess) {
+                CREATE_TRY(hipMemcpy(v->d_a_pack, plan.a_pack.data(), plan.a_pack.size() * sizeof(float), hipMemcpyHostToDevice));
+                v->a_bytes += (int64_t)(plan.a_pack.size() * sizeof(float));
+                CREATE_TRY(hipMalloc((void**)&v->d_psteps, ps.size() * sizeof(StepRec)));
+                CREATE_TRY(hipMemcpy(v->d_psteps, ps.data(), ps.size() * sizeof(StepRec), hipMemcpyHostToDevice));
+                CREATE_TRY(hipMalloc((void**)&v->d_pwrange, plan.pwrange.size() * sizeof(int32_t)));
+                CREATE_TRY(hipMemcpy(v->d_pwrange, plan.pwrange.data(), plan.pwrange.size() * sizeof(int32_t), hipMemcpyHostToDevice));
+                CREATE_TRY(hipMalloc((void**)&v->d_pack_loc, plan.pack_loc.size() * sizeof(PackLoc)));
+                CREATE_TRY(hipMemcpy(v->d_pack_loc, plan.pack_loc.data(), plan.pack_loc.size() * sizeof(PackLoc), hipMemcpyHostToDevice));
+            } else {
+                (void)hipGetLastError();
+                v->d_a_pack = nullptr; v->n_psteps = 0; v->pack_slots = 0;
+            }
+        }
         if (plan.n_hub_steps > 0) {
             v->hub_g = plan.hub_g; v->hub_workers = plan.hub_workers; v->n_hub_steps = plan.n_hub_steps; v->hub_area = plan.hub_area;
             v->hub_union_area = plan.hub_union_area; v->n_hub_tiles = plan.n_hub_tiles; v->n_hub_groups = plan.n_hub_groups;
@@ -1085,6 +1107,19 @@
     info[9] = A->n_sp_rows;
     info[10] = A->a_bytes; info[11] = A->exec_area;
     info[12] = A->n_steps[0] + A->n_steps[1]; info[13] = A->n_workers; info[14] = A->n_split; info[15] = A->last_path;
+    return SPARTA_OK;
+}
+
+int sparta_vbs_packed_info(const sparta_vbs_t* A, int64_t* info) {
+    if (!A || !info) return sparta::fail(SPARTA_ERR_INVALID, "sparta_vbs_packed_info: NULL argument");
+    info[0] = A->d_a_pack != nullptr; info[1] = A->n_psteps; info[2] = A->pack_slots; info[3] = A->dtype == SPARTA_F32 ? A->n_steps[0] : 0;
+    return SPARTA_OK;
+}
+
+int sparta_f32_pack_blocks(int32_t n_blocks, const uint8_t* group_masks, int32_t* step_of_block, int32_t* slot0_of_block, int32_t* n_steps) {
+    if (n_blocks < 0 || !n_steps || (n_blocks > 0 && (!group_masks || !step_of_block || !slot0_of_block)))
+        return sparta::fail(SPARTA_ERR_INVALID, "sparta_f32_pack_blocks: bad argument");
+    *n_steps = f32_pack_blocks(n_blocks, group_masks, step_of_block, slot0_of_block);
     return SPARTA_OK;
 }
 
@@ -1319,7 +1354,8 @@
     const size_t bytes = (size_t)(A->nztot + 128) * sizeof(float);
     HIP_TRY(hipMalloc((void**)&A->d_A, bytes));
     HIP_TRY(hipMemsetAsync(A->d_A, 0, bytes, st));
-    if (A->n_steps[0] > 0) launch_f32_legacy_from_frag(st, A->d_steps[0], A->n_steps[0], A->d_a_frag, A->d_A);
+    if (A->n_steps[0] > 0 && A->d_a_pack) launch_f32_legacy_from_pack(st, A->d_steps[0], A->d_pack_loc, A->n_steps[0], A->d_a_pack, A->d_A);
+    else if (A->n_steps[0] > 0) launch_f32_legacy_from_frag(st, A->d_steps[0], A->n_steps[0], A->d_a_frag, A->d_A);
     HIP_TRY(hipGetLastError());
     A->a_bytes += (int64_t)bytes;
     return SPARTA_OK;
@@ -1327,7 +1363,7 @@
 void drop_legacy_image(sparta_vbs_t* A) {
     static const bool keep = [] { const char* e = std::getenv("SPARTA_F32_KEEP_LEGACY"); return e && atoi(e) != 0; }();
     if (A->create_flags & SPARTA_CREATE_TRANSPOSE) return;
-    if (keep || g_capturing || A->legacy_dropped || !A->d_A || !A->d_a_frag || A->dtype != SPARTA_F32 || A->n_steps[1] != 0 || A->n_sp_rows != 0 || A->class_timing) return;
+    if (keep || g_capturing || A->legacy_dropped || !A->d_A || !(A->d_a_frag || A->d_a_pack) || A->dtype != SPARTA_F32 || A->n_steps[1] != 0 || A->n_sp_rows != 0 || A->class_timing) return;
     (void)hipFree(A->d_A);
     A->d_A = nullptr;
     A->a_bytes -= (int64_t)((A->nztot + 128) * sizeof(float));
@@ -1734,7 +1770,7 @@
                 if (int rc = ensure_scratch(&A->d_ws, &A->d_ws_bytes, slab * n_nt * sizeof(float))) return rc;
             if (shard_rows > 0)
                 if (int rc = ensure_gathered_steps(A, shard_rows, st)) return rc;
-            if (A->n_steps[1] > 0 || !(A->d_a_frag && b_layout == SPARTA_COL_MAJOR && shard_rows == 0))
+            if (A->n_steps[1] > 0 || !((A->d_a_frag || A->d_a_pack) && b_layout == SPARTA_COL_MAJOR && shard_rows == 0))
                 if (int rc = ensure_legacy_image(A, st)) return rc;
             StreamParams sp;
             sp.A = A->d_A; sp.B = dB; sp.C = Cout; sp.ws = (float*)A->d_ws;
@@ -1757,13 +1793,15 @@
                     if (A->n_steps[ty] == 0) continue;
                     sp.steps = shard_rows > 0 ? A->d_steps_g[ty] : A->d_steps[ty]; sp.worker_range = A->d_wrange[ty]; sp.c_nt = c_store_nt(A, ty, sp.C, sp.ldc, sp.c_row_major != 0);
                     sp.clk = (prof && ty == probe_ty) ? A->d_clk : nullptr;
-                    if (ty == 0 && A->d_a_frag && b_layout == SPARTA_COL_MAJOR && shard_rows == 0) {
+                    if (ty == 0 && (A->d_a_frag || A->d_a_pack) && b_layout == SPARTA_COL_MAJOR && shard_rows == 0) {
                         StreamParams sd = sp;
-                        sd.A = A->d_a_frag;
+                        sd.A = A->d_a_pack ? A->d_a_pack : A->d_a_frag;
+                        if (A->d_a_pack) { sd.steps = A->d_psteps; sd.worker_range = A->d_pwrange; }
                         const int cst = [] { const char* e = std::getenv("SPARTA_CSTAGE"); return e ? atoi(e) : -1; }();
                         const bool c_stage = c_layout == SPARTA_COL_MAJOR && (cst >= 0 ? cst != 0 : ring_tiles(A));
                         sd.c_nt = c_store_nt(A, ty, sd.C, sd.ldc, sd.c_row_major != 0, c_stage);
-                        launch_f32_direct(c_stage, grid, st, sd);
+                        if (A->d_a_pack) launch_f32_packed(c_stage, grid, st, sd);
+                        else launch_f32_direct(c_stage, grid, st, sd);
                     } else launch_f32_stream(ty != 0, b_layout == SPARTA_ROW_MAJOR, shard_rows > 0, grid, st, sp);
                 }
                 if (prof) { HIP_TRY(hipEventRecord(A->cev[0][1], st)); A->class_ran[0] = true; }
diff --git a/sparta_amd/csrc/vbs_device.hpp b/sparta_amd/csrc/vbs_device.hpp
--- a/sparta_amd/csrc/vbs_device.hpp
+++ b/sparta_amd/csrc/vbs_device.hpp
@@ -80,6 +80,10 @@
     int32_t c_row, mt;
     int32_t slot_begin, n_slots;
 };
+
+constexpr int32_t kPackNoRow = 0x20000000;
+constexpr int kPackPadSlices = 8;
+struct PackLoc { int32_t step; int32_t slot0_mask; };
 
 struct StreamParams {
     const StepRec* steps;
@@ -316,6 +320,11 @@
     bool tiles_row_aligned[2] = {true, true};
     bool wide16 = false;
     float* d_a_frag = nullptr;
+    float* d_a_pack = nullptr;
+    sparta_dev::StepRec* d_psteps = nullptr;
+    int32_t* d_pwrange = nullptr;
+    sparta_dev::PackLoc* d_pack_loc = nullptr;
+    int64_t n_psteps = 0, pack_slots = 0;
     bool legacy_dropped = false;
     sparta_dev::HubStep* d_hub_steps = nullptr;
     sparta_dev::HubStep* d_hub_steps_g = nullptr;
@@ -430,6 +439,8 @@
 void launch_f32_stream(bool mi2, bool b_row_major, bool gathered, dim3 grid, hipStream_t st, const StreamParams& sp);
 void launch_f32_direct(bool c_stage, dim3 grid, hipStream_t st, const StreamParams& sp);
 void launch_f32_legacy_from_frag(hipStream_t st, const StepRec* steps, int64_t n_steps, const float* a_frag, float* A);
+void launch_f32_packed(bool c_stage, dim3 grid, hipStream_t st, const StreamParams& sp);
+void launch_f32_legacy_from_pack(hipStream_t st, const StepRec* steps, const PackLoc* loc, int64_t n_steps, const float* a_pack, float* A);
 void launch_fixup_group(dim3 grid, hipStream_t st, const FixRec* fix, const int32_t* big, const int32_t* fix_slots, float* ws_all, int64_t ws_slab_stride);
 void launch_fixup(dim3 grid, hipStream_t st, const FixRec* fix, const int32_t* fix_slots, const float* ws_all, int64_t ws_slab_stride, float* C, int64_t ldc,
                   int c_row_major, int accumulate);
@@ -476,6 +487,7 @@
     int32_t dtype, device;
     const uint8_t* skip;
     bool updatable = false;
+    bool allow_pack = false;
 };
 struct StreamPlanHost {
     std::vector<StepRec> steps[2];
@@ -492,6 +504,11 @@
     int64_t n_plan_tiles[2] = {0, 0};
     bool tiles_row_aligned[2] = {true, true};
     std::vector<float> a_frag;
+    std::vector<StepRec> psteps;
+    std::vector<int32_t> pwrange;
+    std::vector<float> a_pack;
+    std::vector<PackLoc> pack_loc;
+    int64_t pack_slots = 0;
     std::vector<HubStep> hub_steps;
     std::vector<HubTile> hub_tiles;
     std::vector<int32_t> hub_wrange;
diff --git a/sparta_amd/csrc/vbs_kernel_common.hpp b/sparta_amd/csrc/vbs_kernel_common.hpp
--- a/sparta_amd/csrc/vbs_kernel_common.hpp
+++ b/sparta_amd/csrc/vbs_kernel_common.hpp
@@ -21,6 +21,26 @@
 __host__ __device__ inline int frag_pairs(uint32_t nonempty) {
     const int nk = __builtin_popcount(nonempty), n_mfma = nk + 1 >= 2 ? (nk + 1) / 2 : 1;
     return (n_mfma + 1) / 2;
+}
+
+inline int32_t f32_pack_blocks(int32_t n_blocks, const uint8_t* masks, int32_t* step_of_block, int32_t* slot0_of_block) {
+    int32_t fill[8 + 1];
+    std::vector<int32_t> order((size_t)std::max(n_blocks, 0)), used;
+    for (int c = 0; c <= 8; c++) fill[c] = 0;
+    for (int32_t b = 0; b < n_blocks; b++) fill[__builtin_popcount(masks[b])]++;
+    int32_t at = 0, start[9];
+    for (int c = 8; c >= 0; c--) { start[c] = at; at += fill[c]; }
+    for (int32_t b = 0; b < n_blocks; b++) order[(size_t)start[__builtin_popcount(masks[b])]++] = b;
+    for (int32_t q = 0; q < n_blocks; q++) {
+        const int32_t b = order[(size_t)q], c = __builtin_popcount(masks[b]);
+        size_t s = 0;
+        while (s < used.size() && used[s] + c > 8) s++;
+        if (s == used.size()) used.push_back(0);
+        step_of_block[b] = (int32_t)s;
+        slot0_of_block[b] = used[s];
+        used[s] += c;
+    }
+    return (int32_t)used.size();
 }
 
 }
diff --git a/sparta_amd/csrc/vbs_plan.cpp b/sparta_amd/csrc/vbs_plan.cpp
--- a/sparta_amd/csrc/vbs_plan.cpp
+++ b/sparta_amd/csrc/vbs_plan.cpp
@@ -131,8 +131,68 @@
                 for (const HubGroup& g : hub_groups) for (int u = 0; u < g.n; u++) hub_role[(size_t)(g.ib[u] - br0)] = 1;
             }
         }
+        bool pack_decided = false;
+        std::vector<int32_t> tile_psteps;
+        std::vector<uint8_t> pack_masks;
+        {
+            constexpr double kPackMinSaving = 0.05;
+            constexpr int64_t kPackMinSteps = 4096;
+            const char* de = std::getenv("SPARTA_F32_PLAN");
+            const bool never = de && (std::strcmp(de, "direct") == 0 || std::strcmp(de, "legacy") == 0), force = de && std::strcmp(de, "packed") == 0;
+            if (!h16 && in.allow_pack && !never) {
+                const int64_t nbr = br1 - br0, spb = w / SK_KP;
+                std::vector<std::vector<int32_t>> per_row((size_t)nbr);
+                std::vector<std::vector<uint8_t>> row_masks((size_t)nbr);
+                sparta::parallel_for_dynamic(nbr, 4, [&](int64_t lo, int64_t hi, int) {
+                    std::vector<uint8_t> mk;
+                    std::vector<int32_t> sob, s0b;
+                    for (int64_t i = lo; i < hi; i++) {
+                        const int64_t ib = br0 + i, h = row_part[ib + 1] - row_part[ib], nb = nzcount[ib];
+                        if ((in.skip && in.skip[i]) || nb == 0) continue;
+                        for (int64_t r0 = 0; r0 < h; r0 += SK_TM) {
+                            const int64_t mt = std::min<int64_t>(SK_TM, h - r0);
+                            if (mt > 32) continue;
+                            mk.clear();
+                            int32_t tails = 0;
+                            for (int64_t b = 0; b < nb; b++) {
+                                const bool tail = (jab[jab_lo + jo_of[(size_t)i] + b] + 1) * w > cols;
+                                for (int64_t ks = 0; ks < w; ks += SK_KP) {
+                                    const float* blk = mab + mab_lo + mo_of[(size_t)i] + r0 + (b * w + ks) * h;
+                                    uint8_t m8 = 0;
+                                    for (int k = 0; k < 32; k++) {
+                                        bool any = false;
+                                        for (int64_t m = 0; m < mt && !any; m++) any = blk[(int64_t)k * h + m] != 0.0f;
+                                        if (any) m8 |= (uint8_t)(1u << (k >> 2));
+                                    }
+                                    row_masks[(size_t)i].push_back(m8);
+                                    if (tail) tails++; else mk.push_back(m8);
+                                }
+                            }
+                            sob.resize(mk.size()); s0b.resize(mk.size());
+                            per_row[(size_t)i].push_back(f32_pack_blocks((int32_t)mk.size(), mk.data(), sob.data(), s0b.data()) + tails);
+                        }
+                    }
+                });
+                int64_t S0 = 0, PS0 = 0, area0 = 0;
+                for (int64_t i = 0; i < nbr; i++) {
+                    const int64_t ib = br0 + i, h = row_part[ib + 1] - row_part[ib];
+                    size_t t = 0;
+                    for (int64_t r0 = 0; r0 < h && !per_row[(size_t)i].empty(); r0 += SK_TM) {
+                        const int64_t mt = std::min<int64_t>(SK_TM, h - r0);
+                        if (mt > 32) continue;
+                        S0 += nzcount[ib] * spb; area0 += nzcount[ib] * spb * mt * SK_KP; PS0 += per_row[(size_t)i][t];
+                        tile_psteps.push_back(per_row[(size_t)i][t++]);
+                    }
+                }
+                const bool frag_ok0 = S0 > 0 && S0 <= ((int64_t)2 << 20) && S0 * kAFragSlice <= 4 * std::max<int64_t>(area0, 1) + (1 << 20);
+                pack_decided = frag_ok0 && (force || (S0 >= kPackMinSteps && (double)PS0 <= (1.0 - kPackMinSaving) * (double)S0));
+                if (pack_decided) for (const auto& rm : row_masks) pack_masks.insert(pack_masks.end(), rm.begin(), rm.end());
+                else tile_psteps.clear();
+            }
+        }
         for (int ty = 0; ty < 2; ty++) {
             std::vector<StepRec>& st = steps[ty];
+            size_t pack_tile_no = 0, pack_mask_no = 0;
             struct TileSpan { int64_t first, last; int32_t c_row, mt; };
             std::vector<TileSpan> spans;
             std::vector<int64_t> cum;
@@ -195,6 +255,8 @@
                             continue;
                         }
                         TileSpan sp{(int64_t)st.size(), 0, c_row, mt};
+                        const int64_t tile_steps = nb * (w / kp), tile_cost = (pack_decided && ty == 0) ? (int64_t)c1 * tile_psteps[pack_tile_no++] : 0;
+                        int64_t step_no = 0;
                         for (int64_t b = 0; b < nb; b++) {
                             const int64_t jb = jab[jab_lo + jo2 + b];
                             for (int64_t ks = 0; ks < w; ks += kp) {
@@ -206,7 +268,7 @@
                                 r.mt_flags = mt;
                                 if ((jb + 1) * w > cols) { r.mt_flags |= STEP_TAIL; r.b_row = (int32_t)ks; }
                                 r.slot = -1;
-                                r.pad = 0;
+                                r.pad = tile_cost ? (int32_t)++pack_mask_no : 0;
                                 if (dbg_probe) {
                                     if (dbg_probe & 1) r.b_row = (int32_t)ks;
                                     if ((dbg_probe & 2) && h16) r.a_off = (ks) * h;
@@ -214,7 +276,8 @@
                                     if (dbg_probe & 4) r.c_row = 0;
                                 }
                                 cum.push_back(total_cost);
-                                total_cost += ty ? c2 : c1;
+                                total_cost += tile_cost ? tile_cost * (step_no + 1) / tile_steps - tile_cost * step_no / tile_steps : (ty ? c2 : c1);
+                                step_no++;
                                 st.push_back(r);
                             }
                         }
@@ -500,7 +563,99 @@
                 const bool off = de && std::strcmp(de, "legacy") == 0;
                 int64_t one_tile_area = 0;
                 for (int64_t q = 0; q < S; q++) one_tile_area += (int64_t)(st[(size_t)q].mt_flags & 0xffff) * SK_KP;
-                if (!off && ty == 0 && !h16 && S <= ((int64_t)2 << 20) && S * kAFragSlice <= 4 * std::max<int64_t>(one_tile_area, 1) + (1 << 20)) {
+                const bool frag_ok = !off && ty == 0 && !h16 && S <= ((int64_t)2 << 20) && S * kAFragSlice <= 4 * std::max<int64_t>(one_tile_area, 1) + (1 << 20);
+                bool packed = false;
+                if (frag_ok && pack_decided) {
+                    if (pack_tile_no != tile_psteps.size() || pack_mask_no != pack_masks.size() || (int64_t)pack_masks.size() != S)
+                        return fail(SPARTA_ERR_INVALID, "sparta_vbs_create: internal error, the packed plan's tiles do not match the one-tile plan");
+                    std::vector<uint8_t> gmask((size_t)S, 0);
+                    for (int64_t q = 0; q < S; q++) { gmask[(size_t)q] = pack_masks[(size_t)st[(size_t)q].pad - 1]; st[(size_t)q].pad = 0; }
+                    std::vector<StepRec>& ps = P.psteps;
+                    std::vector<PackLoc>& loc = P.pack_loc;
+                    std::vector<int64_t> pstart((size_t)S + 1, 0);
+                    std::vector<int32_t> slots_of;
+                    loc.assign((size_t)S, PackLoc{0, 0});
+                    std::vector<uint8_t> mk;
+                    std::vector<int32_t> idx, sob, s0b;
+                    int64_t n_slots = 0;
+                    for (int64_t a = 0; a < S;) {
+                        int64_t b = a;
+                        while (!(st[(size_t)b].mt_flags & STEP_LAST)) b++;
+                        const int64_t base = (int64_t)ps.size();
+                        pstart[(size_t)a] = base;
+                        mk.clear(); idx.clear();
+                        for (int64_t q = a; q <= b; q++)
+                            if (!(st[(size_t)q].mt_flags & STEP_TAIL)) { mk.push_back(gmask[(size_t)q]); idx.push_back((int32_t)(q - a)); }
+                        sob.assign(mk.size(), 0); s0b.assign(mk.size(), 0);
+                        const int32_t ns = f32_pack_blocks((int32_t)mk.size(), mk.data(), sob.data(), s0b.data());
+                        StepRec proto = st[(size_t)a];
+                        proto.mt_flags &= 0xffff; proto.slot = -1; proto.pad = 0; proto.b_row = 0;
+                        ps.insert(ps.end(), (size_t)ns, proto);
+                        slots_of.insert(slots_of.end(), (size_t)ns, 0);
+                        for (size_t u = 0; u < mk.size(); u++) {
+                            const int64_t q = a + idx[u];
+                            const int32_t cnt = __builtin_popcount(mk[u]);
+                            loc[(size_t)q] = PackLoc{(int32_t)(base + sob[u]), s0b[u] | ((int32_t)mk[u] << 8)};
+                            slots_of[(size_t)(base + sob[u])] = std::max(slots_of[(size_t)(base + sob[u])], s0b[u] + cnt);
+                            n_slots += cnt;
+                        }
+                        for (int64_t q = a; q <= b; q++) {
+                            if (!(st[(size_t)q].mt_flags & STEP_TAIL)) continue;
+                            StepRec tr = proto;
+                            tr.mt_flags |= STEP_TAIL;
+                            tr.b_row = st[(size_t)q].b_row;
+                            loc[(size_t)q] = PackLoc{(int32_t)ps.size(), (int32_t)gmask[(size_t)q] << 8};
+                            slots_of.push_back(__builtin_popcount(gmask[(size_t)q]));
+                            n_slots += __builtin_popcount(gmask[(size_t)q]);
+                            ps.push_back(tr);
+                        }
+                        for (size_t u = (size_t)base; u < ps.size(); u++)
+                            ps[u].mt_flags |= (std::max(slots_of[u], 1) - 1) << STEP_KPAIRS_SHIFT;
+                        ps[(size_t)base].mt_flags |= STEP_FIRST;
+                        ps.back().mt_flags |= st[(size_t)b].mt_flags & (STEP_LAST | STEP_SPLIT);
+                        ps.back().slot = st[(size_t)b].slot;
+                        a = b + 1;
+                    }
+                    const int64_t PS = (int64_t)ps.size();
+                    pstart[(size_t)S] = PS;
+                    packed = true;
+                    {
+                        P.pack_slots = n_slots;
+                        P.pwrange.assign((size_t)n_workers * 2, 0);
+                        for (int pos = 0; pos < n_workers; pos++) {
+                            P.pwrange[(size_t)wid_of_pos[(size_t)pos] * 2] = (int32_t)pstart[(size_t)bnd[(size_t)pos]];
+                            P.pwrange[(size_t)wid_of_pos[(size_t)pos] * 2 + 1] = (int32_t)pstart[(size_t)bnd[(size_t)pos + 1]];
+                        }
+                        std::vector<float>& ap = P.a_pack;
+                        ap.assign(((size_t)PS + kPackPadSlices) * (size_t)kAFragSlice, 0.0f);
+                        for (size_t u = 0; u < (size_t)PS + kPackPadSlices; u++) {
+                            int32_t* tab = reinterpret_cast<int32_t*>(ap.data() + u * (size_t)kAFragSlice);
+                            for (int sl = 0; sl < 8; sl++) tab[sl] = kPackNoRow;
+                        }
+                        sparta::parallel_for_dynamic(S, 256, [&](int64_t lo, int64_t hi, int) {
+                            for (int64_t q = lo; q < hi; q++) {
+                                const StepRec& r = st[(size_t)q];
+                                const float* blk = mab + mab_lo + r.a_off;
+                                const int64_t hh = r.h, mt = r.mt_flags & 0xffff;
+                                float* dst = ap.data() + (size_t)loc[(size_t)q].step * (size_t)kAFragSlice;
+                                int32_t* tab = reinterpret_cast<int32_t*>(dst);
+                                float* frag = dst + 16;
+                                const int32_t mask = (loc[(size_t)q].slot0_mask >> 8) & 0xff;
+                                int sl = loc[(size_t)q].slot0_mask & 0xff;
+                                for (int gm = 0; gm < 8; gm++) {
+                                    if (!((mask >> gm) & 1)) continue;
+                                    tab[sl] = r.b_row + 4 * gm;
+                                    for (int e = 0; e < 4; e++) {
+                                        const int j = sl >> 1, g = e >> 1, e2 = 2 * (sl & 1) + (e & 1);
+                                        for (int64_t m = 0; m < mt; m++) frag[((j * 2 + g) * 32 + m) * 4 + e2] = blk[(int64_t)(4 * gm + e) * hh + m];
+                                    }
+                                    sl++;
+                                }
+                            }
+                        });
+                    }
+                }
+                if (frag_ok && !packed) {
                     std::vector<float>& af = P.a_frag;
                     af.assign(((size_t)S + 4) * (size_t)kAFragSlice, 0.0f);
                     sparta::parallel_for_dynamic(S, 256, [&](int64_t lo, int64_t hi, int) {
diff --git a/sparta_amd/device.py b/sparta_amd/device.py
--- a/sparta_amd/device.py
+++ b/sparta_amd/device.py
@@ -123,6 +123,11 @@
                 "sparse_rows", "a_bytes", "exec_area", "stream_steps", "stream_workers", "split_tiles", "last_path"]
         return {k: int(a[i]) for i, k in enumerate(keys)}
 
+    def packed_info(self):
+        a = np.zeros(4, np.int64)
+        check(lib.sparta_vbs_packed_info(self.h, a.ctypes.data_as(_i64p)))
+        return {"packed": int(a[0]), "steps": int(a[1]), "slots": int(a[2]), "block_steps": int(a[3])}
+
     def sparse_info(self):
         a = np.zeros(4, np.int64)
         check(lib.sparta_vbs_sparse_info(self.h, a.ctypes.data_as(_i64p)))
```
